# zhongzisha/multi_frame_super_resolution

Hardware: AMD Instinct MI355X
Metric: Mpix/s end-to-end (N-frame burst -> x2 SR) (higher is better)
Workload: dtype f32

## Files before the change

### include/mfsr.h

```cpp
#ifndef MFSR_H
#define MFSR_H

#include <stddef.h>
#include <stdint.h>

#ifdef __cplusplus
extern "C" {
#endif

#define MFSR_VERSION 100
#define MFSR_MAX_FUSE_GROUP 4
#define MFSR_MAX_BURST_FUSE 16

typedef void* mfsr_stream_t;

typedef struct { float x, y; } mfsr_float2;
typedef struct { float x, y, z; } mfsr_float3;
typedef struct { float x, y, z, w; } mfsr_float4;

typedef struct {
    const void* ptr;
    int32_t pitch;
    int32_t width;
    int32_t height;
// ... 233 lines not shown
int mfsr_preAlignPyramid(const float* img, int width, int height, int pitch, void* pyramid, mfsr_stream_t stream);
int mfsr_preAlign(const void* refPyramid, const void* movedPyramid, int width, int height, float maxAngleDeg,
                  void* workspace, mfsr_prealign* result, mfsr_stream_t stream);
int mfsr_preAlign_identity(mfsr_prealign* result, mfsr_stream_t stream);
int mfsr_trackTilesFusedBase(const float* refImg, const float* movedImg, const mfsr_float2* preShift, int preShiftPitch,
                             mfsr_float2* coordinates, int coordinatesPitch, int imgWidth, int imgHeight, int imgPitch,
                             int maxShift, int tileSize, int tileCountX, int tileCountY, float threshold,
                             const float* refSquaredSums, const mfsr_prealign* base, float baseInvScale,
                             mfsr_stream_t stream);
int mfsr_trackTilesFusedUp(const float* refImg, const float* movedImg, const mfsr_float2* coarseShifts, int coarsePitch,
                           int oldLevel, int newLevel, int oldCountX, int oldCountY, int oldTileSize, mfsr_float2* coordinates,
                           int coordinatesPitch, int imgWidth, int imgHeight, int imgPitch, int maxShift, int tileSize,
                           int tileCountX, int tileCountY, float threshold, const float* refSquaredSums,
                           const mfsr_prealign* base, float baseInvScale, mfsr_stream_t stream);
int mfsr_CreateFlowFieldFromTilesBase(mfsr_float2* outImg, mfsr_tex2d texObjShiftXY, int imgWidth, int imgHeight,
                                      int imgPitch, const mfsr_prealign* base, mfsr_stream_t stream);
int mfsr_lucasKanadeIterationWarped(const mfsr_float2* shiftsIn, mfsr_float2* shiftsOut, int pitchShift, const float* refImg,
                                    const float* movedImg, int pitchImg, const float* sumIn, const float* diffIn, float* sumOut,
                                    float* diffOut, int pitchSD, int width, int height, int halfWindowSize, float minDet,
                                    float outScale, mfsr_stream_t stream);
typedef struct {
    const uint16_t* dataIn;
    mfsr_float3* halfOut;
    float* pyr0;
    float* pyr1;
} mfsr_prepare_frame;
int mfsr_prepareFrameFusedBatch(int nFrames, const mfsr_prepare_frame* frames, int halfPitch, float maxVal, int dimX, int dimY,
                                int pyr0Pitch, int pyr1Pitch, const float* taps, int ntaps, mfsr_stream_t stream);
typedef struct {
    const float* movedImg;
    const mfsr_float2* coarseShifts;
    mfsr_float2* coordinates;
    const mfsr_prealign* base;
} mfsr_track_frame;
int mfsr_trackTilesFastSupported(int tileSize, int maxShift);
int mfsr_trackTilesFusedBatch(int nFrames, const mfsr_track_frame* frames, const float* refImg, int coarsePitch, int oldLevel,
                              int newLevel, int oldCountX, int oldCountY, int oldTileSize, int coordinatesPitch, int imgWidth,
                              int imgHeight, int imgPitch, int maxShift, int tileSize, int tileCountX, int tileCountY, float threshold,
                              const float* refSquaredSums, float baseInvScale, mfsr_stream_t stream);
typedef struct {
    mfsr_float2* outImg;
    const mfsr_float2* tileShifts;
    const mfsr_prealign* base;
    const float* movedImg;
    float* sumOut;
    float* diffOut;
} mfsr_flowfield_frame;
int mfsr_CreateFlowFieldWarpedBatch(int nFrames, const mfsr_flowfield_frame* frames, int tilePitch, int tileCountX, int tileCountY,
                                    int imgWidth, int imgHeight, int imgPitch, const float* refImg, int pitchImg, int pitchSD,
                                    mfsr_stream_t stream);
typedef struct {
    const mfsr_float3* movedHalf;
    mfsr_float4* mask;
    const mfsr_float2* flow;
} mfsr_robustness_frame;
int mfsr_robustnessMaskFusedBatch(int nFrames, const mfsr_robustness_frame* frames, const mfsr_float3* rawImgRef, int flowPitch,
                                  int flowWidth, int flowHeight, int imgWidth, int imgHeight, int imgPitch, int maskPitch, float alpha,
                                  float beta, float thresholdM, mfsr_stream_t stream);
int mfsr_prepareFrameMeansBatch(int nFrames, const mfsr_prepare_frame* frames, int meansRowBytes, float maxVal, int w, int h,
                                int pyr0RowBytes, int pyr1RowBytes, const float* taps, int ntaps, mfsr_stream_t stream);
typedef struct {
    const mfsr_float3* movedMeans;
    const uint16_t* movedRaw;
    mfsr_float4* mask;
    const mfsr_float2* flow;
} mfsr_robustness_group_frame;
int mfsr_robustnessMaskGroup(int nFrames, const mfsr_robustness_group_frame* frames, const mfsr_float3* refHalf, int refRowBytes,
                             int flowRowBytes, int meansRowBytes, int maskRowBytes, int w, int h, float maxVal, float alpha,
                             float beta, float thresholdM, mfsr_stream_t stream);
int mfsr_set_robustness_group(int enable);
typedef struct {
    const mfsr_float2* shiftsIn;
    mfsr_float2* shiftsOut;
    const float* movedImg;
    const float* sumIn;
    const float* diffIn;
    float* sumOut;
    float* diffOut;
} mfsr_lk_frame;
int mfsr_lucasKanadeSweepBatch(int nFrames, const mfsr_lk_frame* frames, const float* refImg, int pitchShift, int pitchImg,
                               int pitchSD, int width, int height, int halfWindowSize, float minDet, float outScale,
                               mfsr_stream_t stream);
int mfsr_lucasKanadeSweepBand(int width, int height, int halfWindowSize, int nFrames);
int mfsr_CreateFlowFieldWarped(mfsr_float2* outImg, mfsr_tex2d texObjShiftXY, int imgWidth, int imgHeight, int imgPitch,
                               mfsr_float2 baseShift, float baseRotation, const mfsr_prealign* base, const float* refImg,
                               const float* movedImg, int pitchImg, float* sumOut, float* diffOut, int pitchSD,
                               mfsr_stream_t stream);

int mfsr_finishFusedRows(const mfsr_float3* finalImg, const mfsr_float3* weight, int imgPitch, const mfsr_float3* fallback,
                         int fbPitch, int fbW, int fbH, float u0, float u1, float v0, float v1, mfsr_float3* outImg,
                         int outPitch, uint16_t* out16, int width, int height, float threshold, int applyGamma, float maxOut,
                         int rowOffset, int fullHeight, mfsr_stream_t stream);
int mfsr_finishFusedWindow(const mfsr_float3* finalImg, const mfsr_float3* weight, int imgPitch, const mfsr_float3* fallback,
                           int fbPitch, int fbW, int fbH, float u0, float u1, float v0, float v1, mfsr_float3* outImg,
                           int outPitch, uint16_t* out16, int width, int height, float threshold, int applyGamma, float maxOut,
                           int colOffset, int rowOffset, int fullWidth, int fullHeight, mfsr_stream_t stream);

typedef struct {
    int32_t width, height;
    int32_t frames;
    int32_t reference;
    int32_t scale;
    int32_t mono;
    int32_t cfa[4];
    float black[3], white[3];
    float maxVal;
    int32_t levels;
    int32_t levelFactor[4];
    int32_t tileSize[4];
    int32_t maxShift[4];
    float minimumThreshold;
    float sigmaTracking;
    int32_t lkIterations;
    int32_t lkHalfWindow;
    float lkMinDet;
    float alpha, beta, thresholdM;
    float sigmaTensor;
    float Dth, Dtr, kDetail, kDenoise, kStretch, kShrink;
    float weightThreshold;
    int32_t applyGamma;
    int32_t fused;
    int32_t pairFrames;
    int32_t asyncFuse;
    int32_t preAlign;
    float preAlignMaxAngle;
    int32_t uploadRing;
    int32_t maskErode;
    int32_t rawPacking;
} mfsr_config;

typedef struct mfsr_burst mfsr_burst;

int mfsr_config_default(mfsr_config* cfg, int width, int height, int frames, int scale, int mono);
size_t mfsr_burst_workspace_bytes(const mfsr_config* cfg);
size_t mfsr_burst_accumulator_bytes(const mfsr_config* cfg);
int mfsr_burst_create(mfsr_burst** out, const mfsr_config* cfg, void* workspace, size_t workspaceBytes);
void mfsr_burst_destroy(mfsr_burst* b);

int mfsr_window_check(const mfsr_config* cfg, int x0, int y0, int w, int h);
int mfsr_burst_set_window(mfsr_burst* b, int x0, int y0, int w, int h);
int mfsr_burst_get_window(const mfsr_burst* b, int* x0, int* y0, int* w, int* h);
int mfsr_burst_set_reference(mfsr_burst* b, const uint16_t* rawRef, mfsr_stream_t stream);
int mfsr_burst_set_reference_rows(mfsr_burst* b, const uint16_t* rawRef, int hrRow0, int hrRow1, mfsr_stream_t stream);
int mfsr_burst_add_frame(mfsr_burst* b, const uint16_t* raw, int isReference, mfsr_float3* imgOut,
                         mfsr_float3* totalWeights, mfsr_stream_t stream);
int mfsr_burst_begin(mfsr_burst* b, mfsr_float3* imgOut, mfsr_float3* totalWeights, mfsr_stream_t stream);
int mfsr_burst_flush(mfsr_burst* b, mfsr_stream_t stream);
int mfsr_burst_hold_fuse(mfsr_burst* b, int enable);
int mfsr_burst_fuse_stats(const mfsr_burst* b, int* burstLaunches, int* groupsFused);
int mfsr_set_burst_fuse(int enable);
int mfsr_set_margin_sites(int enable);
int mfsr_set_finish_fuse(int enable);
int mfsr_burst_debug_finish_fused(const mfsr_burst* b, int* finishes);
int mfsr_burst_finish(mfsr_burst* b, const mfsr_float3* imgOut, const mfsr_float3* totalWeights, mfsr_float3* outImg,
                      uint16_t* out16, mfsr_stream_t stream);
int mfsr_burst_finish_rows(mfsr_burst* b, const mfsr_float3* imgOut, const mfsr_float3* totalWeights,
                           mfsr_float3* outImg, uint16_t* out16, int row0, int rows, mfsr_stream_t stream);
int mfsr_burst_set_reference_host(mfsr_burst* b, const uint16_t* hostRaw, mfsr_stream_t stream);
int mfsr_burst_add_frame_host(mfsr_burst* b, const uint16_t* hostRaw, int isReference, mfsr_float3* imgOut,
                              mfsr_float3* totalWeights, mfsr_stream_t stream);
int mfsr_burst_prefetch_host(mfsr_burst* b, const uint16_t* const* hostRaws, int nFrames, mfsr_stream_t stream);
int mfsr_burst_finish_host(mfsr_burst* b, const mfsr_float3* imgOut, const mfsr_float3* totalWeights, uint16_t* out16Dev,
                           uint16_t* out16Host, mfsr_stream_t stream);
int mfsr_burst_host_sync(mfsr_burst* b);
int mfsr_burst_set_host_row_bytes(mfsr_burst* b, int rowBytes);
int mfsr_burst_field_dims(const mfsr_burst* b, int* flowW, int* flowH, int* maskW, int* maskH);
int mfsr_burst_align_frame(mfsr_burst* b, const uint16_t* raw, int isReference, mfsr_float2* flowOut, int flowPitch,
                           mfsr_float4* maskOut, int maskPitch, mfsr_stream_t stream);
int mfsr_burst_align_frames(mfsr_burst* b, int nFrames, const uint16_t* const* raws, const int* isReference,
                            mfsr_float2* const* flowOut, int flowPitch, mfsr_float4* const* maskOut, int maskPitch,
                            mfsr_stream_t stream);
int mfsr_burst_group_size(const mfsr_config* cfg);
int mfsr_burst_fuse_rows(mfsr_burst* b, int nFrames, const uint16_t* const* raws, const mfsr_float2* const* flows, int flowPitch,
                         const mfsr_float4* const* masks, int maskPitch, mfsr_float3* imgOut, mfsr_float3* totalWeights,
                         int accumulatorsUndefined, int rowBegin, int rowEnd, mfsr_stream_t stream);

typedef struct {
    int32_t rowBegin, rowEnd;
    int32_t flowRow0, flowRows;
    int32_t maskRow0, maskRows;
    int32_t rawRow0, rawRows;
    float maxFlowY;
    int32_t reserved[3];
} mfsr_stripe_plan;
int mfsr_dist_stripe_plan(const mfsr_config* cfg, int worldSize, int rank, int rawHalo, mfsr_stripe_plan* out);
int mfsr_checkFlowBound(const mfsr_float2* flow, int pitch, int width, int rows, float bound, int* flag, mfsr_stream_t stream);
int mfsr_maxAbsFlowY(const mfsr_float2* flow, int pitch, int width, int rows, int* maxBits, mfsr_stream_t stream);
int mfsr_exactDivisionOk(float d);

typedef struct mfsr_stream mfsr_stream;
size_t mfsr_stream_workspace_bytes(const mfsr_config* cfg, int radius);
int mfsr_stream_create(mfsr_stream** out, const mfsr_config* cfg, int radius, int framesInHostMemory, void* workspace,
                       size_t workspaceBytes);
void mfsr_stream_destroy(mfsr_stream* s);
int mfsr_stream_push(mfsr_stream* s, const uint16_t* frame, mfsr_float3* outImg, uint16_t* out16, long long* produced,
                     mfsr_stream_t stream);
int mfsr_stream_drain(mfsr_stream* s, mfsr_float3* outImg, uint16_t* out16, long long* produced, mfsr_stream_t stream);
int mfsr_stream_reset(mfsr_stream* s);
int mfsr_stream_set_window(mfsr_stream* s, int x0, int y0, int w, int h);

size_t mfsr_burst_joint_workspace_bytes(const mfsr_config* cfg);
int mfsr_burst_process_joint(mfsr_burst* b, const uint16_t* const* frames, void* jointWorkspace, size_t jointBytes,
                             mfsr_float3* imgOut, mfsr_float3* totalWeights, mfsr_stream_t stream);

typedef struct {
    int (*next_frame)(void* user, uint16_t* dst, mfsr_stream_t stream);
    void (*reset)(void* user);
    void* user;
} mfsr_frame_source;
int mfsr_burst_process_source(mfsr_burst* b, const mfsr_frame_source* src, mfsr_float3* imgOut, mfsr_float3* totalWeights,
                              mfsr_float3* outImg, uint16_t* out16, int* framesUsed, mfsr_stream_t stream);

int mfsr_frameSharpness(int nFrames, const uint16_t* const* frames, int pitch, int width, int height, const int32_t cfa[4],
                        int mono, const int32_t rect[4], long long* sumsDev, mfsr_stream_t stream);
int mfsr_select_frames(int n, const long long* sums, int candidates, float keepRatio, int* reference, int32_t* keep);
int mfsr_burst_select_frames(mfsr_burst* b, int nFrames, const uint16_t* const* frames, int candidates, float keepRatio,
                             long long* sumsDev, int* reference, int32_t* keep, long long* sums, int32_t rect[4],
                             mfsr_stream_t stream);

int mfsr_detectDefects(int nFrames, const uint16_t* const* frames, int pitch, int width, int height, int mono, int threshold,
                       int spread, int minVotes, uint8_t* mapDev, int mapPitch, uint32_t* countsDev, mfsr_stream_t stream);
int mfsr_repairDefects(int nFrames, uint16_t* const* frames, int pitch, int width, int height, int mono, const uint8_t* mapDev,
                       int mapPitch, mfsr_stream_t stream);
int mfsr_burst_repair_defects(mfsr_burst* b, int nFrames, uint16_t* const* frames, int threshold, int spread, int minVotes,
                              uint8_t* mapDev, uint32_t* countsDev, uint32_t counts[2], mfsr_stream_t stream);

int mfsr_frameLevels(int nFrames, const uint16_t* const* frames, int pitch, int width, int height, const int32_t black[4], int sat,
                     const int32_t rect[4], long long* levelsDev, mfsr_stream_t stream);
int mfsr_exposure_gains(int n, const long long* levels, int reference, const int32_t cfa[4], int mono, int perColour, int deadband,
                        int minGain, int maxGain, int32_t* gains, int32_t* status);
int mfsr_applyGains(int nFrames, uint16_t* const* frames, int pitch, int width, int height, const int32_t cfa[4], int mono,
                    const int32_t black[4], int sat, int maxValue, const int32_t* gains, const int32_t* status, mfsr_stream_t stream);
int mfsr_exposure_defaults(const mfsr_config* cfg, int32_t black[4], int32_t* sat, int32_t* maxValue, int32_t* deadband,
                           int32_t* minGain, int32_t* maxGain, int32_t* perColour);
int mfsr_burst_match_exposure(mfsr_burst* b, int nFrames, uint16_t* const* frames, int reference, int perColour, int deadband,
// ... 309 lines not shown
```

### multi_frame_super_resolution_amd/capi.py

```python
from __future__ import annotations

import ctypes
import os
import re
from typing import Dict, List, Tuple

_PKG_DIR = os.path.dirname(os.path.abspath(__file__))
_ROOT = os.path.dirname(_PKG_DIR)
HEADER_PATH = os.path.join(_ROOT, "include", "mfsr.h")
LIB_PATH = os.environ.get("MFSR_LIB") or os.path.join(_PKG_DIR, "lib", "libmfsr_hip.so")


class Float2(ctypes.Structure):
    _fields_ = [("x", ctypes.c_float), ("y", ctypes.c_float)]


class Float3(ctypes.Structure):
    _fields_ = [("x", ctypes.c_float), ("y", ctypes.c_float), ("z", ctypes.c_float)]


class Float4(ctypes.Structure):
    _fields_ = [("x", ctypes.c_float), ("y", ctypes.c_float), ("z", ctypes.c_float), ("w", ctypes.c_float)]


# ... 177 lines not shown
        ret = re.sub(r"\s+", " ", m.group(1)).replace(" *", "*").strip()
        name = m.group(2)
        args = []
        argtxt = re.sub(r"\s+", " ", m.group(3)).strip()
        if argtxt and argtxt != "void":
            for a in argtxt.split(","):
                a = a.strip()
                am = re.match(r"^(.*?)(\w+)(\[\d*\])?$", a)
                typ = am.group(1).strip()
                if am.group(3):
                    typ += "*"
                typ = typ.replace(" *", "*").replace("* ", "*")
                args.append((typ, am.group(2)))
        protos[name] = (ret, args)
    return protos


def path_names(path: str = HEADER_PATH) -> List[str]:
    text = re.sub(r"/\*.*?\*/", " ", open(path).read(), flags=re.S)
    m = re.search(r"typedef\s+enum\s*\{([^{}]*)\}\s*mfsr_path\s*;", text)
    if not m:
        raise ValueError("mfsr.h: enum mfsr_path not found")
    names = [re.sub(r"\s*=.*", "", e).strip() for e in m.group(1).split(",")]
    names = [n for n in names if n]
    if names[-1] != "MFSR_PATH_COUNT" or any(not n.startswith("MFSR_PATH_") for n in names):
        raise ValueError("mfsr.h: unexpected enumerators in mfsr_path")
    return [n[len("MFSR_PATH_"):].lower() for n in names[:-1]]


def _ctype_of(typ: str):
    if "*" in typ:
        return ctypes.c_void_p
    base = typ.replace("const", "").strip()
    if base not in _BY_VALUE:
        raise TypeError(f"mfsr.h: unhandled parameter type {typ!r}")
    return _BY_VALUE[base]


class MfsrError(RuntimeError):
    def __init__(self, fn: str, code: int, msg: str):
        super().__init__(f"{fn} failed with code {code}: {msg}")
        self.code = code


class StripePlan(ctypes.Structure):

    _fields_ = [("rowBegin", ctypes.c_int32), ("rowEnd", ctypes.c_int32), ("flowRow0", ctypes.c_int32),
                ("flowRows", ctypes.c_int32), ("maskRow0", ctypes.c_int32), ("maskRows", ctypes.c_int32),
                ("rawRow0", ctypes.c_int32), ("rawRows", ctypes.c_int32), ("maxFlowY", ctypes.c_float),
                ("reserved", ctypes.c_int32 * 3)]


DIST_HEADER_PATH = os.path.join(_ROOT, "include", "mfsr_dist.h")
DIST_LIB_PATH = os.path.join(_PKG_DIR, "lib", "libmfsr_dist.so")
DIST_STRIPES, DIST_REDUCE, DIST_REDUCE_SCATTER = 0, 1, 2
DIST_ID_BYTES = 128


class _Lib:

    def __init__(self, path: str = LIB_PATH, header: str = HEADER_PATH, mode: int = ctypes.DEFAULT_MODE):
        if not os.path.exists(path):
            raise ImportError(
                f"{path} is missing: build it with `python -c 'import __graft_entry__ as g; g.build()'` "
                "(hipcc --offload-arch=gfx950).  There is no CPU fallback.")
        self.path = path
        self.cdll = ctypes.CDLL(path, mode=mode)
        self.protos = parse_header(header)
        self.raw = {}
        for name, (ret, args) in self.protos.items():
            fn = getattr(self.cdll, name)
            fn.restype = _RET[ret]
            fn.argtypes = [_ctype_of(t) for t, _ in args]
            self.raw[name] = fn

    def __getattr__(self, name: str):
        raw = self.__dict__["raw"].get("mfsr_" + name) or self.__dict__["raw"].get(name)
        if raw is None:
            raise AttributeError(name)
        full = raw.__name__ if hasattr(raw, "__name__") else name
        ret = self.protos[full][0]
        if ret != "int" or full in ("mfsr_version", "mfsr_device_count", "mfsr_gaussin_filter_1D", "mfsr_burst_group_size",
                                     "mfsr_trackTilesFastSupported", "mfsr_packed_row_bytes", "mfsr_render_row_bytes",
                                     "mfsr_get_accumulate_fast_exp", "mfsr_exactDivisionOk", "mfsr_lucasKanadeSweepBand"):
            return raw

        def checked(*a):
            rc = raw(*a)
            if rc != 0:
                es = self.raw.get("mfsr_error_string") or lib().raw["mfsr_error_string"]
                msg = es(rc)
                raise MfsrError(full, rc, msg.decode() if msg else "?")
            return rc

        checked.__name__ = full
        return checked


_lib = None
_dist_lib = None


def lib() -> _Lib:
    global _lib
    if _lib is None:
        _lib = _Lib()
    return _lib


def dist_lib() -> _Lib:
    global _dist_lib
    if _dist_lib is None:
        lib()
        _dist_lib = _Lib(DIST_LIB_PATH, DIST_HEADER_PATH)
    return _dist_lib


def f3(v) -> Float3:
    return Float3(float(v[0]), float(v[1]), float(v[2]))


def f2(v) -> Float2:
    return Float2(float(v[0]), float(v[1]))


def tex(t, width: int | None = None, height: int | None = None, pitch: int | None = None) -> Tex2D:
    h = t.shape[0] if height is None else height
    w = t.shape[1] if width is None else width
    p = t.stride(0) * t.element_size() if pitch is None else pitch
    return Tex2D(t.data_ptr(), p, w, h)
```

### multi_frame_super_resolution_amd/csrc/common.hpp

```cpp
#pragma once

#include <hip/hip_runtime.h>

#include <atomic>
#include <cstdint>
#include <cstdio>
#include <cstdlib>

#include "../../include/mfsr.h"

#define MFSR_WAVE 64

#define MFSR_HIP_TRY(expr)                                                                          \
    do {                                                                                            \
        hipError_t e_ = (expr);                                                                     \
        if (e_ != hipSuccess) {                                                                     \
            fprintf(stderr, "mfsr: %s failed: %s (%s:%d)\n", #expr, hipGetErrorString(e_), __FILE__, \
                    __LINE__);                                                                      \
            return (int)e_;                                                                         \
        }                                                                                           \
    } while (0)

#define MFSR_REQUIRE(cond)                                                                  \
    do {                                                                                    \
        if (!(cond)) {                                                                      \
            fprintf(stderr, "mfsr: invalid argument: %s (%s:%d)\n", #cond, __FILE__, __LINE__); \
            return MFSR_E_INVALID;                                                          \
        }                                                                                   \
    } while (0)

static inline int mfsr_launch_status(const char* what)
{
    hipError_t e = hipGetLastError();
    if (e != hipSuccess) {
        fprintf(stderr, "mfsr: launch of %s failed: %s\n", what, hipGetErrorString(e));
        return (int)e;
    }
    return MFSR_OK;
}

static inline hipStream_t mfsr_s(mfsr_stream_t s) { return (hipStream_t)s; }

static inline bool mfsr_window_ok(int hrW, int hrH, int x0, int y0, int w, int h)
{
    if (hrW <= 0 || hrH <= 0 || x0 < 0 || y0 < 0 || w <= 0 || h <= 0) return false;
    if ((x0 % 16) != 0 || (y0 % 16) != 0) return false;
    if ((long long)x0 + w > hrW || (long long)y0 + h > hrH) return false;
    if ((w % 16) != 0 && x0 + w != hrW) return false;
    if ((h % 16) != 0 && y0 + h != hrH) return false;
    return true;
}
static inline unsigned mfsr_cdiv(long long a, long long b) { return (unsigned)((a + b - 1) / b); }
int mfsr_render_validate(const mfsr_render* r);
static inline mfsr_render mfsr_plain_render()
{
    mfsr_render r = {};
    r.format = MFSR_OUT_RGB16;
    return r;
}

#define MFSR_BATCH_MAX 4

#define MFSR_INTERNAL __attribute__((visibility("hidden")))

static inline bool mfsr_env_is0(const char* name)
{
    const char* e = getenv(name);
    return e && e[0] == '0';
}
static inline bool mfsr_env_is1(const char* name)
{
    const char* e = getenv(name);
    return e && e[0] == '1';
}
static inline int mfsr_env_int(const char* name, int dflt)
{
    const char* e = getenv(name);
    return e ? atoi(e) : dflt;
}
class MfsrKnob {
public:
    template <class FromEnv>
    int get(FromEnv fromEnv)
    {
        int v = v_.load(std::memory_order_relaxed);
        if (v < 0) {
            const int e = fromEnv();
            if (v_.compare_exchange_strong(v, e, std::memory_order_relaxed)) v = e;
        }
        return v;
    }
    void set(int v) { v_.store(v, std::memory_order_relaxed); }

private:
    std::atomic<int> v_{-1};
};

static inline int mfsr_device_cus()
{
    constexpr int kDevs = 64;
    static std::atomic<int> cache[kDevs];
    int dev = 0, cus = 0;
    if (hipGetDevice(&dev) != hipSuccess || dev < 0 || dev >= kDevs) return 256;
    if ((cus = cache[dev].load(std::memory_order_relaxed)) > 0) return cus;
    if (hipDeviceGetAttribute(&cus, hipDeviceAttributeMultiprocessorCount, dev) != hipSuccess || cus <= 0) return 256;
    cache[dev].store(cus, std::memory_order_relaxed);
    return cus;
}

static inline int mfsr_pack_cfa(const int32_t pattern[4], int* packed)
{
    MFSR_REQUIRE(pattern != nullptr);
    for (int i = 0; i < 4; i++) MFSR_REQUIRE(pattern[i] >= 0 && pattern[i] <= MFSR_WHITE);
    *packed = pattern[0] | (pattern[1] << 8) | (pattern[2] << 16) | (pattern[3] << 24);
    return MFSR_OK;
}
MFSR_INTERNAL int mfsr_cfa_packed();
namespace mfsr_cfa {
MFSR_INTERNAL int deBayersSubSample3(int cfa, const uint16_t* dataIn, mfsr_float3* imgOut, float maxVal, int dimX, int dimY, int strideOut,
                                     mfsr_stream_t stream);
MFSR_INTERNAL int prepareFrames(int cfa, int n, const mfsr_prepare_frame* f, int halfPitch, float maxVal, int dimX, int dimY, int pyr0Pitch,
                                int pyr1Pitch, const float* taps, int ntaps, mfsr_stream_t stream, bool means);
MFSR_INTERNAL int deBayerGreenKernel(int cfa, int width, int height, const float* imgIn, int strideIn, mfsr_float3* outImage, int strideOut,
                                     mfsr_float3 blackPoint, mfsr_float3 scale, mfsr_stream_t stream);
MFSR_INTERNAL int deBayerRedBlueKernel(int cfa, int width, int height, const float* imgIn, int strideIn, mfsr_float3* outImage,
                                       int strideOut, mfsr_float3 blackPoint, mfsr_float3 scale, mfsr_stream_t stream);
MFSR_INTERNAL int deBayerFused(int cfa, const uint16_t* raw, mfsr_float3* outImage, int strideOut, int width, int height,
                               mfsr_float3 blackPoint, mfsr_float3 scale, mfsr_stream_t stream);
MFSR_INTERNAL int deBayerFusedRing(int cfa, const uint16_t* raw, mfsr_tex2d outImage, mfsr_float3 blackPoint, mfsr_float3 scale,
                                   mfsr_stream_t stream);
MFSR_INTERNAL int accumulateSuperResFullRows(int cfa, int nFrames, const uint16_t* const* dataIn, mfsr_float3* imgOut,
                                             mfsr_float3* totalWeights, const mfsr_float4* const* certaintyMask, mfsr_tex2d kernelParam,
                                             const mfsr_tex2d* shifts, mfsr_float3 whiteLevel, mfsr_float3 blackLevel, int dimX, int dimY,
                                             int scale, int strideOut, int strideMask, int accumulatorsUndefined, int rowBegin, int rowEnd,
                                             mfsr_stream_t stream);
MFSR_INTERNAL int accumulateSuperResFullWindow(int cfa, int nFrames, const uint16_t* const* dataIn, mfsr_float3* imgOut,
                                               mfsr_float3* totalWeights, const mfsr_float4* const* certaintyMask, mfsr_tex2d kernelParam,
                                               const mfsr_tex2d* shifts, mfsr_float3 whiteLevel, mfsr_float3 blackLevel, int dimX, int dimY,
                                               int scale, int strideOut, int strideMask, int accumulatorsUndefined, int x0, int y0, int w,
                                               int h, mfsr_stream_t stream);
MFSR_INTERNAL int accumulateSuperResBurst(int cfa, int nFrames, const uint16_t* const* dataIn, mfsr_tex2d imgOut, mfsr_tex2d totalWeights,
                                          const mfsr_tex2d* certaintyMasks, mfsr_tex2d kernelParam, const mfsr_tex2d* shifts,
                                          mfsr_float3 whiteLevel, mfsr_float3 blackLevel, int scale, int accumulatorsUndefined,
                                          mfsr_stream_t stream);
// ... 132 lines not shown
```

### multi_frame_super_resolution_amd/csrc/debayer.hip

```cpp
#include <cstring>
#include "common.hpp"
#include "half_pixel.hpp"

static std::atomic<int> g_cfa{MFSR_RED | (MFSR_GREEN << 8) | (MFSR_GREEN << 16) | (MFSR_BLUE << 24)};

int mfsr_cfa_packed() { return g_cfa.load(std::memory_order_relaxed); }

extern "C" int mfsr_set_cfa_pattern(const int32_t pattern[4])
{
    int packed = 0;
    const int rc = mfsr_pack_cfa(pattern, &packed);
    if (rc == MFSR_OK) g_cfa.store(packed, std::memory_order_relaxed);
    return rc;
}

extern "C" int mfsr_get_cfa_pattern(int32_t pattern[4])
{
    MFSR_REQUIRE(pattern != nullptr);
    const int packed = mfsr_cfa_packed();
    for (int i = 0; i < 4; i++) pattern[i] = (packed >> (8 * i)) & 0xff;
    return MFSR_OK;
}

__global__ void __launch_bounds__(256) k_deBayersSubSample3(const uint16_t* __restrict__ dataIn, pix3* __restrict__ imgOut,
// ... 98 lines not shown
            if (gx == cx && gy == cy && lx >= c0 && lx < c0 + PREP_TX && ly >= c0 && ly < c0 + PREP_TY) row_ptr(halfOut, halfPitch, gy)[gx] = p;
        }
        sG[i] = 0.299f * p.x + 0.587f * p.y + 0.114f * p.z;
    }
    __syncthreads();
    if (MEANS) {
        static_assert(PREP_TY == 16, "four rows for each of the block's four thread rows");
        const int lx = threadIdx.x, r0 = 4 * threadIdx.y;
        float mean[4][3];
#pragma unroll
        for (int c = 0; c < 3; c++) {
            float v[6][3];
#pragma unroll
            for (int y = 0; y < 6; y++)
#pragma unroll
                for (int x = 0; x < 3; x++) v[y][x] = sM[(c * PREP_MH + r0 + y) * PREP_MW + lx + x];
#pragma unroll
            for (int r = 0; r < 4; r++) {
                float m = 0.0f;
#pragma unroll
                for (int y = 0; y < 3; y++)
#pragma unroll
                    for (int x = 0; x < 3; x++) m += v[r + y][x];
                mean[r][c] = div9(m);
            }
        }
        const int gx = x0 + lx;
#pragma unroll
        for (int r = 0; r < 4; r++) {
            const int gy = y0 + r0 + r;
            if (gx < dimX && gy < dimY) {
                const pix3 o = {mean[r][0], mean[r][1], mean[r][2]};
                row_ptr(halfOut, halfPitch, gy)[gx] = o;
            }
        }
        __syncthreads();
    }
    for (int i = tid; i < PREP_TX * GH; i += 256) {
        const int ly = i / PREP_TX, lx = i - ly * PREP_TX;
        float s = 0;
        for (int t = 0; t < taps.n; t++) s += taps.t[t] * sG[ly * GW + lx + t];
        sH[i] = s;
    }
    __syncthreads();
    {
        const int lx = threadIdx.x;
#pragma unroll
        for (int r = 0; r < PREP_TY / 4; r++) {
            const int ly = threadIdx.y + 4 * r;
            float s = 0;
            for (int t = 0; t < taps.n; t++) s += taps.t[t] * sH[(ly + t) * PREP_TX + lx];
            sO[ly * PREP_TX + lx] = s;
            const int gx = x0 + lx, gy = y0 + ly;
            if (gx < dimX && gy < dimY) row_ptr(pyr0, pyr0Pitch, gy)[gx] = s;
        }
    }
    if (pyr1 == nullptr) return;
    __syncthreads();
    {
        const int ox = tid & 31, oy = tid >> 5;
        const int gx = x0 / 2 + ox, gy = y0 / 2 + oy;
        if (gx < dimX / 2 && gy < dimY / 2) {
            const float ax = sO[(2 * oy) * PREP_TX + 2 * ox], ay = sO[(2 * oy) * PREP_TX + 2 * ox + 1];
            const float bx = sO[(2 * oy + 1) * PREP_TX + 2 * ox], by = sO[(2 * oy + 1) * PREP_TX + 2 * ox + 1];
            row_ptr(pyr1, pyr1Pitch, gy)[gx] = ((ax + ay) + (bx + by)) * 0.25f;
        }
    }
}

int mfsr_cfa::prepareFrames(int cfa, int n, const mfsr_prepare_frame* f, int halfPitch, float maxVal, int dimX, int dimY, int pyr0Pitch,
                            int pyr1Pitch, const float* taps, int ntaps, mfsr_stream_t stream, bool means)
{
    MFSR_REQUIRE(f && n >= 1 && n <= MFSR_BATCH_MAX && taps && dimX > 0 && dimY > 0);
    MFSR_REQUIRE((long long)halfPitch >= 12LL * dimX && (halfPitch & 3) == 0);
    MFSR_REQUIRE((long long)pyr0Pitch >= 4LL * dimX && (pyr0Pitch & 3) == 0);
    MFSR_REQUIRE(ntaps > 0 && (ntaps & 1) == 1);
    if (ntaps / 2 > PREP_MAXC0) return MFSR_E_UNSUPPORTED;
    if (means && ntaps < 3) return MFSR_E_UNSUPPORTED;
    PrepFrames fr;
    memset(&fr, 0, sizeof(fr));
    for (int i = 0; i < n; i++) {
        MFSR_REQUIRE(f[i].dataIn && f[i].halfOut && f[i].pyr0 && ((uintptr_t)f[i].dataIn & 3) == 0);
        MFSR_REQUIRE((f[i].pyr1 != nullptr) == (f[0].pyr1 != nullptr));
        fr.f[i] = PrepFrame{f[i].dataIn, (pix3*)f[i].halfOut, f[i].pyr0, f[i].pyr1};
    }
    if (f[0].pyr1) MFSR_REQUIRE((long long)pyr1Pitch >= 4LL * (dimX / 2) && (pyr1Pitch & 3) == 0 && dimX >= 2 && dimY >= 2);
    PrepTaps tp;
    tp.n = ntaps;
    for (int i = 0; i < ntaps; i++) tp.t[i] = taps[i];
    const int c0 = ntaps / 2, GW = PREP_TX + 2 * c0, GH = PREP_TY + 2 * c0;
    const size_t lds = sizeof(float) * ((size_t)GW * GH + (size_t)PREP_TX * GH + (size_t)PREP_TX * PREP_TY);
    dim3 block(64, 4), grid(mfsr_cdiv(dimX, PREP_TX), mfsr_cdiv(dimY, PREP_TY), n);
    if (means) {
        const size_t planes = 3 * PREP_MW * PREP_MH, rows = (size_t)PREP_TX * GH;
        const size_t ldsMeans = sizeof(float) * ((size_t)GW * GH + (planes > rows ? planes : rows));
        hipLaunchKernelGGL(k_prepareFrameFused<true>, grid, block, ldsMeans, mfsr_s(stream), fr, halfPitch, maxVal, dimX, dimY, pyr0Pitch,
                           pyr1Pitch, tp, cfa);
        return mfsr_launch_status("prepareFrameMeans");
    }
    hipLaunchKernelGGL(k_prepareFrameFused<false>, grid, block, lds, mfsr_s(stream), fr, halfPitch, maxVal, dimX, dimY, pyr0Pitch, pyr1Pitch,
                       tp, cfa);
    return mfsr_launch_status("prepareFrameFused");
}

extern "C" int mfsr_prepareFrameFused(const uint16_t* dataIn, mfsr_float3* halfOut, int halfPitch, float maxVal, int dimX,
                                      int dimY, float* pyr0, int pyr0Pitch, float* pyr1, int pyr1Pitch, const float* taps,
                                      int ntaps, mfsr_stream_t stream)
{
    const mfsr_prepare_frame f = {dataIn, halfOut, pyr0, pyr1};
    return mfsr_cfa::prepareFrames(mfsr_cfa_packed(), 1, &f, halfPitch, maxVal, dimX, dimY, pyr0Pitch, pyr1Pitch, taps, ntaps, stream, false);
}

extern "C" int mfsr_prepareFrameFusedBatch(int nFrames, const mfsr_prepare_frame* frames, int halfPitch, float maxVal, int dimX, int dimY,
                                           int pyr0Pitch, int pyr1Pitch, const float* taps, int ntaps, mfsr_stream_t stream)
{
    return mfsr_cfa::prepareFrames(mfsr_cfa_packed(), nFrames, frames, halfPitch, maxVal, dimX, dimY, pyr0Pitch, pyr1Pitch, taps, ntaps, stream,
                                   false);
}

extern "C" int mfsr_prepareFrameMeansBatch(int nFrames, const mfsr_prepare_frame* frames, int meansRowBytes, float maxVal, int w, int h,
                                           int pyr0RowBytes, int pyr1RowBytes, const float* taps, int ntaps, mfsr_stream_t stream)
{
    return mfsr_cfa::prepareFrames(mfsr_cfa_packed(), nFrames, frames, meansRowBytes, maxVal, w, h, pyr0RowBytes, pyr1RowBytes, taps, ntaps,
                                   stream, true);
}

struct Lvl {
    float bp[3], sc[3];
};

__device__ __forceinline__ float green_at(const float* __restrict__ imgIn, int strideIn, int x, int y, int thisPixel,
                                          const Lvl& L)
{
#define RAWC(xx, yy, c) ((row_ptr(imgIn, strideIn, (yy))[(xx)] - L.bp[c]) * L.sc[c])
    if (thisPixel == MFSR_GREEN) return RAWC(x, y, 1);
    if (thisPixel != MFSR_RED && thisPixel != MFSR_BLUE) return 0.0f;
    const int c = (thisPixel == MFSR_RED) ? 0 : 2;
    const float p = RAWC(x, y, c);
    const float xMinus2 = RAWC(x - 2, y, c), xMinus1 = RAWC(x - 1, y, 1), xPlus1 = RAWC(x + 1, y, 1),
                xPlus2 = RAWC(x + 2, y, c);
    const float yMinus2 = RAWC(x, y - 2, c), yMinus1 = RAWC(x, y - 1, 1), yPlus1 = RAWC(x, y + 1, 1),
                yPlus2 = RAWC(x, y + 2, c);
#undef RAWC
    const float gradientX = 0.5f * fabsf(xPlus1 - xMinus1);
    const float gradientY = 0.5f * fabsf(yPlus1 - yMinus1);
    const float laplaceX = 0.25f * fabsf(2.0f * p - xMinus2 - xPlus2);
    const float laplaceY = 0.25f * fabsf(2.0f * p - yMinus2 - yPlus2);
    const float interpolX = 0.125f * (-xMinus2 + 4.0f * xMinus1 + 2.0f * p + 4.0f * xPlus1 - xPlus2);
    const float interpolY = 0.125f * (-yMinus2 + 4.0f * yMinus1 + 2.0f * p + 4.0f * yPlus1 - yPlus2);
    const float weight = (gradientY + laplaceY) / (gradientX + gradientY + laplaceX + laplaceY + 0.000000001f);
    return weight * interpolX + (1.0f - weight) * interpolY;
}

__global__ void __launch_bounds__(256) k_deBayerGreen(int width, int height, const float* __restrict__ imgIn, int strideIn,
                                                     pix3* outImage, int strideOut, Lvl L, int cfa)
{
    const int x = blockIdx.x * blockDim.x + threadIdx.x;
    const int y = blockIdx.y * blockDim.y + threadIdx.y;
    if (x >= width - 2 || x < 2) return;
    if (y >= height - 2 || y < 2) return;
    row_ptr(outImage, strideOut, y)[x].y = green_at(imgIn, strideIn, x, y, cfa_at(cfa, y, x), L);
}

static inline Lvl make_lvl(mfsr_float3 bp, mfsr_float3 sc)
{
    Lvl L;
// ... 224 lines not shown
```

### multi_frame_super_resolution_amd/csrc/erode.hip

```cpp
#include "common.hpp"

#define ER_TX 64
#define ER_TY 16
#define ER_ROWS 4

struct ErodeFrames {
    const float4* in[MFSR_MAX_FUSE_GROUP];
    float4* out[MFSR_MAX_FUSE_GROUP];
};

__device__ __forceinline__ float4 min3(const float4& a, const float4& b)
{
    return make_float4(fminf(a.x, b.x), fminf(a.y, b.y), fminf(a.z, b.z), 0.0f);
}

template <int R>
__global__ void __launch_bounds__(ER_TX* ER_ROWS)
    k_maskErode(ErodeFrames fr, int width, int height, int inPitch, int outPitch)
{
    constexpr int LW = ER_TX + 2 * R, LH = ER_TY + 2 * R;
    constexpr int NT = ER_TX * ER_ROWS, PER = (LH * ER_TX + NT - 1) / NT;
    __shared__ float4 sT[LH][LW];
    const float4* __restrict__ in = fr.in[blockIdx.z];
    float4* __restrict__ out = fr.out[blockIdx.z];
    const int lx = threadIdx.x, ly = threadIdx.y;
    const int tid = ly * ER_TX + lx;
    const int x0 = blockIdx.x * ER_TX, y0 = blockIdx.y * ER_TY;
    for (int t = tid; t < LH * LW; t += NT) {
        const int r = t / LW, c = t - r * LW;
        const int gy = clampi(y0 - R + r, 1, height - 2), gx = clampi(x0 - R + c, 1, width - 2);
        sT[r][c] = row_ptr(in, inPitch, gy)[gx];
    }
    __syncthreads();
    float4 m[PER];
#pragma unroll
    for (int k = 0; k < PER; k++) {
        const int t = tid + k * NT;
        if (t < LH * ER_TX) {
            const int r = t / ER_TX, c = t - r * ER_TX;
            float4 v = sT[r][c];
#pragma unroll
            for (int i = 1; i <= 2 * R; i++) v = min3(v, sT[r][c + i]);
            v.w = sT[r][c + R].w;
            m[k] = v;
        }
    }
    __syncthreads();
#pragma unroll
    for (int k = 0; k < PER; k++) {
        const int t = tid + k * NT;
        if (t < LH * ER_TX) sT[t / ER_TX][t % ER_TX] = m[k];
    }
    __syncthreads();
    const int x = x0 + lx;
    if (x >= width) return;
#pragma unroll
    for (int k = 0; k < ER_TY / ER_ROWS; k++) {
        const int r = ly + k * ER_ROWS, y = y0 + r;
        if (y >= height) break;
        float4 v = sT[r][lx];
#pragma unroll
        for (int j = 1; j <= 2 * R; j++) v = min3(v, sT[r + j][lx]);
        v.w = sT[r + R][lx].w;
        if (x < 1 || y < 1 || x >= width - 1 || y >= height - 1) v = make_float4(0.0f, 0.0f, 0.0f, 0.0f);
        row_ptr(out, outPitch, y)[x] = v;
    }
}

extern "C" int mfsr_erodeMaskBatch(int nFrames, const mfsr_float4* const* in, mfsr_float4* const* out, int width, int height,
                                   int inPitch, int outPitch, int radius, mfsr_stream_t stream)
{
    MFSR_REQUIRE(nFrames >= 1 && nFrames <= MFSR_MAX_FUSE_GROUP && in != nullptr && out != nullptr);
    MFSR_REQUIRE(radius >= 1 && radius <= 2);
    MFSR_REQUIRE(width >= 3 && height >= 3);
    MFSR_REQUIRE((long long)inPitch >= 16LL * width && (inPitch & 15) == 0);
    MFSR_REQUIRE((long long)outPitch >= 16LL * width && (outPitch & 15) == 0);
    ErodeFrames fr;
    for (int k = 0; k < MFSR_MAX_FUSE_GROUP; k++) {
        fr.in[k] = nullptr;
        fr.out[k] = nullptr;
    }
    const unsigned long long inSpan = (unsigned long long)inPitch * (height - 1) + 16ULL * width;
    const unsigned long long outSpan = (unsigned long long)outPitch * (height - 1) + 16ULL * width;
    for (int k = 0; k < nFrames; k++) {
        MFSR_REQUIRE(in[k] != nullptr && out[k] != nullptr);
        MFSR_REQUIRE(((uintptr_t)in[k] & 15) == 0 && ((uintptr_t)out[k] & 15) == 0);
        fr.in[k] = (const float4*)in[k];
        fr.out[k] = (float4*)out[k];
    }
    for (int k = 0; k < nFrames; k++) {
        const unsigned long long o0 = (unsigned long long)(uintptr_t)out[k], o1 = o0 + outSpan;
        for (int j = 0; j < nFrames; j++) {
            const unsigned long long i0 = (unsigned long long)(uintptr_t)in[j];
            MFSR_REQUIRE(o1 <= i0 || i0 + inSpan <= o0);
            if (j != k) {
                const unsigned long long p0 = (unsigned long long)(uintptr_t)out[j];
                MFSR_REQUIRE(o1 <= p0 || p0 + outSpan <= o0);
            }
        }
    }
    dim3 block(ER_TX, ER_ROWS), grid(mfsr_cdiv(width, ER_TX), mfsr_cdiv(height, ER_TY), nFrames);
    if (radius == 1)
        hipLaunchKernelGGL(k_maskErode<1>, grid, block, 0, mfsr_s(stream), fr, width, height, inPitch, outPitch);
    else
        hipLaunchKernelGGL(k_maskErode<2>, grid, block, 0, mfsr_s(stream), fr, width, height, inPitch, outPitch);
    return mfsr_launch_status("erodeMaskBatch");
}
```

### multi_frame_super_resolution_amd/csrc/lk_fused.hip

```cpp
#include <cstdlib>
#include <cstring>
#include "common.hpp"
#include "lk_math.hpp"

constexpr int LK_TY = 16;

__device__ __forceinline__ int lk_mirror_index(int i, int n)
{
    i = i < 0 ? -1 - i : i;
    return i >= n ? 2 * n - 1 - i : i;
}

__device__ __forceinline__ int lk_mirror_index_clamped(int i, int n)
{
    return clampi(lk_mirror_index(i, n), 0, n - 1);
}

template <typename T>
__device__ __forceinline__ T* lk_at(T* base, int pitch, int y, int x)
{
    return (T*)((char*)base + (uint32_t)((uint32_t)y * (uint32_t)pitch + (uint32_t)x * (uint32_t)sizeof(T)));
}

struct LkGather {
// ... 321 lines not shown
        sf = base->sinRotation;
        bx = base->shiftX;
        by = base->shiftY;
    } else {
        if (baseRotation != 0.0f) {
            cf = cosf(baseRotation);
            sf = sinf(baseRotation);
        }
        bx = baseShift.x;
        by = baseShift.y;
    }
    float2 shift;
    shift.x = cf * -bx - sf * -by;
    shift.y = sf * -bx + cf * -by;
    const float patchCenterX = (float)(pxX - imgWidth / 2);
    const float patchCenterY = (float)(pxY - imgHeight / 2);
    shift.x += cf * patchCenterX - sf * patchCenterY - patchCenterX;
    shift.y += sf * patchCenterX + cf * patchCenterY - patchCenterY;
    const float2 shiftPatch =
        tex2<ADDR_CLAMP>(texShift, mfsr_div((float)pxX + 0.5f, dW), mfsr_div((float)pxY + 0.5f, dH));
    shift.x += shiftPatch.x;
    shift.y += shiftPatch.y;
    *lk_at(outImg, imgPitch, pxY, pxX) = shift;
    float wv, rv;
    lk_warp_sample(refImg, movedImg, pitchImg, imgWidth, imgHeight, pxX, pxY, shift, wv, rv, dW, dH);
    *lk_at(sumOut, pitchSD, pxY, pxX) = wv + rv;
    *lk_at(diffOut, pitchSD, pxY, pxX) = wv - rv;
}

static int flow_field_warped_impl(int n, const mfsr_flowfield_frame* f, int tilePitch, int tileW, int tileH, int imgWidth, int imgHeight,
                                  int imgPitch, mfsr_float2 baseShift, float baseRotation, const float* refImg, int pitchImg, int pitchSD,
                                  mfsr_stream_t stream)
{
    MFSR_REQUIRE(f && n >= 1 && n <= MFSR_BATCH_MAX && refImg && imgWidth >= 2 && imgHeight >= 2);
    MFSR_REQUIRE((long long)imgPitch >= 8LL * imgWidth && (imgPitch & 7) == 0);
    MFSR_REQUIRE((long long)pitchImg >= 4LL * imgWidth && (pitchImg & 3) == 0 && (long long)pitchSD >= 4LL * imgWidth && (pitchSD & 3) == 0);
    if ((long long)imgPitch * imgHeight >= (1LL << 32) || (long long)pitchImg * imgHeight >= (1LL << 32) ||
        (long long)pitchSD * imgHeight >= (1LL << 32))
        return MFSR_E_UNSUPPORTED;
    mfsr_tex2d tex;
    tex.ptr = f[0].tileShifts;
    tex.pitch = tilePitch;
    tex.width = tileW;
    tex.height = tileH;
    MFSR_REQUIRE(mfsr_tex_ok(tex, 8) && (tilePitch & 7) == 0);
    FlowFieldFrames fr;
    memset(&fr, 0, sizeof(fr));
    for (int i = 0; i < n; i++) {
        MFSR_REQUIRE(f[i].outImg && f[i].tileShifts && f[i].movedImg && f[i].sumOut && f[i].diffOut);
        MFSR_REQUIRE(((uintptr_t)f[i].outImg & 7) == 0 && ((uintptr_t)f[i].tileShifts & 7) == 0);
        MFSR_REQUIRE((f[i].base != nullptr) == (f[0].base != nullptr));
        fr.f[i] = FlowFieldFrame{(float2*)f[i].outImg, (const float2*)f[i].tileShifts, f[i].base, f[i].movedImg, f[i].sumOut, f[i].diffOut};
    }
    dim3 block(64, 4), grid(mfsr_cdiv(imgWidth, 64), mfsr_cdiv(imgHeight, 4), n);
    const MfsrExactDiv dW = mfsr_exact_div((float)imgWidth), dH = mfsr_exact_div((float)imgHeight);
    if (f[0].base)
        hipLaunchKernelGGL(k_flowFieldWarped<true>, grid, block, 0, mfsr_s(stream), fr, tex, imgWidth, imgHeight, imgPitch,
                           make_float2(0.0f, 0.0f), 0.0f, refImg, pitchImg, pitchSD, dW, dH);
    else
        hipLaunchKernelGGL(k_flowFieldWarped<false>, grid, block, 0, mfsr_s(stream), fr, tex, imgWidth, imgHeight, imgPitch,
                           make_float2(baseShift.x, baseShift.y), baseRotation, refImg, pitchImg, pitchSD, dW, dH);
    return mfsr_launch_status("CreateFlowFieldWarped");
}

extern "C" int mfsr_CreateFlowFieldWarped(mfsr_float2* outImg, mfsr_tex2d texObjShiftXY, int imgWidth, int imgHeight, int imgPitch,
                                          mfsr_float2 baseShift, float baseRotation, const mfsr_prealign* base, const float* refImg,
                                          const float* movedImg, int pitchImg, float* sumOut, float* diffOut, int pitchSD,
                                          mfsr_stream_t stream)
{
    const mfsr_flowfield_frame f = {outImg, (const mfsr_float2*)texObjShiftXY.ptr, base, movedImg, sumOut, diffOut};
    return flow_field_warped_impl(1, &f, texObjShiftXY.pitch, texObjShiftXY.width, texObjShiftXY.height, imgWidth, imgHeight, imgPitch,
                                  baseShift, baseRotation, refImg, pitchImg, pitchSD, stream);
}

extern "C" int mfsr_CreateFlowFieldWarpedBatch(int nFrames, const mfsr_flowfield_frame* frames, int tilePitch, int tileCountX,
                                               int tileCountY, int imgWidth, int imgHeight, int imgPitch, const float* refImg,
                                               int pitchImg, int pitchSD, mfsr_stream_t stream)
{
    const mfsr_float2 z = {0.0f, 0.0f};
    return flow_field_warped_impl(nFrames, frames, tilePitch, tileCountX, tileCountY, imgWidth, imgHeight, imgPitch, z, 0.0f, refImg,
                                  pitchImg, pitchSD, stream);
}

#define MFSR_LK_SWEEP_MAX_BATCH 4
struct LkSweepFrame {
    const float2* flowIn;
    float2* flowOut;
    const float* moved;
    const float* sumIn;
    const float* diffIn;
    float* sumOut;
    float* diffOut;
};
struct LkSweepBatch {
    LkSweepFrame f[MFSR_LK_SWEEP_MAX_BATCH];
};

__device__ __forceinline__ float lk_wshr1(float v)
{
    return __uint_as_float(__builtin_amdgcn_update_dpp(0u, __float_as_uint(v), 0x138, 0xf, 0xf, true));
}
__device__ __forceinline__ float lk_wshl1(float v)
{
    return __uint_as_float(__builtin_amdgcn_update_dpp(0u, __float_as_uint(v), 0x130, 0xf, 0xf, true));
}

template <int HT>
__global__ void __launch_bounds__(64)
    k_lkSweep(LkSweepBatch batch, const float* __restrict__ refImg, int pitchShift, int pitchImg, int pitchSD, int width, int height,
              float minDet, float outScale, int bandRows, int strips, int bands, int perXcd, int nFramesLaunch, MfsrExactDiv dW, MfsrExactDiv dH)
{
    constexpr int h = HT, HALO = HT + 2, WIN = 2 * HT + 1, VW = 64 - 2 * HALO;
    int sIdx, bIdx, fIdx;
    if (perXcd > 0) {
        const int t = ((int)blockIdx.x & 7) * perXcd + ((int)blockIdx.x >> 3);
        if (t >= strips * bands * nFramesLaunch) return;
        sIdx = t % strips;
        bIdx = (t / strips) % bands;
        fIdx = t / (strips * bands);
    } else {
        sIdx = blockIdx.x, bIdx = blockIdx.y, fIdx = blockIdx.z;
    }
    const LkSweepFrame F = batch.f[fIdx];
    const int lane = threadIdx.x;
    const int cx0 = sIdx * VW, ry0 = bIdx * bandRows;
    const int colIn = cx0 - HALO + lane;
    const int gxIn = lk_mirror_index(colIn, width);
    const int colOut = colIn - h;
    const bool outLane = lane >= 2 * h + 2 && lane <= 61 && colOut < width;
    const int colOutC = min(max(colOut, 0), width - 1);
    const bool ringCol = colOut < h || colOut >= width - h;
    const int rows = min(bandRows, height - ry0);
    const int T = rows + 2 * HALO;

    float s0 = 0, s1 = 0, s2 = 0, s3 = 0, s4 = 0;
    float d0 = 0;
    float H[5][WIN];
#pragma unroll
    for (int k = 0; k < 5; k++)
#pragma unroll
        for (int j = 0; j < WIN; j++) H[k][j] = 0.0f;

    auto load_sum = [&](int t, float& sv) { sv = *lk_at(F.sumIn, pitchSD, lk_mirror_index(ry0 - HALO + t, height), gxIn); };
    auto load_diff = [&](int t, float& dv) { dv = *lk_at(F.diffIn, pitchSD, lk_mirror_index(ry0 - HALO + t, height), gxIn); };
    float sA, sB, dA = 0, dB = 0;
    load_sum(0, sA);
    load_sum(min(1, T - 1), sB);
    LkGather pend;
    int pendY = -1;
    auto finish_pending = [&]() {
        if (pendY < 0) return;
        const float wv = lk_warp_finish(pend);
        const float rv = pend.rv;
        if (outLane) {
            *lk_at(F.sumOut, pitchSD, pendY, colOutC) = wv + rv;
            *lk_at(F.diffOut, pitchSD, pendY, colOutC) = wv - rv;
        }
    };

    for (int t0 = 0; t0 < T; t0 += WIN) {
#pragma unroll
        for (int j = 0; j < WIN; j++) {
            const int t = t0 + j;
            if (t >= T) break;
            s0 = s1, s1 = s2, s2 = s3, s3 = s4, s4 = sA;
            d0 = dA, dA = dB;
            sA = sB;
            load_sum(min(t + 2, T - 1), sB);
            load_diff(t, dB);
            if (t < 4) continue;
            const int y = ry0 + t - 2 * HALO;
            const int yc = min(max(y, 0), height - 1);
            float2 shift = *lk_at(F.flowIn, pitchShift, yc, colOutC);
            const float rvOwn = *lk_at(refImg, pitchImg, yc, colOutC);
            const float xp1 = lk_wshl1(s2), xp2 = lk_wshl1(xp1), xm1 = lk_wshr1(s2), xm2 = lk_wshr1(xm1);
            float tx = xp2;
            tx -= xp1 * 8.0f;
            tx += xm1 * 8.0f;
            tx -= xm2;
            const float Ix = tx * (1.0f / 24.0f);
            float ty = s4;
            ty -= s3 * 8.0f;
            ty += s1 * 8.0f;
            ty -= s0;
            const float Iy = ty * (1.0f / 24.0f);
            const float It = d0;
            float P[5] = {Ix * Ix, Ix * Iy, Iy * Iy, Ix * It, Iy * It};
#pragma unroll
            for (int k = 0; k < 5; k++) {
                float acc = P[k];
#pragma unroll
                for (int q = 0; q < 2 * HT; q++) acc = P[k] + lk_wshr1(acc);
                H[k][j] = acc;
            }
            if (t < 2 * HALO) continue;
            float V[5];
#pragma unroll
            for (int k = 0; k < 5; k++) {
                float sum = 0;
#pragma unroll
                for (int d = 1; d <= WIN; d++) sum += H[k][(j + d) % WIN];
                V[k] = sum;
            }
            if (!(ringCol || y < h || y >= height - h)) {
                float inv[4];
                if (lk_pinv(V[0], V[1], V[2], minDet, inv)) {
                    float UV0 = inv[0] * V[3] + inv[1] * V[4];
                    float UV1 = inv[2] * V[3] + inv[3] * V[4];
                    UV0 = isnan(UV0) ? 0 : UV0;
                    UV1 = isnan(UV1) ? 0 : UV1;
                    shift.x += UV0;
                    shift.y += UV1;
                }
            }
            if (F.sumOut) {
                finish_pending();
                lk_warp_issue(F.moved, pitchImg, width, height, colOutC, y, shift, outLane, pend, dW, dH);
                pend.rv = rvOwn;
                pendY = y;
            }
            shift.x *= outScale;
            shift.y *= outScale;
            if (outLane) *lk_at(F.flowOut, pitchShift, y, colOutC) = shift;
        }
    }
    if (F.sumOut) finish_pending();
}

static bool lk_sweep_geometry(int nFrames, int width, int height, int h)
{
    return nFrames >= 1 && nFrames <= MFSR_LK_SWEEP_MAX_BATCH && h >= 1 && h <= 7 && width >= 64 && height >= 2 * (h + 2);
}
int mfsr_lk_sweep_accepts(int nFrames, int width, int height, int halfWindowSize, int pitchShift, int pitchImg, int pitchSD)
{
    MFSR_REQUIRE(nFrames >= 1 && nFrames <= MFSR_LK_SWEEP_MAX_BATCH);
    if (!lk_sweep_geometry(nFrames, width, height, halfWindowSize)) return MFSR_E_UNSUPPORTED;
    MFSR_REQUIRE((long long)pitchShift >= 8LL * width && (pitchShift & 7) == 0);
    MFSR_REQUIRE((long long)pitchImg >= 4LL * width && (pitchImg & 3) == 0 && (long long)pitchSD >= 4LL * width && (pitchSD & 3) == 0);
    if ((long long)pitchShift * height >= (1LL << 32) || (long long)pitchImg * height >= (1LL << 32) || (long long)pitchSD * height >= (1LL << 32))
        return MFSR_E_UNSUPPORTED;
    return MFSR_OK;
}

extern "C" int mfsr_lucasKanadeSweepBand(int width, int height, int halfWindowSize, int nFrames)
{
    if (!lk_sweep_geometry(nFrames, width, height, halfWindowSize)) return 0;
    const int h = halfWindowSize, VW = 64 - 2 * (h + 2);
    const int strips = mfsr_cdiv(width, VW);
    static const int forceBand = mfsr_env_int("MFSR_LK_BAND", 0);
    int band = (int)((long long)height * strips * nFrames / 8192);
    band = (band + 4) & ~7;
    band = band < 8 ? 8 : (band > 32 ? 32 : band);
    {
        static const int occ[8] = {0, 8, 7, 6, 5, 4, 4, 4};
        const long long places = 1024LL * occ[h];
        const long long maxBands = places / ((long long)strips * nFrames);
        if (maxBands >= 1) {
            int b = (int)((height + maxBands - 1) / maxBands);
            b = b < 8 ? 8 : b;
            if (b <= 64) band = b;
        }
    }
    if (forceBand >= 8) band = forceBand;
    return band;
}

extern "C" int mfsr_lucasKanadeSweepBatch(int nFrames, const mfsr_lk_frame* frames, const float* refImg, int pitchShift, int pitchImg,
                                          int pitchSD, int width, int height, int halfWindowSize, float minDet, float outScale,
                                          mfsr_stream_t stream)
{
    MFSR_REQUIRE(frames && refImg);
    const int rc = mfsr_lk_sweep_accepts(nFrames, width, height, halfWindowSize, pitchShift, pitchImg, pitchSD);
    if (rc) return rc;
    LkSweepBatch b;
    memset(&b, 0, sizeof(b));
    for (int i = 0; i < nFrames; i++) {
        const mfsr_lk_frame& f = frames[i];
        MFSR_REQUIRE(f.shiftsIn && f.shiftsOut && f.shiftsIn != f.shiftsOut && f.movedImg && f.sumIn && f.diffIn);
        MFSR_REQUIRE(((uintptr_t)f.shiftsIn & 7) == 0 && ((uintptr_t)f.shiftsOut & 7) == 0);
        MFSR_REQUIRE((f.sumOut != nullptr) == (f.diffOut != nullptr) && f.sumOut != f.sumIn && f.diffOut != f.diffIn);
        MFSR_REQUIRE(!f.sumOut || outScale == 1.0f);
        b.f[i] = LkSweepFrame{(const float2*)f.shiftsIn, (float2*)f.shiftsOut, f.movedImg, f.sumIn, f.diffIn, f.sumOut, f.diffOut};
    }
    const int h = halfWindowSize, VW = 64 - 2 * (h + 2);
    const int strips = mfsr_cdiv(width, VW);
    const int band = mfsr_lucasKanadeSweepBand(width, height, h, nFrames);
    static const int xcdRemap = mfsr_env_int("MFSR_LK_XCD", 1);
    const int bands = mfsr_cdiv(height, band);
    const int total = strips * bands * nFrames;
    const int perXcd = xcdRemap ? mfsr_cdiv(total, 8) : 0;
    dim3 grid = perXcd ? dim3(8 * perXcd, 1, 1) : dim3(strips, bands, nFrames), block(64);
    const MfsrExactDiv dW = mfsr_exact_div((float)width), dH = mfsr_exact_div((float)height);
#define LKS_CASE(HT)                                                                                                          \
    case HT:                                                                                                                  \
        hipLaunchKernelGGL(k_lkSweep<HT>, grid, block, 0, mfsr_s(stream), b, refImg, pitchShift, pitchImg, pitchSD, width,    \
                           height, minDet, outScale, band, strips, bands, perXcd, nFrames, dW, dH);                           \
        break;
    switch (h) {
        LKS_CASE(1)
        LKS_CASE(2)
        LKS_CASE(3)
        LKS_CASE(4)
        LKS_CASE(5)
        LKS_CASE(6)
        LKS_CASE(7)
    }
#undef LKS_CASE
    return mfsr_launch_status("lucasKanadeSweepBatch");
}
```

### multi_frame_super_resolution_amd/csrc/pipeline.cpp

```cpp
#include <hip/hip_runtime.h>

#include <cmath>
#include <cstdio>
#include <cstring>
#include <new>
#include <vector>

#include "common.hpp"
#include "raw_stage.hpp"

namespace {

constexpr int kMaxLevels = 4;
constexpr int kMaxTimedLaunches = 4096;
constexpr int kRing = 2 * MFSR_MAX_FUSE_GROUP;
constexpr int kRingMax = MFSR_MAX_BURST_FUSE;
inline int ring_size(const mfsr_config* c) { return c->frames <= kRing ? kRing : (c->frames < kRingMax ? c->frames : kRingMax); }
constexpr int kMaxUploadRing = 32;

inline size_t align_up(size_t v, size_t a) { return (v + a - 1) / a * a; }

struct Img {
    void* ptr = nullptr;
    int pitch = 0;
    int w = 0, h = 0;
};

struct FrameProducts {
    uint16_t* raw;
    Img half;
    Img pyr[8];
    void* prePyr;
};

struct AlignScratch {
    Img shifts[kMaxLevels];
    Img lkSum[2], lkDiff[2];
    mfsr_prealign* preResult;
};

struct Layout {
    int W, H, hw, hh, tw, th, hrW, hrH;
    int flowScale;
    int lw[kMaxLevels], lh[kMaxLevels];
    int tcx[kMaxLevels], tcy[kMaxLevels];
    int maxFactor;
    FrameProducts ref, mov[MFSR_MAX_FUSE_GROUP];
    AlignScratch work[MFSR_MAX_FUSE_GROUP];
    int nAlign;
    Img kparam4;
    Img tensor, tensorTmp, tensorSm;
    Img fallback;
    Img tmpA, tmpB;
    Img flowBuf[2 * kRingMax];
    Img maskBuf[kRingMax];
    Img maskRaw[MFSR_MAX_FUSE_GROUP];
    Img pre[kMaxLevels];
    Img warped, Ix, Iy, It, rawf;
    float *refTiles, *movTiles, *cc, *boxX, *boxY, *sqsum, *dist;
    float* refSq[kMaxLevels];
    void* preWork;
    uint16_t* rawRing[kMaxUploadRing];
    uint16_t* refRaw[2];
    uint8_t* stage[kMaxUploadRing + 2];
    size_t total;
};

struct Bump {
    char* base;
    size_t off;
    void* take(size_t bytes)
    {
        off = align_up(off, 256);
        void* p = base ? base + off : nullptr;
        off += bytes;
        return p;
    }
    Img image(int w, int h, int elemBytes)
    {
        Img im;
        im.w = w;
        im.h = h;
        im.pitch = (int)align_up((size_t)w * elemBytes, 64);
        im.ptr = take((size_t)im.pitch * h);
        return im;
    }
};

int ilog2(int v)
{
    int l = 0;
    while ((1 << l) < v) l++;
    return l;
}

int validate(const mfsr_config* c)
{
    MFSR_REQUIRE(c != nullptr);
    MFSR_REQUIRE(c->width >= 64 && c->height >= 64 && (c->width % 4) == 0 && (c->height % 4) == 0);
    MFSR_REQUIRE(c->frames >= 1 && c->reference >= 0 && c->reference < c->frames);
    MFSR_REQUIRE(c->scale >= 1 && c->scale <= 8);
    MFSR_REQUIRE(c->levels >= 1 && c->levels <= kMaxLevels);
    MFSR_REQUIRE(c->levelFactor[c->levels - 1] == 1);
    for (int l = 0; l < c->levels; l++) {
        const int f = c->levelFactor[l];
        MFSR_REQUIRE(f >= 1 && f <= 128 && (f & (f - 1)) == 0);
        if (l > 0) MFSR_REQUIRE(c->levelFactor[l] < c->levelFactor[l - 1]);
        MFSR_REQUIRE(c->tileSize[l] >= 4 && c->tileSize[l] <= 128 && c->maxShift[l] >= 1 && c->maxShift[l] <= 15);
        MFSR_REQUIRE(c->tileSize[l] > 2 * c->maxShift[l]);
        if (c->fused) {
            const long long T = c->tileSize[l], S = c->maxShift[l], Lt = T + 2 * S, R = 2 * S + 1;
            if (4 * (T * T + Lt * (Lt + 1) + 1 + Lt * R + R * R + 4) > 160 * 1024) {
                fprintf(stderr, "mfsr: tileSize %d / maxShift %d exceeds the fused tile tracker's LDS budget (use cfg.fused = 0)\n",
                        (int)T, (int)S);
                return MFSR_E_UNSUPPORTED;
            }
        }
    }
    MFSR_REQUIRE(c->lkIterations >= 0 && c->lkHalfWindow >= 0 && c->lkHalfWindow <= 15);
    MFSR_REQUIRE(c->maxVal > 0);
    if (c->preAlign) MFSR_REQUIRE(c->preAlignMaxAngle >= 0.0f && c->preAlignMaxAngle <= 45.0f);
    MFSR_REQUIRE(c->uploadRing == 0 || (c->uploadRing >= 3 && c->uploadRing <= kMaxUploadRing));
    MFSR_REQUIRE(c->pairFrames >= 0 && c->pairFrames <= MFSR_MAX_FUSE_GROUP);
    MFSR_REQUIRE(c->maskErode >= 0 && c->maskErode <= 2);
    if (c->rawPacking != MFSR_PACK_NONE) MFSR_REQUIRE(c->uploadRing > 0 && mfsr_packed_row_bytes(c->rawPacking, c->width) > 0);
    return MFSR_OK;
}

Layout make_layout(const mfsr_config* c, char* base)
{
    Layout layout;
    memset((void*)&layout, 0, sizeof(layout));
    Layout* L = &layout;
    Bump b{base, 0};
    L->W = c->width;
    L->H = c->height;
    L->hw = c->width / 2;
    L->hh = c->height / 2;
    L->tw = c->mono ? L->W : L->hw;
    L->th = c->mono ? L->H : L->hh;
    L->flowScale = c->mono ? 1 : 2;
    L->hrW = c->width * c->scale;
    L->hrH = c->height * c->scale;
    L->maxFactor = c->levelFactor[0];
    const int nl = ilog2(L->maxFactor) + 1;

    L->ref.half = b.image(L->hw, L->hh, 12);
    L->mov[0].half = b.image(L->hw, L->hh, 12);
    for (int i = 0; i < nl; i++) {
        L->ref.pyr[i] = b.image(L->tw >> i, L->th >> i, 4);
        L->mov[0].pyr[i] = b.image(L->tw >> i, L->th >> i, 4);
    }
    L->kparam4 = b.image(L->tw, L->th, 16);
    L->tensor = b.image(L->tw, L->th, 12);
    L->tensorTmp = b.image(L->tw, L->th, 12);
    L->tensorSm = b.image(L->tw, L->th, 12);
    L->fallback = b.image(L->W, L->H, 12);
    L->tmpA = b.image(L->tw, L->th, 4);
    L->tmpB = b.image(L->tw, L->th, 4);
    for (int i = 0; i < 2 * kRing; i++) L->flowBuf[i] = b.image(L->tw, L->th, 8);
    for (int i = 0; i < kRing; i++) L->maskBuf[i] = b.image(L->hw, L->hh, 16);
    size_t maxTileFloats = 0, maxTiles = 0, maxDist = 0;
    for (int l = 0; l < c->levels; l++) {
        const int f = c->levelFactor[l];
        L->lw[l] = L->tw / f;
        L->lh[l] = L->th / f;
        L->tcx[l] = L->lw[l] / c->tileSize[l] > 0 ? L->lw[l] / c->tileSize[l] : 1;
        L->tcy[l] = L->lh[l] / c->tileSize[l] > 0 ? L->lh[l] / c->tileSize[l] : 1;
        L->work[0].shifts[l] = b.image(L->tcx[l], L->tcy[l], 8);
        L->pre[l] = b.image(L->tcx[l], L->tcy[l], 8);
        const size_t tiles = (size_t)L->tcx[l] * L->tcy[l];
        const size_t Lt = (size_t)c->tileSize[l] + 2 * c->maxShift[l];
        const size_t R = 2 * (size_t)c->maxShift[l] + 1;
        if (tiles * Lt * Lt > maxTileFloats) maxTileFloats = tiles * Lt * Lt;
        if (tiles > maxTiles) maxTiles = tiles;
        if (tiles * R * R > maxDist) maxDist = tiles * R * R;
    }
    for (int l = 0; l < kMaxLevels; l++) L->refSq[l] = nullptr;
    if (c->fused) {
        for (int l = 0; l < c->levels; l++) L->refSq[l] = (float*)b.take((size_t)L->tcx[l] * L->tcy[l] * 4);
        for (int i = 0; i < 2; i++) {
            L->work[0].lkSum[i] = b.image(L->tw, L->th, 4);
            L->work[0].lkDiff[i] = b.image(L->tw, L->th, 4);
        }
    }
    L->Ix = b.image(L->tw, L->th, 4);
    L->Iy = b.image(L->tw, L->th, 4);
    if (!c->fused) {
        L->warped = b.image(L->tw, L->th, 4);
        L->It = b.image(L->tw, L->th, 4);
        L->rawf = b.image(L->W, L->H, 4);
        L->refTiles = (float*)b.take(maxTileFloats * 4);
        L->movTiles = (float*)b.take(maxTileFloats * 4);
        L->cc = (float*)b.take(maxTileFloats * 4);
        L->boxX = (float*)b.take(maxTileFloats * 4);
        L->boxY = (float*)b.take(maxTileFloats * 4);
        L->sqsum = (float*)b.take(maxTiles * 4);
        L->dist = (float*)b.take(maxDist * 4);
    }
    if (c->preAlign) {
        const size_t pb = mfsr_preAlign_pyramid_bytes(L->tw, L->th);
        L->ref.prePyr = b.take(pb);
        L->mov[0].prePyr = b.take(pb);
        L->preWork = b.take(mfsr_preAlign_workspace_bytes(c->preAlignMaxAngle));
        L->work[0].preResult = (mfsr_prealign*)b.take(sizeof(mfsr_prealign));
    }
    L->nAlign = c->fused ? mfsr_burst_group_size(c) : 1;
    for (int q = 1; q < L->nAlign; q++) {
        FrameProducts& M = L->mov[q];
        AlignScratch& S = L->work[q];
        M.half = b.image(L->hw, L->hh, 12);
        for (int i = 0; i < nl; i++) M.pyr[i] = b.image(L->tw >> i, L->th >> i, 4);
        for (int l = 0; l < c->levels; l++) S.shifts[l] = b.image(L->tcx[l], L->tcy[l], 8);
        for (int i = 0; i < 2; i++) {
            S.lkSum[i] = b.image(L->tw, L->th, 4);
            S.lkDiff[i] = b.image(L->tw, L->th, 4);
        }
        if (c->preAlign) {
            M.prePyr = b.take(mfsr_preAlign_pyramid_bytes(L->tw, L->th));
            S.preResult = (mfsr_prealign*)b.take(sizeof(mfsr_prealign));
        }
    }
    for (int i = 0; i < c->uploadRing; i++) L->rawRing[i] = (uint16_t*)b.take((size_t)L->W * L->H * 2);
    if (c->uploadRing > 0)
        for (int i = 0; i < 2; i++) L->refRaw[i] = (uint16_t*)b.take((size_t)L->W * L->H * 2);
    if (c->maskErode > 0)
        for (int i = 0; i < mfsr_burst_group_size(c); i++) L->maskRaw[i] = b.image(L->hw, L->hh, 16);
    if (c->rawPacking != MFSR_PACK_NONE)
        for (int i = 0; i < c->uploadRing + 2; i++)
            L->stage[i] = (uint8_t*)b.take((size_t)mfsr_packed_row_bytes(c->rawPacking, L->W) * L->H);
    for (int i = kRing; i < ring_size(c); i++) {
        L->flowBuf[2 * i] = b.image(L->tw, L->th, 8);
        L->flowBuf[2 * i + 1] = b.image(L->tw, L->th, 8);
        L->maskBuf[i] = b.image(L->hw, L->hh, 16);
    }
    L->total = align_up(b.off, 256);
    return layout;
}

mfsr_tex2d as_tex(const Img& im)
{
    mfsr_tex2d t;
    t.ptr = im.ptr;
    t.pitch = im.pitch;
    t.width = im.w;
    t.height = im.h;
    return t;
}

}

struct FuseGroup {
    int n;
    int slot[MFSR_MAX_FUSE_GROUP];
    const uint16_t* raw[MFSR_MAX_FUSE_GROUP];
    const Img* flow[MFSR_MAX_FUSE_GROUP];
    const Img* mask[MFSR_MAX_FUSE_GROUP];
    bool deferred[MFSR_MAX_FUSE_GROUP];
    int isRef[MFSR_MAX_FUSE_GROUP];
    mfsr_float3 *imgOut, *totalWeights;
};

struct mfsr_burst {
    mfsr_burst(const mfsr_config& c, char* workspace) : cfg(c), L(make_layout(&c, workspace)) {}
    mfsr_config cfg;
    int cfa;
    const Layout L;
    FrameProducts ref;
    float taps[99];
    int ntaps;
    float tensorTaps[99];
    int ntensorTaps;
    const Img* flowCur;
    const Img* maskCur;
    mfsr_prealign* preCur;
    bool haveRef;
    bool refStale;
    FuseGroup pend;
    FuseGroup held;
    bool heldHas;
    int group;
    bool holdFuse;
    int nHold;
    FuseGroup hold[MFSR_MAX_BURST_FUSE / MFSR_MAX_FUSE_GROUP];
    int burstLaunches, burstGroups;
    int nFramesTimed;
    struct Fresh {
        bool has;
        mfsr_float3 *imgOut, *totalWeights;
    } fresh;
    int frameCounter;
    hipStream_t fuseStream;
    int ring;
    hipEvent_t evAligned[kRingMax];
    hipEvent_t evFused[kRingMax];
    hipEvent_t evRefStart, evRefDone;
    bool refOnFuse;
    bool fusedOutstanding[kRingMax];
    const Img* slotFlow[kRingMax];
    hipStream_t copyStream;
    hipStream_t downStream;
    hipEvent_t evFinished, evDown;
    bool downRecorded;
    hipEvent_t evBand[16];
    int framesSinceRef;
    bool holdLastGroup;
    hipEvent_t evUp[kMaxUploadRing + 2];
    hipEvent_t evFree[kMaxUploadRing + 2];
    bool freeRecorded[kMaxUploadRing + 2];
    hipStream_t freeOn[kMaxUploadRing + 2];
    int hostRowBytes;
    bool renderOn;
    mfsr_render render;
    bool sharpenOn;
    mfsr_sharpen sharpen;
    int sharpenedFinishes;
    bool denoiseOn;
    mfsr_denoise denoise;
    int denoisedFinishes;
    int robustGroupLaunches;
    uint16_t* finishOut16;
    bool finishTaken;
    int fusedFinishes;
    std::vector<uint64_t> autoStats;
    std::vector<float> autoLut;
    bool localToneOn;
    mfsr_local_tone localTone;
    const float* localToneGrid;
    std::vector<uint64_t> toneStats;
    std::vector<float> toneGrid;
    bool chainOn;
    mfsr_finish_chain chain;
    const float* chainGrid;
    int chainReach;
    int chainedFinishes;
    int geometryFinishes;
    unsigned long long hostEpoch;
    hipEvent_t evEpoch;
    hipEvent_t evUnp[kMaxUploadRing + 2];
    hipEvent_t unpDone[kMaxUploadRing + 2];
    int unpQ[kMaxUploadRing + 2], nUnp;
    struct Prefetched {
        const uint16_t* host;
        int slot;
    } prefetched[kMaxUploadRing];
    int nPrefetched, prefetchHead;
    bool upPending;
    int upPendingSlot;
    int refSlot;
    bool hostBusy;
    int upCounter, refCounter;
    const uint16_t* refHost;
    const uint16_t* refDev;
    std::vector<float> jointHost;
    struct Window {
        bool on = false;
        int x0 = 0, y0 = 0, w = 0, h = 0;
    } win, winNext;
    bool timing;
    int nEvents;
    hipEvent_t evStart[kMaxTimedLaunches], evStop[kMaxTimedLaunches];
    unsigned char evLaunches[kMaxTimedLaunches];
    int32_t paths[MFSR_PATH_COUNT];
};

#define TRY(expr)                  \
    do {                           \
// ... 19 lines not shown
}

static int fuse_group(mfsr_burst* b, const FuseGroup& g, int fresh, int r0, int r1, mfsr_stream_t stream)
{
    const mfsr_config& c = b->cfg;
    const Layout& L = b->L;
    const mfsr_float3 white = cfg_white(c), black = cfg_black(c);
    mfsr_tex2d maskTex[MFSR_MAX_FUSE_GROUP], flows[MFSR_MAX_FUSE_GROUP];
    group_tables(g, maskTex, flows);
    const mfsr_float4* masks[MFSR_MAX_FUSE_GROUP];
    for (int i = 0; i < g.n; i++) masks[i] = (const mfsr_float4*)maskTex[i].ptr;
    const int maskPitch = maskTex[0].pitch;
    if (!b->win.on)
        return mfsr_cfa::accumulateSuperResFullRows(b->cfa, g.n, g.raw, g.imgOut, g.totalWeights, masks, as_tex(L.kparam4), flows, white, black,
                                               L.W, L.H, c.scale, 12 * L.hrW, maskPitch, fresh, r0, r1, stream);
    const int pitch = 12 * b->win.w;
    const size_t off = (size_t)r0 * pitch;
    return mfsr_cfa::accumulateSuperResFullWindow(b->cfa, g.n, g.raw, (mfsr_float3*)((char*)g.imgOut + off),
                                             (mfsr_float3*)((char*)g.totalWeights + off), masks, as_tex(L.kparam4), flows, white, black, L.W,
                                             L.H, c.scale, pitch, maskPitch, fresh, b->win.x0, b->win.y0 + r0, b->win.w, r1 - r0, stream);
}

extern "C" int mfsr_config_default(mfsr_config* cfg, int width, int height, int frames, int scale, int mono)
{
    MFSR_REQUIRE(cfg != nullptr);
    memset(cfg, 0, sizeof(*cfg));
    cfg->width = width;
    cfg->height = height;
    cfg->frames = frames;
    cfg->reference = 0;
    cfg->scale = scale;
    cfg->mono = mono;
    if (mono) {
        cfg->cfa[0] = cfg->cfa[1] = cfg->cfa[2] = cfg->cfa[3] = MFSR_GREEN;
    } else {
        cfg->cfa[0] = MFSR_RED;
        cfg->cfa[1] = MFSR_GREEN;
        cfg->cfa[2] = MFSR_GREEN;
        cfg->cfa[3] = MFSR_BLUE;
    }
    for (int i = 0; i < 3; i++) {
        cfg->black[i] = 256.0f;
        cfg->white[i] = 4095.0f - 256.0f;
    }
    cfg->maxVal = 4095.0f;
    cfg->levels = 2;
    cfg->levelFactor[0] = 2;
    cfg->levelFactor[1] = 1;
    cfg->tileSize[0] = 32;
    cfg->tileSize[1] = 32;
    cfg->maxShift[0] = 4;
    cfg->maxShift[1] = 4;
    cfg->minimumThreshold = 0.0f;
    cfg->sigmaTracking = 0.5f;
    cfg->lkIterations = 3;
    cfg->lkHalfWindow = 3;
    cfg->lkMinDet = 1e-4f;
    cfg->alpha = 1e-4f;
    cfg->beta = 1e-6f;
    cfg->thresholdM = 1.0f;
    cfg->sigmaTensor = 1.0f;
    cfg->Dth = 0.005f;
    cfg->Dtr = 0.05f;
    cfg->kDetail = 0.3f;
    cfg->kDenoise = 2.0f;
    cfg->kStretch = 2.0f;
    cfg->kShrink = 2.0f;
    cfg->weightThreshold = 1e-3f;
    cfg->applyGamma = 0;
    cfg->fused = 1;
    cfg->pairFrames = 1;
    cfg->preAlign = 0;
    cfg->preAlignMaxAngle = 20.0f;
    cfg->asyncFuse = 0;
    return MFSR_OK;
}

extern "C" size_t mfsr_burst_workspace_bytes(const mfsr_config* cfg)
{
    if (validate(cfg) != MFSR_OK) return 0;
    return make_layout(cfg, nullptr).total;
}

extern "C" size_t mfsr_burst_accumulator_bytes(const mfsr_config* cfg)
{
    if (!cfg || cfg->width <= 0 || cfg->height <= 0 || cfg->scale <= 0) return 0;
    return (size_t)12 * cfg->scale * cfg->width * (size_t)cfg->scale * cfg->height;
}

extern "C" int mfsr_burst_create(mfsr_burst** out, const mfsr_config* cfg, void* workspace, size_t workspaceBytes)
{
    MFSR_REQUIRE(out != nullptr && workspace != nullptr);
    TRY(validate(cfg));
    int cfa = 0;
    TRY(mfsr_pack_cfa(cfg->cfa, &cfa));
    if (mfsr_device_count() <= 0) {
        fprintf(stderr, "mfsr: no HIP device available (there is no CPU fallback)\n");
        return MFSR_E_NODEVICE;
    }
    MFSR_REQUIRE(((uintptr_t)workspace & 255) == 0);
    mfsr_burst* b = new (std::nothrow) mfsr_burst(*cfg, (char*)workspace);
    MFSR_REQUIRE(b != nullptr);
    if (b->L.total > workspaceBytes) {
        fprintf(stderr, "mfsr: workspace too small: need %zu bytes, got %zu\n", b->L.total, workspaceBytes);
        delete b;
        return MFSR_E_WORKSPACE;
    }
    b->cfa = cfa;
    b->ntaps = mfsr_gaussin_filter_1D(cfg->sigmaTracking, b->taps);
    b->ntensorTaps = mfsr_gaussin_filter_1D(cfg->sigmaTensor, b->tensorTaps);
    b->flowCur = &b->L.flowBuf[0];
    b->maskCur = &b->L.maskBuf[0];
    b->preCur = b->L.work[0].preResult;
    b->ref = b->L.ref;
    b->pend.n = 0;
    b->group = mfsr_burst_group_size(&b->cfg);
    b->ring = ring_size(&b->cfg);
    b->holdFuse = false;
    b->nHold = 0;
    b->burstLaunches = b->burstGroups = 0;
    b->fresh.has = false;
    b->nFramesTimed = 0;
    b->timing = false;
    b->nEvents = 0;
    memset(b->evStart, 0, sizeof(b->evStart));
    memset(b->evStop, 0, sizeof(b->evStop));
    b->frameCounter = 0;
    b->fuseStream = nullptr;
    b->evRefStart = b->evRefDone = nullptr;
    b->refOnFuse = false;
    for (int i = 0; i < kRingMax; i++) {
        b->evAligned[i] = b->evFused[i] = nullptr;
        b->fusedOutstanding[i] = false;
        b->slotFlow[i] = nullptr;
    }
    if (cfg->asyncFuse) {
        int lo = 0, hi = 0;
        hipError_t e = hipDeviceGetStreamPriorityRange(&lo, &hi);
        static const int prioMode = [] {
            const char* v = getenv("MFSR_FUSE_PRIO");
            return !v ? 0 : (v[0] == 'l' ? 1 : (v[0] == 'n' ? 2 : 0));
        }();
        const int prio = prioMode == 1 ? lo : (prioMode == 2 ? (lo + hi) / 2 : hi);
        if (e == hipSuccess) e = hipStreamCreateWithPriority(&b->fuseStream, hipStreamNonBlocking, prio);
        if (e == hipSuccess) e = hipEventCreateWithFlags(&b->evRefStart, hipEventDisableTiming);
        if (e == hipSuccess) e = hipEventCreateWithFlags(&b->evRefDone, hipEventDisableTiming);
        for (int i = 0; i < b->ring && e == hipSuccess; i++) {
            e = hipEventCreateWithFlags(&b->evAligned[i], hipEventDisableTiming);
            if (e == hipSuccess) e = hipEventCreateWithFlags(&b->evFused[i], hipEventDisableTiming);
        }
        if (e != hipSuccess) {
            mfsr_burst_destroy(b);
            return MFSR_E_NODEVICE;
        }
    }
    b->copyStream = nullptr;
    b->downStream = nullptr;
    b->evFinished = b->evDown = nullptr;
    b->downRecorded = false;
    b->upCounter = b->refCounter = 0;
    for (int i = 0; i < 16; i++) b->evBand[i] = nullptr;
    b->framesSinceRef = 0;
    b->holdLastGroup = false;
    b->heldHas = false;
    b->held.n = 0;
    b->refHost = b->refDev = nullptr;
    b->refSlot = -1;
    b->hostBusy = false;
    b->upPending = false;
    b->upPendingSlot = -1;
    b->nPrefetched = b->prefetchHead = 0;
    for (int i = 0; i < kMaxUploadRing + 2; i++) {
        b->evUp[i] = b->evFree[i] = b->evUnp[i] = b->unpDone[i] = nullptr;
        b->freeRecorded[i] = false;
        b->freeOn[i] = nullptr;
    }
    b->hostRowBytes = 0;
    b->renderOn = false;
    b->sharpenOn = false;
    b->sharpenedFinishes = 0;
    b->denoiseOn = false;
    b->denoisedFinishes = 0;
    b->localToneOn = false;
    b->localToneGrid = nullptr;
    b->chainOn = false;
    b->chainGrid = nullptr;
    b->chainReach = 0;
    b->chainedFinishes = 0;
    b->geometryFinishes = 0;
    b->robustGroupLaunches = 0;
    b->finishOut16 = nullptr;
    b->finishTaken = false;
    b->fusedFinishes = 0;
    b->nUnp = 0;
    b->hostEpoch = 0;
    b->evEpoch = nullptr;
    if (cfg->uploadRing > 0) {
        hipError_t e = hipStreamCreateWithFlags(&b->copyStream, hipStreamNonBlocking);
        if (e == hipSuccess) e = hipStreamCreateWithFlags(&b->downStream, hipStreamNonBlocking);
        if (e == hipSuccess) e = hipEventCreateWithFlags(&b->evFinished, hipEventDisableTiming);
        if (e == hipSuccess) e = hipEventCreateWithFlags(&b->evDown, hipEventDisableTiming);
        if (e == hipSuccess) e = hipEventCreateWithFlags(&b->evEpoch, hipEventDisableTiming);
// ... 321 lines not shown
    *w = v.on ? v.w : b->L.hrW;
    *h = v.on ? v.h : b->L.hrH;
    return MFSR_OK;
}

static int track_tiles(mfsr_burst* b, const FrameProducts& refF, float* const* refSq, const FrameProducts& movF,
                       const AlignScratch& work, const mfsr_prealign* hostBase, mfsr_stream_t stream)
{
    const mfsr_config& c = b->cfg;
    const Layout& L = b->L;
    const mfsr_float2 zero2 = {0.0f, 0.0f};
    for (int l = 0; l < c.levels; l++) {
        const int pi = ilog2(c.levelFactor[l]);
        const Img& ref = refF.pyr[pi];
        const Img& mov = movF.pyr[pi];
        const int T = c.tileSize[l], S = c.maxShift[l];
        const int tiles = L.tcx[l] * L.tcy[l];
        const mfsr_float2* pre = nullptr;
        b->paths[mfsr_trackTilesFastSupported(T, S) ? MFSR_PATH_TRACK_FAST_PAIR : MFSR_PATH_TRACK_GENERIC_PAIR]++;
        if (c.fused && l > 0) {
            TRY(mfsr_trackTilesFusedUp((const float*)ref.ptr, (const float*)mov.ptr, (const mfsr_float2*)work.shifts[l - 1].ptr,
                                       work.shifts[l - 1].pitch, c.levelFactor[l - 1], c.levelFactor[l], L.tcx[l - 1], L.tcy[l - 1],
                                       c.tileSize[l - 1], (mfsr_float2*)work.shifts[l].ptr, work.shifts[l].pitch, ref.w, ref.h, ref.pitch, S,
                                       T, L.tcx[l], L.tcy[l], c.minimumThreshold, refSq[l], c.preAlign ? work.preResult : nullptr,
                                       1.0f / (float)c.levelFactor[l], stream));
            b->paths[MFSR_PATH_TRACK_FUSED_UP]++;
            continue;
        }
        if (l > 0) {
            TRY(mfsr_UpSampleShifts((const mfsr_float2*)work.shifts[l - 1].ptr, (mfsr_float2*)L.pre[l].ptr,
                                    work.shifts[l - 1].pitch, L.pre[l].pitch, c.levelFactor[l - 1], c.levelFactor[l],
                                    L.tcx[l - 1], L.tcy[l - 1], L.tcx[l], L.tcy[l], c.tileSize[l - 1], T, stream));
            pre = (const mfsr_float2*)L.pre[l].ptr;
        }
        if (c.fused) {
            TRY(mfsr_trackTilesFusedBase((const float*)ref.ptr, (const float*)mov.ptr, pre, L.pre[l].pitch,
                                         (mfsr_float2*)work.shifts[l].ptr, work.shifts[l].pitch, ref.w, ref.h, ref.pitch, S, T,
                                         L.tcx[l], L.tcy[l], c.minimumThreshold, refSq[l],
                                         c.preAlign ? work.preResult : nullptr, 1.0f / (float)c.levelFactor[l], stream));
            b->paths[MFSR_PATH_TRACK_FUSED_BASE]++;
        } else {
            b->paths[MFSR_PATH_TRACK_CHAIN]++;
            if (!pre) {
                MFSR_HIP_TRY(hipMemsetAsync(L.pre[l].ptr, 0, (size_t)L.pre[l].pitch * L.pre[l].h, mfsr_s(stream)));
                pre = (const mfsr_float2*)L.pre[l].ptr;
            }
            TRY(mfsr_convertToTilesOverlapBorder((const float*)ref.ptr, L.refTiles, ref.w, ref.h, ref.pitch, S, T, L.tcx[l],
                                                 L.tcy[l], zero2, 0.0f, stream));
            mfsr_float2 base = zero2;
            float rot = 0.0f;
            if (hostBase) {
                const float inv = 1.0f / (float)c.levelFactor[l];
                base.x = hostBase->shiftX * inv;
                base.y = hostBase->shiftY * inv;
                rot = hostBase->rotation;
            }
            TRY(mfsr_convertToTilesOverlapPreShift((const float*)mov.ptr, L.movTiles, pre, L.pre[l].pitch, mov.w, mov.h,
                                                   mov.pitch, S, T, L.tcx[l], L.tcy[l], base, rot, stream));
            TRY(mfsr_crossCorrelateTiles(L.refTiles, L.movTiles, L.cc, S, T, tiles, stream));
            TRY(mfsr_squaredSum(L.refTiles, L.sqsum, S, T, tiles, stream));
            TRY(mfsr_boxFilterWithBorderX(L.movTiles, L.boxX, S, T, tiles, stream));
            TRY(mfsr_boxFilterWithBorderY(L.boxX, L.boxY, S, T, tiles, stream));
            TRY(mfsr_normalizedCC(L.cc, L.sqsum, L.boxY, L.dist, S, T, tiles, stream));
            TRY(mfsr_findMinimum(L.dist, (mfsr_float2*)work.shifts[l].ptr, work.shifts[l].pitch, S, tiles, L.tcx[l],
                                 c.minimumThreshold, stream));
            TRY(mfsr_addRoundedPreShift(pre, L.pre[l].pitch, (mfsr_float2*)work.shifts[l].ptr, work.shifts[l].pitch, L.tcx[l],
                                        L.tcy[l], stream));
        }
    }
    return MFSR_OK;
}

static int upload_slot_of(const mfsr_burst* b, const uint16_t* raw)
{
    if (!raw) return -1;
    for (int i = 0; i < b->cfg.uploadRing; i++)
        if (b->L.rawRing[i] == raw) return i;
    for (int i = 0; i < 2; i++)
        if (b->cfg.uploadRing > 0 && b->L.refRaw[i] == raw) return b->cfg.uploadRing + i;
    return -1;
}

static int align_deferred(mfsr_burst* b, FuseGroup& g, mfsr_stream_t stream);

static int timed_begin(mfsr_burst* b, mfsr_stream_t stream, bool* timed)
{
    *timed = b->timing && b->nEvents < kMaxTimedLaunches;
    if (*timed) {
        const int i = b->nEvents;
        if (!b->evStart[i]) MFSR_HIP_TRY(hipEventCreate(&b->evStart[i]));
        if (!b->evStop[i]) MFSR_HIP_TRY(hipEventCreate(&b->evStop[i]));
        MFSR_HIP_TRY(hipEventRecord(b->evStart[i], mfsr_s(stream)));
    }
    return MFSR_OK;
}
static int timed_end(mfsr_burst* b, bool timed, int launches, int frames, mfsr_stream_t stream)
{
    if (timed) {
        MFSR_HIP_TRY(hipEventRecord(b->evStop[b->nEvents], mfsr_s(stream)));
        b->evLaunches[b->nEvents] = launches;
        b->nEvents++;
        b->nFramesTimed += frames;
    }
    return MFSR_OK;
}

static bool fresh_for(const mfsr_burst* b, const mfsr_float3* imgOut, const mfsr_float3* totalWeights)
{
    return b->fresh.has && b->fresh.imgOut == imgOut && b->fresh.totalWeights == totalWeights;
}
static int zero_fresh(mfsr_burst* b, mfsr_stream_t stream)
{
    const size_t bytes = acc_bytes(b);
    MFSR_HIP_TRY(hipMemsetAsync(b->fresh.imgOut, 0, bytes, mfsr_s(stream)));
    MFSR_HIP_TRY(hipMemsetAsync(b->fresh.totalWeights, 0, bytes, mfsr_s(stream)));
    b->fresh.has = false;
    return MFSR_OK;
}
static int take_fresh(mfsr_burst* b, const mfsr_float3* imgOut, const mfsr_float3* totalWeights, mfsr_stream_t stream, int* freshNow)
{
    *freshNow = fresh_for(b, imgOut, totalWeights);
    if (b->fresh.has && !*freshNow) TRY(zero_fresh(b, stream));
    b->fresh.has = false;
    return MFSR_OK;
}

static int release_group_slots(mfsr_burst* b, const FuseGroup& g, mfsr_stream_t stream)
{
    if (!b->copyStream) return MFSR_OK;
    for (int j = 0; j < g.n; j++) {
        const int us = upload_slot_of(b, g.raw[j]);
        if (us >= 0) TRY(record_free(b, us, stream));
    }
    return MFSR_OK;
}

static int wait_slot_fused(mfsr_burst* b, int slot, mfsr_stream_t stream)
{
    if (b->fuseStream && b->fusedOutstanding[slot]) {
        MFSR_HIP_TRY(hipStreamWaitEvent(mfsr_s(stream), b->evFused[slot], 0));
        b->fusedOutstanding[slot] = false;
    }
    return MFSR_OK;
}

static bool burst_idle(const mfsr_burst* b) { return b->pend.n == 0 && !b->heldHas && b->nHold == 0 && b->nUnp == 0; }

static MfsrKnob g_burst_fuse;
static bool burst_fuse_enabled()
{
    return g_burst_fuse.get([] { return mfsr_env_is0("MFSR_BURST_FUSE") ? 0 : 1; }) == 1;
}
extern "C" int mfsr_set_burst_fuse(int enable)
{
    g_burst_fuse.set(enable ? 1 : 0);
    return MFSR_OK;
}
static MfsrKnob g_finish_fuse;
static bool finish_fuse_enabled()
{
    return g_finish_fuse.get([] { return mfsr_env_is0("MFSR_FINISH_FUSE") ? 0 : 1; }) == 1;
}
extern "C" int mfsr_set_finish_fuse(int enable)
{
    g_finish_fuse.set(enable ? 1 : 0);
    return MFSR_OK;
}
extern "C" int mfsr_burst_debug_finish_fused(const mfsr_burst* b, int* finishes)
{
    MFSR_REQUIRE(b && finishes);
    *finishes = b->fusedFinishes;
    return MFSR_OK;
}
extern "C" int mfsr_burst_hold_fuse(mfsr_burst* b, int enable)
{
    MFSR_REQUIRE(b != nullptr);
    b->holdFuse = enable != 0;
    return MFSR_OK;
}
extern "C" int mfsr_burst_fuse_stats(const mfsr_burst* b, int* burstLaunches, int* groupsFused)
{
    MFSR_REQUIRE(b && burstLaunches && groupsFused);
    *burstLaunches = b->burstLaunches;
    *groupsFused = b->burstGroups;
    return MFSR_OK;
}

static bool can_hold_group(const mfsr_burst* b, bool hostBurst)
{
    const mfsr_config& c = b->cfg;
    if (!b->holdFuse || !burst_fuse_enabled() || hostBurst || b->heldHas || b->fuseStream || b->win.on) return false;
    if (!c.fused || c.mono || c.scale != 2 || b->group != MFSR_MAX_FUSE_GROUP || b->pend.n != MFSR_MAX_FUSE_GROUP) return false;
    if (b->L.tw * 2 != b->L.W || b->L.th * 2 != b->L.H) return false;
    if (b->nHold >= MFSR_MAX_BURST_FUSE / MFSR_MAX_FUSE_GROUP) return false;
    if (b->nHold > 0 && (b->hold[0].imgOut != b->pend.imgOut || b->hold[0].totalWeights != b->pend.totalWeights)) return false;
    for (int i = 0; i < b->pend.n; i++)
        if (upload_slot_of(b, b->pend.raw[i]) >= 0) return false;
    return true;
}

static int launch_group(mfsr_burst* b, const FuseGroup& g, mfsr_stream_t callerStream)
{
    const int n = g.n;
    if (n == 0) return MFSR_OK;
    mfsr_stream_t stream = callerStream;
    if (b->fuseStream) {
        stream = (mfsr_stream_t)b->fuseStream;
        for (int i = 0; i < n; i++) MFSR_HIP_TRY(hipStreamWaitEvent(b->fuseStream, b->evAligned[g.slot[i]], 0));
    }
    bool timed;
    TRY(timed_begin(b, stream, &timed));
    int freshNow;
    TRY(take_fresh(b, g.imgOut, g.totalWeights, stream, &freshNow));
    TRY(fuse_group(b, g, freshNow, 0, out_h(b), stream));
    TRY(timed_end(b, timed, 1, n, stream));
    TRY(release_group_slots(b, g, stream));
    if (b->fuseStream) {
        for (int i = 0; i < n; i++) {
            MFSR_HIP_TRY(hipEventRecord(b->evFused[g.slot[i]], b->fuseStream));
            b->fusedOutstanding[g.slot[i]] = true;
        }
    }
    return MFSR_OK;
}

static int drain_waiting(mfsr_burst* b, mfsr_stream_t stream, bool heldToo = true)
{
    const int G = b->nHold;
    b->nHold = 0;
    const mfsr_config& c = b->cfg;
    const Layout& L = b->L;
    int rc = MFSR_E_UNSUPPORTED;
    if (G >= 2) {
        const uint16_t* raws[MFSR_MAX_BURST_FUSE];
        mfsr_tex2d masks[MFSR_MAX_BURST_FUSE], flows[MFSR_MAX_BURST_FUSE];
        for (int g = 0; g < G; g++) {
            const int k = g * MFSR_MAX_FUSE_GROUP;
            for (int i = 0; i < MFSR_MAX_FUSE_GROUP; i++) raws[k + i] = b->hold[g].raw[i];
            group_tables(b->hold[g], masks + k, flows + k);
        }
        mfsr_float3* imgOut = b->hold[0].imgOut;
        mfsr_float3* totalWeights = b->hold[0].totalWeights;
        mfsr_tex2d acc[2];
        for (int p = 0; p < 2; p++) {
            acc[p].ptr = p ? (void*)totalWeights : (void*)imgOut;
            acc[p].pitch = 12 * L.hrW;
            acc[p].width = L.hrW;
            acc[p].height = L.hrH;
        }
        int freshNow = fresh_for(b, imgOut, totalWeights);
        bool timed;
        TRY(timed_begin(b, stream, &timed));
        const mfsr_float3 white = cfg_white(c), black = cfg_black(c);
        uint16_t* const out16 = b->finishOut16;
        b->finishOut16 = nullptr;
        if (out16) {
            mfsr_tex2d fb;
            fb.ptr = L.fallback.ptr;
            fb.pitch = L.fallback.pitch;
            fb.width = L.W;
            fb.height = L.H;
            rc = mfsr_cfa::accumulateSuperResBurstFinish(b->cfa, G * MFSR_MAX_FUSE_GROUP, raws, acc[0], acc[1], masks, as_tex(L.kparam4), flows, white,
                                                    black, c.scale, freshNow, fb, 0.0f, 1.0f, 0.0f, 1.0f, c.weightThreshold, out16,
                                                    L.hrW, L.hrH, 0, 65535.0f, 0, 0, L.hrW, L.hrH, stream);
            if (rc == MFSR_OK) {
                b->finishTaken = true;
                b->fusedFinishes++;
            }
        }
        if (rc == MFSR_E_UNSUPPORTED)
            rc = mfsr_cfa::accumulateSuperResBurst(b->cfa, G * MFSR_MAX_FUSE_GROUP, raws, acc[0], acc[1], masks, as_tex(L.kparam4), flows, white, black,
                                              c.scale, freshNow, stream);
        if (rc == MFSR_OK) {
            TRY(take_fresh(b, imgOut, totalWeights, stream, &freshNow));
            b->burstLaunches++;
            b->burstGroups += G;
            TRY(timed_end(b, timed, G, G * MFSR_MAX_FUSE_GROUP, stream));
        } else if (rc != MFSR_E_UNSUPPORTED)
            return rc;
    }
    for (int g = 0; g < G && rc == MFSR_E_UNSUPPORTED; g++) {
        TRY(wait_uploads(b, stream));
        TRY(launch_group(b, b->hold[g], stream));
    }
    if (!heldToo || !b->heldHas) return MFSR_OK;
    const FuseGroup held = b->held;
    b->heldHas = false;
    b->held.n = 0;
    TRY(wait_uploads(b, stream));
    return launch_group(b, held, stream);
}

static int accumulate_pending(mfsr_burst* b, mfsr_stream_t stream)
{
    TRY(drain_waiting(b, stream));
    TRY(align_deferred(b, b->pend, stream));
    TRY(wait_uploads(b, stream));
    const FuseGroup g = b->pend;
    b->pend.n = 0;
    return launch_group(b, g, stream);
}

static int wait_ref_products(mfsr_burst* b, mfsr_stream_t stream)
{
    if (b->refOnFuse && mfsr_s(stream) != b->fuseStream) MFSR_HIP_TRY(hipStreamWaitEvent(mfsr_s(stream), b->evRefDone, 0));
    return MFSR_OK;
}

static int join_fuse(mfsr_burst* b, mfsr_stream_t stream)
{
// ... 17 lines not shown
static bool lk_warped_path(const mfsr_burst* b)
{
    static const bool lkWarped = !mfsr_env_is0("MFSR_LK_WARPED");
    const mfsr_config& c = b->cfg;
    return c.fused && lkWarped && c.lkIterations > 0 && b->L.tw >= 64 && b->L.th >= 32;
}

static const Img* final_flow(const mfsr_burst* b, int slot, int isReference)
{
    const mfsr_config& c = b->cfg;
    return &b->L.flowBuf[2 * slot + (!isReference && c.fused ? (c.lkIterations & 1) : 0)];
}

static int align_pre(mfsr_burst* b, const uint16_t* raw, int isReference, int slot, const FrameProducts& mov, bool prepared,
                     const AlignScratch& work, const Img* suppliedShifts, mfsr_stream_t stream)
{
    const mfsr_config& c = b->cfg;
    const Layout& L = b->L;
    const FrameProducts& ref = b->ref;
    TRY(wait_uploads(b, stream));
    TRY(wait_slot_fused(b, slot, stream));
    const Img* flow = &L.flowBuf[2 * slot];
    if (isReference) {
        const Img* mask = &L.maskBuf[slot];
        MFSR_HIP_TRY(hipMemsetAsync(flow->ptr, 0, (size_t)flow->pitch * flow->h, mfsr_s(stream)));
        return mfsr_fill_f32((float*)mask->ptr, (size_t)mask->pitch / 4 * mask->h, 1.0f, stream);
    }
    if (!prepared) TRY(prepare_frame(b, raw, mov, stream));
    mfsr_prealign hostBase;
    const mfsr_prealign* hb = nullptr;
    if (c.preAlign) {
        if (!prepared) TRY(mfsr_preAlignPyramid((const float*)mov.pyr[0].ptr, L.tw, L.th, mov.pyr[0].pitch, mov.prePyr, stream));
        TRY(mfsr_preAlign(ref.prePyr, mov.prePyr, L.tw, L.th, c.preAlignMaxAngle, L.preWork, work.preResult, stream));
        b->preCur = work.preResult;
        if (!c.fused) {
            MFSR_HIP_TRY(hipMemcpyAsync(&hostBase, work.preResult, sizeof(hostBase), hipMemcpyDeviceToHost, mfsr_s(stream)));
            MFSR_HIP_TRY(hipStreamSynchronize(mfsr_s(stream)));
            hb = &hostBase;
        }
    }
    if (!suppliedShifts) TRY(track_tiles(b, ref, L.refSq, mov, work, hb, stream));
    const int last = c.levels - 1;
    const Img& tileShifts = suppliedShifts ? *suppliedShifts : work.shifts[last];
    const mfsr_float2 zero2 = {0.0f, 0.0f};
    if (lk_warped_path(b)) {
        TRY(mfsr_CreateFlowFieldWarped((mfsr_float2*)flow->ptr, as_tex(tileShifts), L.tw, L.th, flow->pitch, zero2, 0.0f,
                                       c.preAlign ? work.preResult : nullptr, (const float*)ref.pyr[0].ptr,
                                       (const float*)mov.pyr[0].ptr, ref.pyr[0].pitch, (float*)work.lkSum[0].ptr,
                                       (float*)work.lkDiff[0].ptr, work.lkSum[0].pitch, stream));
        b->paths[MFSR_PATH_FLOW_WARPED]++;
    } else if (c.preAlign && c.fused) {
        TRY(mfsr_CreateFlowFieldFromTilesBase((mfsr_float2*)flow->ptr, as_tex(tileShifts), L.tw, L.th, flow->pitch, work.preResult,
                                              stream));
        b->paths[MFSR_PATH_FLOW_BASE]++;
    } else {
        mfsr_float2 base = zero2;
        float rot = 0.0f;
        if (hb) {
            base.x = hb->shiftX;
            base.y = hb->shiftY;
            rot = hb->rotation;
        }
        TRY(mfsr_CreateFlowFieldFromTiles((mfsr_float2*)flow->ptr, as_tex(tileShifts), c.tileSize[last], L.tcx[last], L.tcy[last],
                                          L.tw, L.th, flow->pitch, base, rot, stream));
        b->paths[MFSR_PATH_FLOW_PLAIN]++;
    }
    return MFSR_OK;
}

static mfsr_lk_frame lk_frame_desc(const Layout& L, int slot, int it, bool lastIt, const FrameProducts& mov, const AlignScratch& work)
{
    const int in = it & 1, out = in ^ 1;
    mfsr_lk_frame f;
    f.shiftsIn = (const mfsr_float2*)L.flowBuf[2 * slot + in].ptr;
    f.shiftsOut = (mfsr_float2*)L.flowBuf[2 * slot + out].ptr;
    f.movedImg = (const float*)mov.pyr[0].ptr;
    f.sumIn = (const float*)work.lkSum[in].ptr;
    f.diffIn = (const float*)work.lkDiff[in].ptr;
    f.sumOut = lastIt ? nullptr : (float*)work.lkSum[out].ptr;
    f.diffOut = lastIt ? nullptr : (float*)work.lkDiff[out].ptr;
    return f;
}

static void prepare_table(const Layout& L, const FuseGroup& g, const int* idx, const int* mq, int m, mfsr_prepare_frame* pf)
{
    const int nlev = ilog2(L.maxFactor) + 1;
    for (int k = 0; k < m; k++) {
        const Img* pyr = L.mov[mq[k]].pyr;
        pf[k].dataIn = g.raw[idx[mq[k]]];
        pf[k].halfOut = (mfsr_float3*)L.mov[mq[k]].half.ptr;
        pf[k].pyr0 = (float*)pyr[0].ptr;
        pf[k].pyr1 = nlev > 1 ? (float*)pyr[1].ptr : nullptr;
    }
}

static int align_lk(mfsr_burst* b, int slot, const FrameProducts& mov, const AlignScratch& work, mfsr_stream_t stream)
{
    const mfsr_config& c = b->cfg;
    const Layout& L = b->L;
    const FrameProducts& ref = b->ref;
    const bool warped = lk_warped_path(b);
    for (int it = 0; it < c.lkIterations; it++) {
        const bool lastIt = it == c.lkIterations - 1;
        const int in = it & 1, out = in ^ 1;
        const float scale = lastIt ? (float)L.flowScale : 1.0f;
        const Img* flow = &L.flowBuf[2 * slot + (c.fused ? in : 0)];
        const Img* other = &L.flowBuf[2 * slot + out];
        if (warped) {
            const mfsr_lk_frame one = lk_frame_desc(L, slot, it, lastIt, mov, work);
            const int rcs = mfsr_lucasKanadeSweepBatch(1, &one, (const float*)ref.pyr[0].ptr, flow->pitch, ref.pyr[0].pitch,
                                                       work.lkSum[0].pitch, L.tw, L.th, c.lkHalfWindow, c.lkMinDet, scale, stream);
            if (rcs != MFSR_E_UNSUPPORTED) {
                if (rcs) return rcs;
                b->paths[MFSR_PATH_LK_SWEEP_SINGLE]++;
                continue;
            }
            TRY(mfsr_lucasKanadeIterationWarped((const mfsr_float2*)flow->ptr, (mfsr_float2*)other->ptr, flow->pitch,
                                                (const float*)ref.pyr[0].ptr, (const float*)mov.pyr[0].ptr, ref.pyr[0].pitch,
                                                one.sumIn, one.diffIn, one.sumOut, one.diffOut, work.lkSum[0].pitch, L.tw, L.th,
                                                c.lkHalfWindow, c.lkMinDet, scale, stream));
            b->paths[MFSR_PATH_LK_ITERATION_WARPED]++;
        } else if (c.fused) {
            TRY(mfsr_lucasKanadeIterationFused((const mfsr_float2*)flow->ptr, (mfsr_float2*)other->ptr, flow->pitch,
                                               (const float*)ref.pyr[0].ptr, (const float*)mov.pyr[0].ptr, ref.pyr[0].pitch, L.tw, L.th,
                                               c.lkHalfWindow, c.lkMinDet, scale, stream));
            b->paths[MFSR_PATH_LK_ITERATION_FUSED]++;
        } else {
            TRY(mfsr_WarpingKernel(L.tw, L.th, L.warped.pitch, as_tex(*flow), (float*)L.warped.ptr, as_tex(mov.pyr[0]), stream));
            TRY(mfsr_ComputeDerivativesKernel(L.tw, L.th, L.Ix.pitch, (float*)L.Ix.ptr, (float*)L.Iy.ptr, (float*)L.It.ptr,
                                              as_tex(L.warped), as_tex(ref.pyr[0]), stream));
            TRY(mfsr_lucasKanadeOptim((mfsr_float2*)flow->ptr, (const float*)L.Ix.ptr, (const float*)L.Iy.ptr, (const float*)L.It.ptr,
                                      flow->pitch, L.Ix.pitch, L.tw, L.th, c.lkHalfWindow, c.lkMinDet, stream));
            b->paths[MFSR_PATH_LK_CHAIN]++;
        }
    }
    if (L.flowScale != 1 && !(c.fused && c.lkIterations > 0)) {
        const Img* flow = final_flow(b, slot, 0);
        TRY(mfsr_scaleFlow((mfsr_float2*)flow->ptr, flow->pitch, L.tw, L.th, (float)L.flowScale, stream));
        b->paths[MFSR_PATH_SCALE_FLOW]++;
    }
    return MFSR_OK;
}

static int align_post(mfsr_burst* b, int slot, const FrameProducts& mov, mfsr_stream_t stream)
{
    const mfsr_config& c = b->cfg;
    const Layout& L = b->L;
    const FrameProducts& ref = b->ref;
    const Img* flow = final_flow(b, slot, 0);
    const Img* mask = &L.maskBuf[slot];
    const Img* fOut = c.maskErode > 0 ? &L.maskRaw[0] : mask;
    if (c.fused) {
        TRY(mfsr_robustnessMaskFused((const mfsr_float3*)ref.half.ptr, (const mfsr_float3*)mov.half.ptr, (mfsr_float4*)fOut->ptr,
                                     as_tex(*flow), L.hw, L.hh, ref.half.pitch, fOut->pitch, c.alpha, c.beta, c.thresholdM, stream));
        b->paths[MFSR_PATH_ROBUST_FUSED]++;
    } else {
        b->paths[MFSR_PATH_ROBUST_CHAIN]++;
        TRY(mfsr_zeroRing_f32x4((mfsr_float4*)fOut->ptr, fOut->pitch, L.hw, L.hh, stream));
        TRY(mfsr_ComputeRobustnessMask((const mfsr_float3*)ref.half.ptr, (const mfsr_float3*)mov.half.ptr, (mfsr_float4*)fOut->ptr,
                                       as_tex(*flow), L.hw, L.hh, ref.half.pitch, fOut->pitch, c.alpha, c.beta, c.thresholdM, stream));
    }
    if (c.maskErode > 0) {
        const mfsr_float4* ein = (const mfsr_float4*)fOut->ptr;
        mfsr_float4* eout = (mfsr_float4*)mask->ptr;
        TRY(mfsr_erodeMaskBatch(1, &ein, &eout, L.hw, L.hh, fOut->pitch, mask->pitch, c.maskErode, stream));
    }
    return MFSR_OK;
}

static void aligned_outputs(mfsr_burst* b, int slot, int isReference, const Img** flowOut, const Img** maskOut)
{
    *flowOut = b->slotFlow[slot] = final_flow(b, slot, isReference);
    *maskOut = &b->L.maskBuf[slot];
}

static int align_frame(mfsr_burst* b, const uint16_t* raw, int isReference, int slot, const FrameProducts* prepared,
                       const Img* suppliedShifts, const Img** flowOut, const Img** maskOut, mfsr_stream_t stream)
{
    const FrameProducts& mov = prepared ? *prepared : b->L.mov[0];
    const AlignScratch& work = b->L.work[0];
    TRY(align_pre(b, raw, isReference, slot, mov, prepared != nullptr, work, suppliedShifts, stream));
    if (!isReference) {
        TRY(align_lk(b, slot, mov, work, stream));
        TRY(align_post(b, slot, mov, stream));
    }
    aligned_outputs(b, slot, isReference, flowOut, maskOut);
    return MFSR_OK;
}

enum AlignBatch { ALIGN_BATCH_OFF, ALIGN_BATCH_LK, ALIGN_BATCH_STAGES };
static AlignBatch align_batch_mode()
{
    static const AlignBatch mode = [] {
        const char* e = getenv("MFSR_ALIGN_BATCH");
        if (e && e[0] == '0') return ALIGN_BATCH_OFF;
        return e && e[0] == '1' && e[1] == 's' ? ALIGN_BATCH_LK : ALIGN_BATCH_STAGES;
    }();
    return mode;
}

static bool can_defer_alignment(const mfsr_burst* b, bool supplied)
{
    const mfsr_config& c = b->cfg;
    static const bool hostDefer = mfsr_env_is1("MFSR_HOST_DEFER");
    const bool hostImmediate = b->holdLastGroup && !b->hostBusy && (b->framesSinceRef < b->group || !hostDefer);
    const Layout& L = b->L;
    return align_batch_mode() != ALIGN_BATCH_OFF && b->group > 1 && L.nAlign >= b->group && lk_warped_path(b) && !supplied &&
           !hostImmediate &&
           mfsr_lk_sweep_accepts(b->group, L.tw, L.th, c.lkHalfWindow, L.flowBuf[0].pitch, b->ref.pyr[0].pitch, L.work[0].lkSum[0].pitch) ==
               MFSR_OK;
}

static int align_deferred(mfsr_burst* b, FuseGroup& g, mfsr_stream_t stream)
{
    const mfsr_config& c = b->cfg;
    const Layout& L = b->L;
    const FrameProducts& ref = b->ref;
    int idx[MFSR_MAX_FUSE_GROUP], n = 0;
    for (int i = 0; i < g.n; i++)
        if (g.deferred[i]) idx[n++] = i;
    if (n == 0) return MFSR_OK;
    TRY(wait_uploads(b, stream));
    b->paths[MFSR_PATH_ALIGN_BATCHES]++;
    const int nlev = ilog2(L.maxFactor) + 1;
    bool stageBatch = align_batch_mode() == ALIGN_BATCH_STAGES && c.fused && !c.mono && !c.preAlign && b->ntaps / 2 <= 8 &&
                      L.tw == L.hw && L.th == L.hh;
    for (int l = 0; l < c.levels && stageBatch; l++) stageBatch = mfsr_trackTilesFastSupported(c.tileSize[l], c.maxShift[l]) != 0;
    int mq[MFSR_MAX_FUSE_GROUP], m = 0;
    for (int q = 0; q < n; q++)
        if (!g.isRef[idx[q]]) mq[m++] = q;
    const bool maskGroup = stageBatch && m > 0 && b->ntaps >= 3 && mfsr_robustness_group() != 0 &&
                           mfsr_robustness_group_fits(L.hh, L.flowBuf[0].pitch, L.mov[0].half.pitch, L.maskBuf[0].pitch) != 0;
    if (stageBatch) {
        b->paths[MFSR_PATH_STAGE_BATCHES]++;
        for (int q = 0; q < n; q++) {
            const int i = idx[q], slot = g.slot[i];
            if (g.isRef[i]) {
                TRY(align_pre(b, g.raw[i], 1, slot, L.mov[q], false, L.work[q], nullptr, stream));
            } else
                TRY(wait_slot_fused(b, slot, stream));
        }
        if (m > 0) {
            mfsr_prepare_frame pf[MFSR_MAX_FUSE_GROUP];
            prepare_table(L, g, idx, mq, m, pf);
            TRY(mfsr_cfa::prepareFrames(b->cfa, m, pf, L.mov[0].half.pitch, c.maxVal, L.hw, L.hh, L.mov[0].pyr[0].pitch,
                                        nlev > 1 ? L.mov[0].pyr[1].pitch : 0, b->taps, b->ntaps, stream, maskGroup));
            b->paths[MFSR_PATH_PREPARE_BATCH]++;
            for (int k = 0; k < m; k++) {
                const Img* pyr = L.mov[mq[k]].pyr;
                for (int i = 2; i < nlev; i++)
                    TRY(mfsr_downsample2x((const float*)pyr[i - 1].ptr, pyr[i - 1].pitch, (float*)pyr[i].ptr, pyr[i].pitch, pyr[i].w, pyr[i].h,
                                          stream));
            }
            for (int l = 0; l < c.levels; l++) {
                const int pi = ilog2(c.levelFactor[l]);
                mfsr_track_frame tf[MFSR_MAX_FUSE_GROUP];
                for (int k = 0; k < m; k++) {
                    tf[k].movedImg = (const float*)L.mov[mq[k]].pyr[pi].ptr;
                    tf[k].coarseShifts = l > 0 ? (const mfsr_float2*)L.work[mq[k]].shifts[l - 1].ptr : nullptr;
                    tf[k].coordinates = (mfsr_float2*)L.work[mq[k]].shifts[l].ptr;
                    tf[k].base = nullptr;
                }
                const Img& refImg = ref.pyr[pi];
                const Img* shifts = L.work[0].shifts;
                TRY(mfsr_trackTilesFusedBatch(m, tf, (const float*)refImg.ptr, l > 0 ? shifts[l - 1].pitch : 0, l > 0 ? c.levelFactor[l - 1] : 0,
                                              c.levelFactor[l], l > 0 ? L.tcx[l - 1] : 0, l > 0 ? L.tcy[l - 1] : 0,
                                              l > 0 ? c.tileSize[l - 1] : 0, shifts[l].pitch, refImg.w, refImg.h, refImg.pitch, c.maxShift[l],
                                              c.tileSize[l], L.tcx[l], L.tcy[l], c.minimumThreshold, L.refSq[l],
                                              1.0f / (float)c.levelFactor[l], stream));
                b->paths[MFSR_PATH_TRACK_FUSED_BATCH]++;
                b->paths[MFSR_PATH_TRACK_FAST_PAIR]++;
            }
            const int last = c.levels - 1;
            mfsr_flowfield_frame ff[MFSR_MAX_FUSE_GROUP];
            for (int k = 0; k < m; k++) {
                const int slot = g.slot[idx[mq[k]]];
                ff[k].outImg = (mfsr_float2*)L.flowBuf[2 * slot].ptr;
                ff[k].tileShifts = (const mfsr_float2*)L.work[mq[k]].shifts[last].ptr;
                ff[k].base = nullptr;
                ff[k].movedImg = (const float*)L.mov[mq[k]].pyr[0].ptr;
                ff[k].sumOut = (float*)L.work[mq[k]].lkSum[0].ptr;
                ff[k].diffOut = (float*)L.work[mq[k]].lkDiff[0].ptr;
            }
            const Img& grid = L.work[0].shifts[last];
            TRY(mfsr_CreateFlowFieldWarpedBatch(m, ff, grid.pitch, grid.w, grid.h, L.tw, L.th, L.flowBuf[0].pitch,
                                                (const float*)ref.pyr[0].ptr, ref.pyr[0].pitch, L.work[0].lkSum[0].pitch, stream));
            b->paths[MFSR_PATH_FLOW_WARPED_BATCH]++;
        }
    } else {
        for (int q = 0; q < n; q++) {
            const int i = idx[q];
            TRY(align_pre(b, g.raw[i], g.isRef[i], g.slot[i], L.mov[q], false, L.work[q], nullptr, stream));
        }
    }
    for (int it = 0; it < c.lkIterations; it++) {
        mfsr_lk_frame fr[MFSR_MAX_FUSE_GROUP];
        int m = 0;
        const bool lastIt = it == c.lkIterations - 1;
        for (int q = 0; q < n; q++)
            if (!g.isRef[idx[q]]) fr[m++] = lk_frame_desc(L, g.slot[idx[q]], it, lastIt, L.mov[q], L.work[q]);
        if (m == 0) break;
        TRY(mfsr_lucasKanadeSweepBatch(m, fr, (const float*)ref.pyr[0].ptr, L.flowBuf[0].pitch, ref.pyr[0].pitch, L.work[0].lkSum[0].pitch,
                                       L.tw, L.th, c.lkHalfWindow, c.lkMinDet, lastIt ? (float)L.flowScale : 1.0f, stream));
        b->paths[MFSR_PATH_LK_SWEEP_BATCH]++;
    }
    bool maskBatch = stageBatch && m > 0;
    if (maskBatch && maskGroup) {
        mfsr_robustness_group_frame gf[MFSR_MAX_FUSE_GROUP];
        for (int k = 0; k < m; k++) {
            const int slot = g.slot[idx[mq[k]]];
            gf[k].movedMeans = (const mfsr_float3*)L.mov[mq[k]].half.ptr;
            gf[k].movedRaw = g.raw[idx[mq[k]]];
            gf[k].mask = (mfsr_float4*)(c.maskErode > 0 ? L.maskRaw[k].ptr : L.maskBuf[slot].ptr);
            gf[k].flow = (const mfsr_float2*)final_flow(b, slot, 0)->ptr;
        }
        TRY(mfsr_cfa::robustnessMaskGroup(b->cfa, m, gf, (const mfsr_float3*)ref.half.ptr, ref.half.pitch, L.flowBuf[0].pitch, L.mov[0].half.pitch,
                                     L.maskBuf[0].pitch, L.hw, L.hh, c.maxVal, c.alpha, c.beta, c.thresholdM, stream));
        b->robustGroupLaunches++;
        b->paths[MFSR_PATH_ROBUST_BATCH]++;
    } else if (maskBatch) {
        mfsr_robustness_frame rf[MFSR_MAX_FUSE_GROUP];
        for (int k = 0; k < m; k++) {
            const int slot = g.slot[idx[mq[k]]];
            rf[k].movedHalf = (const mfsr_float3*)L.mov[mq[k]].half.ptr;
            rf[k].mask = (mfsr_float4*)(c.maskErode > 0 ? L.maskRaw[k].ptr : L.maskBuf[slot].ptr);
            rf[k].flow = (const mfsr_float2*)final_flow(b, slot, 0)->ptr;
        }
        const int rc = mfsr_robustnessMaskFusedBatch(m, rf, (const mfsr_float3*)ref.half.ptr, L.flowBuf[0].pitch, L.tw, L.th, L.hw, L.hh,
                                                     ref.half.pitch, L.maskBuf[0].pitch, c.alpha, c.beta, c.thresholdM, stream);
        if (rc == MFSR_E_UNSUPPORTED)
            maskBatch = false;
        else if (rc)
            return rc;
        else
            b->paths[MFSR_PATH_ROBUST_BATCH]++;
    }
    if (maskBatch && c.maskErode > 0) {
        const mfsr_float4* ein[MFSR_MAX_FUSE_GROUP];
        mfsr_float4* eout[MFSR_MAX_FUSE_GROUP];
        for (int k = 0; k < m; k++) {
            ein[k] = (const mfsr_float4*)L.maskRaw[k].ptr;
            eout[k] = (mfsr_float4*)L.maskBuf[g.slot[idx[mq[k]]]].ptr;
        }
        TRY(mfsr_erodeMaskBatch(m, ein, eout, L.hw, L.hh, L.maskRaw[0].pitch, L.maskBuf[0].pitch, c.maskErode, stream));
    }
    for (int q = 0; q < n; q++) {
        const int i = idx[q], slot = g.slot[i];
        if (!g.isRef[i] && !maskBatch) TRY(align_post(b, slot, L.mov[q], stream));
        aligned_outputs(b, slot, g.isRef[i], &g.flow[i], &g.mask[i]);
        g.deferred[i] = false;
        b->flowCur = g.flow[i];
        b->maskCur = g.mask[i];
        if (b->fuseStream) MFSR_HIP_TRY(hipEventRecord(b->evAligned[g.slot[i]], mfsr_s(stream)));
    }
    return MFSR_OK;
}

static int add_frame_impl(mfsr_burst* b, const uint16_t* raw, int isReference, mfsr_float3* imgOut, mfsr_float3* totalWeights,
                          bool hostBurst, mfsr_stream_t stream, const FrameProducts* prepared = nullptr,
                          const Img* suppliedShifts = nullptr)
{
    MFSR_REQUIRE(b && raw && imgOut && totalWeights);
    MFSR_REQUIRE(b->haveRef);
    MFSR_REQUIRE(!b->refStale);
    const mfsr_config& c = b->cfg;
    b->holdLastGroup = hostBurst;
    if (b->pend.n && (b->pend.imgOut != imgOut || b->pend.totalWeights != totalWeights)) TRY(flush_pending(b, stream));
    if (b->nHold && (b->hold[0].imgOut != imgOut || b->hold[0].totalWeights != totalWeights ||
                     b->nHold * MFSR_MAX_FUSE_GROUP + b->pend.n >= b->ring))
        TRY(drain_waiting(b, stream, false));
    if (b->pend.n >= b->group) TRY(accumulate_pending(b, stream));
    MFSR_REQUIRE(b->pend.n < MFSR_MAX_FUSE_GROUP);
    const int slot = b->frameCounter++ % b->ring;
    const Img *flow = nullptr, *mask = nullptr;
    const bool defer = can_defer_alignment(b, prepared || suppliedShifts);
    b->paths[defer ? MFSR_PATH_FRAMES_DEFERRED : MFSR_PATH_FRAMES_IMMEDIATE]++;
    if (!defer) {
        TRY(align_deferred(b, b->pend, stream));
        TRY(align_frame(b, raw, isReference, slot, prepared, suppliedShifts, &flow, &mask, stream));
        b->flowCur = flow;
        b->maskCur = mask;
        if (b->fuseStream) MFSR_HIP_TRY(hipEventRecord(b->evAligned[slot], mfsr_s(stream)));
    }
    if (defer) b->slotFlow[slot] = nullptr;
    const int i = b->pend.n++;
    b->pend.slot[i] = slot;
    b->pend.raw[i] = raw;
    b->pend.flow[i] = flow;
    b->pend.mask[i] = mask;
    b->pend.deferred[i] = defer;
    b->pend.isRef[i] = isReference;
    b->pend.imgOut = imgOut;
    b->pend.totalWeights = totalWeights;
    b->framesSinceRef++;
    if (b->pend.n < b->group) return MFSR_OK;
    if (b->holdLastGroup && b->framesSinceRef == c.frames) return MFSR_OK;
    static const int holdGroups = mfsr_env_int("MFSR_HOST_HOLD", 2);
    if (b->holdLastGroup && holdGroups >= 2 && !b->heldHas && c.frames - b->framesSinceRef <= b->group &&
        c.frames - b->framesSinceRef > 0 && !b->pend.deferred[0]) {
        bool aligned = true;
        for (int j = 0; j < b->pend.n; j++) aligned = aligned && !b->pend.deferred[j];
        if (aligned) {
            b->held = b->pend;
            b->heldHas = true;
            b->pend.n = 0;
            return MFSR_OK;
        }
    }
    if (can_hold_group(b, hostBurst)) {
        TRY(align_deferred(b, b->pend, stream));
        b->hold[b->nHold++] = b->pend;
        b->pend.n = 0;
        return MFSR_OK;
    }
    return accumulate_pending(b, stream);
}

extern "C" int mfsr_burst_add_frame(mfsr_burst* b, const uint16_t* raw, int isReference, mfsr_float3* imgOut,
                                    mfsr_float3* totalWeights, mfsr_stream_t stream)
{
    return add_frame_impl(b, raw, isReference, imgOut, totalWeights, false, stream);
}

extern "C" int mfsr_burst_group_size(const mfsr_config* cfg)
{
    if (!cfg || cfg->pairFrames <= 0) return 1;
    if (cfg->pairFrames >= 2) return cfg->pairFrames < MFSR_MAX_FUSE_GROUP ? cfg->pairFrames : MFSR_MAX_FUSE_GROUP;
    return ((cfg->scale == 2 || cfg->scale == 4) && !cfg->mono) ? MFSR_MAX_FUSE_GROUP : 2;
}

extern "C" int mfsr_burst_field_dims(const mfsr_burst* b, int* flowW, int* flowH, int* maskW, int* maskH)
{
    MFSR_REQUIRE(b != nullptr);
    if (flowW) *flowW = b->L.tw;
    if (flowH) *flowH = b->L.th;
    if (maskW) *maskW = b->L.hw;
    if (maskH) *maskH = b->L.hh;
    return MFSR_OK;
}

extern "C" int mfsr_burst_align_frame(mfsr_burst* b, const uint16_t* raw, int isReference, mfsr_float2* flowOut, int flowPitch,
                                      mfsr_float4* maskOut, int maskPitch, mfsr_stream_t stream)
{
    MFSR_REQUIRE(b && raw && flowOut && maskOut);
    MFSR_REQUIRE(b->haveRef);
    MFSR_REQUIRE(!b->refStale);
    const Layout& L = b->L;
    MFSR_REQUIRE((long long)flowPitch >= 8LL * L.tw && (flowPitch & 7) == 0 && ((uintptr_t)flowOut & 7) == 0);
    MFSR_REQUIRE((long long)maskPitch >= 16LL * L.hw && (maskPitch & 15) == 0 && ((uintptr_t)maskOut & 15) == 0);
    TRY(drain_waiting(b, stream, false));
    const int slot = b->frameCounter++ % b->ring;
    const Img *flow = nullptr, *mask = nullptr;
    TRY(align_frame(b, raw, isReference, slot, nullptr, nullptr, &flow, &mask, stream));
    b->flowCur = flow;
    b->maskCur = mask;
    MFSR_HIP_TRY(hipMemcpy2DAsync(flowOut, flowPitch, flow->ptr, flow->pitch, (size_t)L.tw * 8, L.th, hipMemcpyDeviceToDevice,
                                  mfsr_s(stream)));
    MFSR_HIP_TRY(hipMemcpy2DAsync(maskOut, maskPitch, mask->ptr, mask->pitch, (size_t)L.hw * 16, L.hh, hipMemcpyDeviceToDevice,
                                  mfsr_s(stream)));
    return MFSR_OK;
}

extern "C" int mfsr_burst_align_frames(mfsr_burst* b, int nFrames, const uint16_t* const* raws, const int* isReference,
                                       mfsr_float2* const* flowOut, int flowPitch, mfsr_float4* const* maskOut, int maskPitch,
                                       mfsr_stream_t stream)
{
    MFSR_REQUIRE(b && raws && flowOut && maskOut && nFrames >= 0);
    MFSR_REQUIRE(b->haveRef && !b->refStale);
    MFSR_REQUIRE(b->pend.n == 0);
    const Layout& L = b->L;
    MFSR_REQUIRE((long long)flowPitch >= 8LL * L.tw && (flowPitch & 7) == 0);
    MFSR_REQUIRE((long long)maskPitch >= 16LL * L.hw && (maskPitch & 15) == 0);
    for (int k = 0; k < nFrames; k++)
        MFSR_REQUIRE(raws[k] && flowOut[k] && maskOut[k] && ((uintptr_t)flowOut[k] & 7) == 0 && ((uintptr_t)maskOut[k] & 15) == 0);
    TRY(drain_waiting(b, stream, false));
    const bool batch = can_defer_alignment(b, false);
    const int per = batch ? b->group : 1;
    for (int k0 = 0; k0 < nFrames; k0 += per) {
        const int n = nFrames - k0 < per ? nFrames - k0 : per;
        FuseGroup p = {};
        p.n = n;
        for (int j = 0; j < n; j++) {
            p.slot[j] = b->frameCounter++ % b->ring;
            p.raw[j] = raws[k0 + j];
            p.isRef[j] = isReference ? isReference[k0 + j] : 0;
            p.deferred[j] = batch;
            if (!batch) TRY(align_frame(b, p.raw[j], p.isRef[j], p.slot[j], nullptr, nullptr, &p.flow[j], &p.mask[j], stream));
        }
        TRY(align_deferred(b, p, stream));
        for (int j = 0; j < n; j++) {
            b->flowCur = p.flow[j];
            b->maskCur = p.mask[j];
            MFSR_HIP_TRY(hipMemcpy2DAsync(flowOut[k0 + j], flowPitch, p.flow[j]->ptr, p.flow[j]->pitch, (size_t)L.tw * 8, L.th,
                                          hipMemcpyDeviceToDevice, mfsr_s(stream)));
            MFSR_HIP_TRY(hipMemcpy2DAsync(maskOut[k0 + j], maskPitch, p.mask[j]->ptr, p.mask[j]->pitch, (size_t)L.hw * 16, L.hh,
// ... 1084 lines not shown
    s->mask = s->flow0 + (size_t)(nFrames - 1) * s->flowBytes;
    s->total = s->mask + up256((size_t)16 * s->hw * s->hh);
    return true;
}
}

extern "C" size_t mfsr_noise_temporal_scratch_bytes(const mfsr_config* cfg, int nFrames)
{
    TemporalScratch s;
    return temporal_scratch(cfg, nFrames, &s) ? s.total : 0;
}

extern "C" int mfsr_burst_calibrate_noise_temporal(mfsr_burst* b, int nFrames, const uint16_t* const* frames, int reference, float tol,
                                                   int minBlocks, void* scratchDev, size_t scratchBytes, double* alpha, double* beta,
                                                   int32_t* status, int32_t* points, long long* blocks, mfsr_stream_t stream)
{
    MFSR_REQUIRE(b && frames && scratchDev && alpha && beta && status);
    MFSR_REQUIRE(nFrames >= 2 && nFrames <= 64 && reference >= 0 && reference < nFrames);
    MFSR_REQUIRE(!(tol > 0.25f) && tol == tol);
    for (int k = 0; k < nFrames; k++) MFSR_REQUIRE(frames[k] != nullptr && ((uintptr_t)frames[k] & 1) == 0);
    const mfsr_config& c = b->cfg;
    TemporalScratch s;
    MFSR_REQUIRE(temporal_scratch(&c, nFrames, &s));
    MFSR_REQUIRE(((uintptr_t)scratchDev & 255) == 0 && scratchBytes >= s.total);
    if (!burst_idle(b)) {
        fprintf(stderr, "mfsr: mfsr_burst_calibrate_noise_temporal with frames pending (flush or finish the burst first)\n");
        return MFSR_E_INVALID;
    }
    int32_t black[4], sat = 0, defBlocks = 0, r[4];
    float white[4];
    TRY(mfsr_noise_defaults(&c, black, white, &sat, &defBlocks, r));
    const float useTol = tol > 0.0f ? tol : 0.0625f;
    const int useBlocks = minBlocks > 0 ? minBlocks : defBlocks;

    TRY(flush_pending(b, stream));
    memset(b->paths, 0, sizeof(b->paths));
    b->sharpenedFinishes = b->denoisedFinishes = b->chainedFinishes = b->geometryFinishes = 0;
    b->robustGroupLaunches = 0;
    b->fusedFinishes = 0;
    TRY(mfsr_burst_set_reference(b, frames[reference], stream));

    char* base = (char*)scratchDev;
    const uint16_t* moved[64];
    const mfsr_float2* flows[64];
    mfsr_float2* flowOut[64];
    mfsr_float4* maskOut[64];
    int m = 0;
    for (int k = 0; k < nFrames; k++) {
        if (k == reference) {
            flows[k] = nullptr;
            continue;
        }
        moved[m] = frames[k];
        flowOut[m] = (mfsr_float2*)(base + s.flow0 + (size_t)m * s.flowBytes);
        maskOut[m] = (mfsr_float4*)(base + s.mask);
        flows[k] = flowOut[m];
        m++;
    }
    TRY(mfsr_burst_align_frames(b, m, moved, nullptr, flowOut, 8 * s.tw, maskOut, 16 * s.hw, stream));
    uint32_t* histDev = (uint32_t*)base;
    long long* sumDev = (long long*)(base + sizeof(uint32_t) * MFSR_NOISE_HIST_ENTRIES);
    long long* countDev = sumDev + MFSR_NOISE_LEVEL_ENTRIES;
    TRY(mfsr_noiseStatsTemporal(nFrames, frames, 2 * c.width, c.width, c.height, flows, 8 * s.tw, s.tw, s.th, black, sat, r, useTol,
                                histDev, sumDev, countDev, stream));
    std::vector<unsigned char> host(MFSR_NOISE_SCRATCH_BYTES);
    TRY(download(host.data(), scratchDev, host.size(), stream));
    const uint32_t* hist = (const uint32_t*)host.data();
    const long long* sum = (const long long*)(host.data() + sizeof(uint32_t) * MFSR_NOISE_HIST_ENTRIES);
    const long long* count = sum + MFSR_NOISE_LEVEL_ENTRIES;
    TRY(mfsr_noise_fit_temporal(hist, sum, count, black, white, useBlocks, alpha, beta, status, points));
    if (blocks) {
        long long n = 0;
        for (int l = 0; l < 64; l++) n += count[l];
        *blocks = n;
    }
    return MFSR_OK;
}

extern "C" int mfsr_burst_debug_views(mfsr_burst* b, mfsr_tex2d* flow, mfsr_tex2d* mask, mfsr_tex2d* kernelParam,
                                      mfsr_tex2d* tracking)
{
    MFSR_REQUIRE(b != nullptr);
    if ((flow || mask) && b->pend.n > 0 && b->pend.deferred[b->pend.n - 1]) return MFSR_E_INVALID;
    if (flow) *flow = as_tex(*b->flowCur);
    if (mask) *mask = as_tex(*b->maskCur);
    if (kernelParam) *kernelParam = as_tex(b->L.kparam4);
    if (tracking) *tracking = as_tex(b->ref.pyr[0]);
    return MFSR_OK;
}

extern "C" int mfsr_burst_debug_paths(const mfsr_burst* b, int32_t* counts, int capacity, int* count)
{
    MFSR_REQUIRE(b && counts && count && capacity >= 0);
    const int n = capacity < (int)MFSR_PATH_COUNT ? capacity : (int)MFSR_PATH_COUNT;
    for (int i = 0; i < n; i++) counts[i] = b->paths[i];
    *count = (int)MFSR_PATH_COUNT;
    return MFSR_OK;
}

extern "C" int mfsr_burst_debug_frame_views(mfsr_burst* b, int framesBack, mfsr_tex2d* flow, mfsr_tex2d* mask)
{
    MFSR_REQUIRE(b != nullptr && framesBack >= 0 && framesBack < b->ring && framesBack < b->frameCounter);
    const int slot = (int)((b->frameCounter - 1 - framesBack) % b->ring);
    MFSR_REQUIRE(b->slotFlow[slot] != nullptr);
    if (flow) *flow = as_tex(*b->slotFlow[slot]);
    if (mask) *mask = as_tex(b->L.maskBuf[slot]);
    return MFSR_OK;
}

extern "C" int mfsr_burst_prealign_result(mfsr_burst* b, mfsr_prealign* hostOut, mfsr_stream_t stream)
{
    MFSR_REQUIRE(b && hostOut);
    MFSR_REQUIRE(b->cfg.preAlign && b->preCur);
    TRY(align_deferred(b, b->pend, stream));
    MFSR_HIP_TRY(hipMemcpyAsync(hostOut, b->preCur, sizeof(*hostOut), hipMemcpyDeviceToHost, mfsr_s(stream)));
    MFSR_HIP_TRY(hipStreamSynchronize(mfsr_s(stream)));
    return MFSR_OK;
}

namespace {
struct StreamLayout {
    size_t burstWs, accBytes, entryBytes;
    size_t offBurst, offImg, offTw, offEntries, total;
};
size_t stream_entry(const mfsr_config* c, char* base, FrameProducts* fp)
{
    const Layout L = make_layout(c, nullptr);
    Bump b{base, 0};
    const int nl = ilog2(L.maxFactor) + 1;
    FrameProducts tmp;
    memset((void*)&tmp, 0, sizeof(tmp));
    tmp.raw = (uint16_t*)b.take((size_t)L.W * L.H * 2);
    tmp.half = b.image(L.hw, L.hh, 12);
    for (int i = 0; i < nl; i++) tmp.pyr[i] = b.image(L.tw >> i, L.th >> i, 4);
    tmp.prePyr = c->preAlign ? b.take(mfsr_preAlign_pyramid_bytes(L.tw, L.th)) : nullptr;
    if (fp) *fp = tmp;
    return align_up(b.off, 256);
}
int stream_layout(const mfsr_config* c, int radius, StreamLayout* S)
{
    memset(S, 0, sizeof(*S));
    const Layout L = make_layout(c, nullptr);
    S->burstWs = L.total;
    S->accBytes = (size_t)12 * L.hrW * L.hrH;
    S->entryBytes = stream_entry(c, nullptr, nullptr);
    size_t off = 0;
    S->offBurst = off;
    off = align_up(off + S->burstWs, 256);
    S->offImg = off;
    off = align_up(off + S->accBytes, 256);
    S->offTw = off;
    off = align_up(off + S->accBytes, 256);
    S->offEntries = off;
    off += S->entryBytes * (size_t)(2 * radius + 1);
    S->total = align_up(off, 256);
    return MFSR_OK;
}
}

struct mfsr_stream {
    mfsr_config cfg;
    int R, cap, hostFrames;
    mfsr_burst* b;
    StreamLayout S;
    mfsr_float3 *imgOut, *totalWeights;
    std::vector<FrameProducts>* fp;
    long long pushed, produced;
    hipStream_t copyStream;
    hipEvent_t evUp, evWindow[64];
    bool windowRecorded[64];
    long long lastWindow;
};

extern "C" size_t mfsr_stream_workspace_bytes(const mfsr_config* cfg, int radius)
{
    if (validate(cfg) != MFSR_OK || radius < 0 || radius > 15) return 0;
    StreamLayout S;
    stream_layout(cfg, radius, &S);
    return S.total;
}

extern "C" int mfsr_stream_create(mfsr_stream** out, const mfsr_config* cfg, int radius, int framesInHostMemory, void* workspace,
                                  size_t workspaceBytes)
{
    MFSR_REQUIRE(out && workspace && radius >= 0 && radius <= 15 && ((uintptr_t)workspace & 255) == 0);
    TRY(validate(cfg));
    mfsr_stream* s = new (std::nothrow) mfsr_stream;
    MFSR_REQUIRE(s != nullptr);
    memset((void*)s, 0, sizeof(*s));
    s->cfg = *cfg;
    s->cfg.frames = 2 * radius + 1;
    s->cfg.uploadRing = 0;
    s->R = radius;
    s->cap = 2 * radius + 1;
    s->hostFrames = framesInHostMemory ? 1 : 0;
    stream_layout(&s->cfg, radius, &s->S);
// ... 368 lines not shown
```

### multi_frame_super_resolution_amd/csrc/robustness.hip

```cpp
#include <cstdlib>
#include <cstring>
#include "common.hpp"
#include "half_pixel.hpp"

__global__ void __launch_bounds__(256)
    k_ComputeRobustnessMask(const pix3* __restrict__ rawImgRef, const pix3* __restrict__ rawImgMoved,
                            float4* __restrict__ robustnessMask, mfsr_tex2d texUV, int imgWidth, int imgHeight,
                            int imgPitch, int maskPitch, float alpha, float beta, float thresholdM)
{
    const int pxX = blockIdx.x * blockDim.x + threadIdx.x;
    const int pxY = blockIdx.y * blockDim.y + threadIdx.y;
    if (pxX >= imgWidth - 1 || pxY >= imgHeight - 1 || pxX < 1 || pxY < 1) return;

    const float2 shiftf =
        tex2<ADDR_CLAMP>(texUV, ((float)pxX + 0.5f) / (float)imgWidth, ((float)pxY + 0.5f) / (float)imgHeight);
    const float2 s = tex2<ADDR_CLAMP>(texUV, ((float)pxX + (float)2 + 0.5f) / (float)imgWidth,
                                      ((float)pxY + (float)2 + 0.5f) / (float)imgHeight);
    float2 maxShift, minShift;
    maxShift.x = fmaxf(s.x, shiftf.x);
    maxShift.y = fmaxf(s.y, shiftf.y);
    minShift.x = fminf(s.x, shiftf.x);
    minShift.y = fminf(s.y, shiftf.y);

    const int shx = round2i(shiftf.x * 0.5f);
// ... 104 lines not shown
        const pix3 p = row_ptr(rawImgRef, imgPitch, gy)[gx];
        sR[0][r][c] = p.x;
        sR[1][r][c] = p.y;
        sR[2][r][c] = p.z;
    }
    const int shxE = round2i(shiftfE.x * 0.5f), shyE = round2i(shiftfE.y * 0.5f);
    pix3 pmv[9];
#pragma unroll
    for (int y = 0; y < 3; y++) {
        const pix3* rm = row_ptr(rawImgMoved, imgPitch, clampi(pxYe + shyE + y - 1, 0, imgHeight - 1));
#pragma unroll
        for (int x = 0; x < 3; x++) pmv[y * 3 + x] = rm[clampi(pxXe + shxE + x - 1, 0, imgWidth - 1)];
    }
    __syncthreads();
    const int pxX = x0 + lx, pxY = y0 + ly;
    if (pxX >= imgWidth || pxY >= imgHeight) return;
    float4* out = row_ptr(robustnessMask, maskPitch, pxY) + pxX;
    if (pxX < 1 || pxY < 1 || pxX >= imgWidth - 1 || pxY >= imgHeight - 1) {
        *out = make_float4(0.0f, 0.0f, 0.0f, 0.0f);
        return;
    }
    const float2 shiftf = shiftfE, s = sE;
    float2 maxShift, minShift;
    maxShift.x = fmaxf(s.x, shiftf.x);
    maxShift.y = fmaxf(s.y, shiftf.y);
    minShift.x = fminf(s.x, shiftf.x);
    minShift.y = fminf(s.y, shiftf.y);

    float pr[3][9];
    float mr[3] = {0.0f, 0.0f, 0.0f}, mm[3] = {0.0f, 0.0f, 0.0f};
#pragma unroll
    for (int y = 0; y < 3; y++) {
#pragma unroll
        for (int x = 0; x < 3; x++) {
#pragma unroll
            for (int c = 0; c < 3; c++) {
                pr[c][y * 3 + x] = sR[c][ly + y][lx + x];
                mr[c] += pr[c][y * 3 + x];
            }
            const pix3 p = pmv[y * 3 + x];
            mm[0] += p.x;
            mm[1] += p.y;
            mm[2] += p.z;
        }
    }
#pragma unroll
    for (int c = 0; c < 3; c++) {
        mr[c] = div9(mr[c]);
        mm[c] = div9(mm[c]);
    }
    float meandist = fabsf(mr[0] - mm[0]) + fabsf(mr[1] - mm[1]) + fabsf(mr[2] - mm[2]);
    meandist = div3(meandist);
    const float hm = 0.5f * meandist;
    const float ddx = maxShift.x * hm - minShift.x * hm, ddy = maxShift.y * hm - minShift.y * hm;
    const float M = __builtin_amdgcn_sqrtf(ddx * ddx + ddy * ddy);
    const float sc = (M > thresholdM) ? 0.0f : 1.5f;
    float m3[3];
#pragma unroll
    for (int c = 0; c < 3; c++) {
        float sd2 = 0.0f;
#pragma unroll
        for (int p = 0; p < 9; p++) {
            const float d = pr[c][p] - mr[c];
            sd2 = __builtin_fmaf(d, d, sd2);
        }
        sd2 = div9(sd2);
        float smd2 = __builtin_fmaf(alpha, mr[c], beta);
        if (c == 1) smd2 *= 0.5f;
        const float sg2 = fmaxf(smd2, sd2);
        float d = fabsf(mr[c] - mm[c]);
        d = d * (sd2 * __builtin_amdgcn_rcpf(sd2 + smd2));
        const float e = __builtin_amdgcn_exp2f(-(d * d) * __builtin_amdgcn_rcpf(sg2) * 1.44269504088896340736f);
        m3[c] = fmaxf(fminf(__builtin_fmaf(sc, e, -0.12f), 1.0f), 0.0f);
    }
    *out = make_float4(m3[0], m3[1], m3[2], M);
}

struct RobustGroupFrame {
    const pix3* means;
    const uint16_t* raw;
    float4* mask;
    const float2* flow;
};
struct RobustGroupArgs {
    RobustGroupFrame f[MFSR_BATCH_MAX];
};
__device__ __forceinline__ int rb_wrap_add(int a, int b) { return (int)((unsigned)a + (unsigned)b); }

constexpr int RB_GROUP_WAVES = 8;
template <int NF>
__global__ void __launch_bounds__(RB_TX* RB_TY) __attribute__((amdgpu_waves_per_eu(RB_GROUP_WAVES, RB_GROUP_WAVES)))
    k_robustnessGroup(const pix3* __restrict__ rawImgRef, RobustGroupArgs ga, int imgWidth, int imgHeight, int imgPitch, int flowPitch,
                      int meansPitch, int maskPitch, float maxVal, int cfa, float alpha, float beta, float thresholdM, MfsrExactDiv dW,
                      MfsrExactDiv dH)
{
    __shared__ float sR[3][RB_TY + 2][RB_TX + 2];
    const int lx = threadIdx.x, ly = threadIdx.y;
    const int x0 = blockIdx.x * RB_TX, y0 = blockIdx.y * RB_TY;
    const int pxXe = min(x0 + lx, imgWidth - 1), pxYe = min(y0 + ly, imgHeight - 1);
    float2 shiftf[NF], s[NF];
    pix3 mm[NF];
    const TexCoord tc = tex_coord<ADDR_CLAMP>(imgWidth, imgHeight, mfsr_div((float)pxXe + 0.5f, dW), mfsr_div((float)pxYe + 0.5f, dH));
    const unsigned fr0 = (unsigned)tc.j0 * (unsigned)flowPitch, fr1 = (unsigned)tc.j1 * (unsigned)flowPitch;
    const unsigned o00 = fr0 + 8u * (unsigned)tc.i0, o10 = fr0 + 8u * (unsigned)tc.i1, o01 = fr1 + 8u * (unsigned)tc.i0,
                   o11 = fr1 + 8u * (unsigned)tc.i1;
    const unsigned oS = (unsigned)min(pxYe + 2, imgHeight - 1) * (unsigned)flowPitch + 8u * (unsigned)min(pxXe + 2, imgWidth - 1);
    auto fetch_flow = [&](int f) {
        const char* base = (const char*)ga.f[f].flow;
        const float2 t00 = *(const float2*)(base + o00), t10 = *(const float2*)(base + o10), t01 = *(const float2*)(base + o01),
                     t11 = *(const float2*)(base + o11);
        shiftf[f] = make_float2(lerp4(t00.x, t10.x, t01.x, t11.x, tc.a, tc.b), lerp4(t00.y, t10.y, t01.y, t11.y, tc.a, tc.b));
        s[f] = *(const float2*)(base + oS);
    };
    auto gather_mean = [&](int f) {
        const int qx = rb_wrap_add(pxXe, round2i(shiftf[f].x * 0.5f)), qy = rb_wrap_add(pxYe, round2i(shiftf[f].y * 0.5f));
        const unsigned o = (unsigned)clampi(qy, 0, imgHeight - 1) * (unsigned)meansPitch + 12u * (unsigned)clampi(qx, 0, imgWidth - 1);
        mm[f] = *(const pix3*)((const char*)ga.f[f].means + o);
    };
#pragma unroll
    for (int f = 0; f < NF && f < 2; f++) fetch_flow(f);
    for (int t = ly * RB_TX + lx; t < (RB_TY + 2) * (RB_TX + 2); t += RB_TX * RB_TY) {
        const int r = t / (RB_TX + 2), c = t - r * (RB_TX + 2);
        const int gy = clampi(y0 - 1 + r, 0, imgHeight - 1), gx = clampi(x0 - 1 + c, 0, imgWidth - 1);
        const pix3 p = row_ptr(rawImgRef, imgPitch, gy)[gx];
        sR[0][r][c] = p.x;
        sR[1][r][c] = p.y;
        sR[2][r][c] = p.z;
    }
#pragma unroll
    for (int f = 0; f < NF && f < 2; f++) gather_mean(f);
#pragma unroll
    for (int f = 2; f < NF; f++) fetch_flow(f);
    __syncthreads();
    const int pxX = x0 + lx, pxY = y0 + ly;
    if (pxX >= imgWidth || pxY >= imgHeight) return;
    const unsigned oM = (unsigned)pxY * (unsigned)maskPitch + 16u * (unsigned)pxX;
    if (pxX < 1 || pxY < 1 || pxX >= imgWidth - 1 || pxY >= imgHeight - 1) {
#pragma unroll
        for (int f = 0; f < NF; f++) *(float4*)((char*)ga.f[f].mask + oM) = make_float4(0.0f, 0.0f, 0.0f, 0.0f);
        return;
    }
#pragma unroll
    for (int f = 2; f < NF; f++) gather_mean(f);
    float mr[3], A[3], Rg[3];
    int patch = ly * (RB_TX + 2) + lx;
#pragma unroll
    for (int c = 0; c < 3; c++) {
        float pr[9];
        float m = 0.0f;
#pragma unroll
        for (int p = 0; p < 9; p++) {
            pr[p] = (&sR[c][0][0])[patch + (p / 3) * (RB_TX + 2) + p % 3];
            m += pr[p];
        }
        m = div9(m);
        float sd2 = 0.0f;
#pragma unroll
        for (int p = 0; p < 9; p++) {
            const float d = pr[p] - m;
            sd2 = __builtin_fmaf(d, d, sd2);
        }
        sd2 = div9(sd2);
        float smd2 = __builtin_fmaf(alpha, m, beta);
        if (c == 1) smd2 *= 0.5f;
        mr[c] = m;
        A[c] = sd2 * __builtin_amdgcn_rcpf(sd2 + smd2);
        Rg[c] = __builtin_amdgcn_rcpf(fmaxf(smd2, sd2));
        asm volatile("" : "+v"(patch) : "v"(mr[c]), "v"(A[c]), "v"(Rg[c]));
// ... 61 lines not shown
    texUV.pitch = flowPitch;
    texUV.width = flowWidth;
    texUV.height = flowHeight;
    MFSR_REQUIRE(mfsr_tex_ok(texUV, 8) && (flowPitch & 7) == 0);
    RobustFusedFrames fr;
    memset(&fr, 0, sizeof(fr));
    for (int i = 0; i < nFrames; i++) {
        MFSR_REQUIRE(frames[i].movedHalf && frames[i].mask && frames[i].flow);
        MFSR_REQUIRE(((uintptr_t)frames[i].mask & 15) == 0 && ((uintptr_t)frames[i].flow & 7) == 0);
        fr.f[i] = RobustFusedFrame{(const pix3*)frames[i].movedHalf, (float4*)frames[i].mask, (const float2*)frames[i].flow};
    }
    dim3 block(RB_TX, RB_TY), grid(mfsr_cdiv(imgWidth, RB_TX), mfsr_cdiv(imgHeight, RB_TY), nFrames);
    const MfsrExactDiv dW = mfsr_exact_div((float)imgWidth), dH = mfsr_exact_div((float)imgHeight);
    if (flowWidth == imgWidth && flowHeight == imgHeight)
        hipLaunchKernelGGL(k_robustnessFused<true>, grid, block, 0, mfsr_s(stream), (const pix3*)rawImgRef, fr, texUV, imgWidth, imgHeight,
                           imgPitch, maskPitch, alpha, beta, thresholdM, dW, dH);
    else
        hipLaunchKernelGGL(k_robustnessFused<false>, grid, block, 0, mfsr_s(stream), (const pix3*)rawImgRef, fr, texUV, imgWidth, imgHeight,
                           imgPitch, maskPitch, alpha, beta, thresholdM, dW, dH);
    return mfsr_launch_status(what);
}

extern "C" int mfsr_robustnessMaskFused(const mfsr_float3* rawImgRef, const mfsr_float3* rawImgMoved, mfsr_float4* robustnessMask,
                                        mfsr_tex2d texUV, int imgWidth, int imgHeight, int imgPitch, int maskPitch, float alpha,
                                        float beta, float thresholdM, mfsr_stream_t stream)
{
    MFSR_REQUIRE(rawImgRef && rawImgMoved && robustnessMask && imgWidth > 2 && imgHeight > 2);
    MFSR_REQUIRE((long long)imgPitch >= 12LL * imgWidth && (imgPitch & 3) == 0);
    MFSR_REQUIRE((long long)maskPitch >= 16LL * imgWidth && (maskPitch & 15) == 0 && ((uintptr_t)robustnessMask & 15) == 0);
    MFSR_REQUIRE(mfsr_tex_ok(texUV, 8) && ((uintptr_t)texUV.ptr & 7) == 0 && (texUV.pitch & 7) == 0);
    if (!g_robustness_fast) {
        int rc = mfsr_zeroRing_f32x4(robustnessMask, maskPitch, imgWidth, imgHeight, stream);
        if (rc) return rc;
        return mfsr_ComputeRobustnessMask(rawImgRef, rawImgMoved, robustnessMask, texUV, imgWidth, imgHeight, imgPitch, maskPitch,
                                          alpha, beta, thresholdM, stream);
    }
    const mfsr_robustness_frame one = {rawImgMoved, robustnessMask, (const mfsr_float2*)texUV.ptr};
    return robustness_fused_launch(1, &one, rawImgRef, texUV.pitch, texUV.width, texUV.height, imgWidth, imgHeight, imgPitch, maskPitch,
                                   alpha, beta, thresholdM, stream, "robustnessMaskFused");
}

extern "C" int mfsr_robustnessMaskFusedBatch(int nFrames, const mfsr_robustness_frame* frames, const mfsr_float3* rawImgRef, int flowPitch,
                                             int flowWidth, int flowHeight, int imgWidth, int imgHeight, int imgPitch, int maskPitch,
                                             float alpha, float beta, float thresholdM, mfsr_stream_t stream)
{
    MFSR_REQUIRE(frames && nFrames >= 1 && nFrames <= MFSR_BATCH_MAX && rawImgRef && imgWidth > 2 && imgHeight > 2);
    MFSR_REQUIRE((long long)imgPitch >= 12LL * imgWidth && (imgPitch & 3) == 0);
    MFSR_REQUIRE((long long)maskPitch >= 16LL * imgWidth && (maskPitch & 15) == 0);
    if (!g_robustness_fast) return MFSR_E_UNSUPPORTED;
    return robustness_fused_launch(nFrames, frames, rawImgRef, flowPitch, flowWidth, flowHeight, imgWidth, imgHeight, imgPitch, maskPitch,
                                   alpha, beta, thresholdM, stream, "robustnessMaskFusedBatch");
}

static MfsrKnob g_robustness_group;
extern "C" int mfsr_set_robustness_group(int enable)
{
    g_robustness_group.set(enable ? 1 : 0);
    return MFSR_OK;
}
int mfsr_robustness_group()
{
    return g_robustness_group.get([] { return mfsr_env_is0("MFSR_ROBUST_GROUP") ? 0 : 1; }) && g_robustness_fast;
}

int mfsr_robustness_group_fits(int h, int flowRowBytes, int meansRowBytes, int maskRowBytes)
{
    const long long lim = 1LL << 31;
    return (long long)flowRowBytes * h < lim && (long long)meansRowBytes * h < lim && (long long)maskRowBytes * h < lim;
}

template <int NF>
static void launch_robustness_group(int cfa, dim3 grid, dim3 block, hipStream_t st, const pix3* ref, const RobustGroupArgs& ga, int w, int h,
                                    int refRowBytes, int flowRowBytes, int meansRowBytes, int maskRowBytes, float maxVal, float alpha,
                                    float beta, float thresholdM)
{
    hipLaunchKernelGGL(k_robustnessGroup<NF>, grid, block, 0, st, ref, ga, w, h, refRowBytes, flowRowBytes, meansRowBytes, maskRowBytes,
                       maxVal, cfa, alpha, beta, thresholdM, mfsr_exact_div((float)w), mfsr_exact_div((float)h));
}

int mfsr_cfa::robustnessMaskGroup(int cfa, int nFrames, const mfsr_robustness_group_frame* frames, const mfsr_float3* refHalf,
                                  int refRowBytes, int flowRowBytes, int meansRowBytes, int maskRowBytes, int w, int h, float maxVal,
                                  float alpha, float beta, float thresholdM, mfsr_stream_t stream)
{
    MFSR_REQUIRE(frames && nFrames >= 1 && nFrames <= MFSR_BATCH_MAX && refHalf && w > 2 && h > 2);
    MFSR_REQUIRE((long long)refRowBytes >= 12LL * w && (refRowBytes & 3) == 0);
    MFSR_REQUIRE((long long)meansRowBytes >= 12LL * w && (meansRowBytes & 3) == 0);
    MFSR_REQUIRE((long long)maskRowBytes >= 16LL * w && (maskRowBytes & 15) == 0);
    MFSR_REQUIRE((long long)flowRowBytes >= 8LL * w && (flowRowBytes & 7) == 0);
    MFSR_REQUIRE(((uintptr_t)refHalf & 3) == 0);
    RobustGroupArgs ga;
    memset(&ga, 0, sizeof(ga));
    for (int i = 0; i < nFrames; i++) {
        MFSR_REQUIRE(frames[i].movedMeans && frames[i].movedRaw && frames[i].mask && frames[i].flow);
        MFSR_REQUIRE(((uintptr_t)frames[i].mask & 15) == 0 && ((uintptr_t)frames[i].flow & 7) == 0);
        MFSR_REQUIRE(((uintptr_t)frames[i].movedMeans & 3) == 0 && ((uintptr_t)frames[i].movedRaw & 3) == 0);
        ga.f[i].means = (const pix3*)frames[i].movedMeans;
        ga.f[i].raw = frames[i].movedRaw;
        ga.f[i].mask = (float4*)frames[i].mask;
        ga.f[i].flow = (const float2*)frames[i].flow;
    }
    if (!g_robustness_fast || !mfsr_robustness_group_fits(h, flowRowBytes, meansRowBytes, maskRowBytes)) return MFSR_E_UNSUPPORTED;
    dim3 block(RB_TX, RB_TY), grid(mfsr_cdiv(w, RB_TX), mfsr_cdiv(h, RB_TY));
    const pix3* ref = (const pix3*)refHalf;
    hipStream_t st = mfsr_s(stream);
#define RB_GROUP_ARGS cfa, grid, block, st, ref, ga, w, h, refRowBytes, flowRowBytes, meansRowBytes, maskRowBytes, maxVal, alpha, beta, thresholdM
    switch (nFrames) {
        case 1: launch_robustness_group<1>(RB_GROUP_ARGS); break;
        case 2: launch_robustness_group<2>(RB_GROUP_ARGS); break;
        case 3: launch_robustness_group<3>(RB_GROUP_ARGS); break;
        default: launch_robustness_group<4>(RB_GROUP_ARGS); break;
    }
#undef RB_GROUP_ARGS
    return mfsr_launch_status("robustnessMaskGroup");
}
extern "C" int mfsr_robustnessMaskGroup(int nFrames, const mfsr_robustness_group_frame* frames, const mfsr_float3* refHalf, int refRowBytes,
                                        int flowRowBytes, int meansRowBytes, int maskRowBytes, int w, int h, float maxVal, float alpha,
                                        float beta, float thresholdM, mfsr_stream_t stream)
{
    return mfsr_cfa::robustnessMaskGroup(mfsr_cfa_packed(), nFrames, frames, refHalf, refRowBytes, flowRowBytes, meansRowBytes, maskRowBytes, w,
                                         h, maxVal, alpha, beta, thresholdM, stream);
}

extern "C" int mfsr_ComputeRobustnessMask(const mfsr_float3* rawImgRef, const mfsr_float3* rawImgMoved,
                                          mfsr_float4* robustnessMask, mfsr_tex2d texUV, int imgWidth, int imgHeight,
                                          int imgPitch, int maskPitch, float alpha, float beta, float thresholdM,
                                          mfsr_stream_t stream)
{
    MFSR_REQUIRE(rawImgRef && rawImgMoved && robustnessMask && imgWidth > 2 && imgHeight > 2);
    MFSR_REQUIRE((long long)imgPitch >= 12LL * imgWidth && (imgPitch & 3) == 0);
    MFSR_REQUIRE((long long)maskPitch >= 16LL * imgWidth && (maskPitch & 15) == 0 && ((uintptr_t)robustnessMask & 15) == 0);
    MFSR_REQUIRE(mfsr_tex_ok(texUV, 8) && ((uintptr_t)texUV.ptr & 7) == 0 && (texUV.pitch & 7) == 0);
    dim3 block(64, 4), grid(mfsr_cdiv(imgWidth, 64), mfsr_cdiv(imgHeight, 4));
    hipLaunchKernelGGL(k_ComputeRobustnessMask, grid, block, 0, mfsr_s(stream), (const pix3*)rawImgRef,
                       (const pix3*)rawImgMoved, (float4*)robustnessMask, texUV, imgWidth, imgHeight, imgPitch, maskPitch,
                       alpha, beta, thresholdM);
    return mfsr_launch_status("ComputeRobustnessMask");
}
```

### multi_frame_super_resolution_amd/pipeline.py

```python
from __future__ import annotations

import ctypes
from collections import namedtuple
from typing import Iterable, Optional, Sequence, Tuple

import torch

from . import capi


def default_config(width: int, height: int, frames: int, scale: int = 2, mono: bool = False) -> capi.Config:
    cfg = capi.Config()
    capi.lib().config_default(ctypes.byref(cfg), width, height, frames, scale, 1 if mono else 0)
    return cfg


WINDOW_GRID = 16


def align_window(cfg: capi.Config, x: int, y: int, w: int, h: int) -> Tuple[int, int, int, int]:
    hr_w, hr_h = cfg.width * cfg.scale, cfg.height * cfg.scale
    if w <= 0 or h <= 0:
        raise ValueError("window must not be empty")
    x1, y1 = min(x + w, hr_w), min(y + h, hr_h)
# ... 857 lines not shown
        raise ValueError("count: a float32 device tensor of img's shape with dense pixels")
    h, w = int(img.shape[0]), int(img.shape[1])
    fw, fh = (w, h) if full is None else (int(full[0]), int(full[1]))
    with torch.cuda.device(img.device):
        c, grid, _ = _chain_struct(fw, fh, denoise, sharpen, local_tone, img.device)
        if c is None:
            raise ValueError("finish_chain_image: one stage at least must be on")
        r, lut, out = None, None, None
        if format is not None:
            r, lut = _render_struct(format, matrix, tone_lut, img.device, yuv)
            out = _render_buffer(format, h, w, img.device)
        two = format in capi.YUV_FORMATS
        fl = torch.empty(h, w, 3, dtype=torch.float32, device=img.device) if (want_float or out is None) else None
        rb = 0 if out is None else render_row_bytes(format, w)
        capi.lib().chainImage(img.data_ptr(), img.stride(0) * 4, None if count is None else count.data_ptr(),
                              0 if count is None else count.stride(0) * 4, None if fl is None else fl.data_ptr(), 12 * w,
                              None if out is None else out.data_ptr(), rb, out.data_ptr() + rb * h if two else None, rb if two else 0,
                              w, h, None if r is None else ctypes.byref(r), 1 if apply_gamma else 0, ctypes.byref(c),
                              None if grid is None else grid.data_ptr(), int(offset[0]), int(offset[1]), fw, fh,
                              torch.cuda.current_stream().cuda_stream)
        del lut, grid
    if out is None:
        return fl
    return (out, fl) if want_float else out


_GEO_FILTERS = {"bilinear": capi.GEO_BILINEAR, "cubic": capi.GEO_CUBIC}


def lens_geometry(src_w: int, src_h: int, out_w: int, out_h: int, zoom: float = 1.0, distortion=(0, 0, 0), lateral=(1, 1),
                  filter: str = "cubic") -> capi.Geometry:
    if filter not in _GEO_FILTERS:
        raise ValueError('filter: "bilinear" or "cubic"')
    k = [float(v) for v in distortion]
    lat = [float(v) for v in lateral]
    if len(k) != 3 or len(lat) != 2:
        raise ValueError("distortion: (k1, k2, k3); lateral: (red, blue)")
    g = capi.Geometry()
    if capi.lib().raw["mfsr_geometry_lens"](int(src_w), int(src_h), int(out_w), int(out_h), float(zoom), (ctypes.c_double * 3)(*k),
                                            (ctypes.c_double * 2)(*lat), _GEO_FILTERS[filter], ctypes.byref(g)) != 0:
        raise ValueError("lens_geometry: extents 1 .. 32768, step in [1/8, 8], |lateral - 1| <= 0.25, |k| <= 4, all finite")
    return g


def geometry_image(img: torch.Tensor, geometry: capi.Geometry, format: Optional[int] = None, matrix=None, tone_lut=None, rect=None,
                   apply_gamma: bool = False, want_float: bool = True):
    if not _dense_f3(img):
        raise ValueError("img: a float32 device tensor [h, w, 3] with dense pixels")
    src_h, src_w = int(img.shape[0]), int(img.shape[1])
    x, y, w, h = (0, 0, geometry.outW, geometry.outH) if rect is None else (int(v) for v in rect)
    with torch.cuda.device(img.device):
        r, lut, out = None, None, None
        if format is not None:
            r, lut = _render_struct(format, matrix, tone_lut, img.device)
            out = _render_buffer(format, h, w, img.device)
        fl = torch.empty(h, w, 3, dtype=torch.float32, device=img.device) if (want_float or out is None) else None
        capi.lib().geometryImage(img.data_ptr(), img.stride(0) * 4, src_w, src_h, None if fl is None else fl.data_ptr(), 12 * w,
                                 None if out is None else out.data_ptr(), 0 if out is None else render_row_bytes(format, w),
                                 None if r is None else ctypes.byref(r), ctypes.byref(geometry), 1 if apply_gamma else 0, x, y, w, h,
                                 torch.cuda.current_stream().cuda_stream)
        del lut
    if out is None:
        return fl
    return (out, fl) if want_float else out


class BurstPipeline:

    def __init__(self, cfg: capi.Config, device: Optional[torch.device] = None, window: Optional[Sequence[int]] = None):
        if not torch.cuda.is_available():
            raise RuntimeError("multi_frame_super_resolution_amd needs a HIP device (MI355X); there is no CPU fallback")
        self.L = capi.lib()
        self.cfg = cfg
        self.window = _Window(cfg, window)
        self._sharpen_on = self._denoise_on = False
        self._chain_reach = 0
        self._chain = self._chain_grid = None
        self._local_tone = None
        self.local_tone_result = None
        self.device = torch.device("cuda", torch.cuda.current_device()) if device is None else torch.device(device)
        nbytes = self.L.burst_workspace_bytes(ctypes.byref(cfg))
        if nbytes == 0:
            raise ValueError("invalid mfsr_config")
        with torch.cuda.device(self.device):
            self.workspace = torch.empty(nbytes + 256, dtype=torch.uint8, device=self.device)
            base = self.workspace.data_ptr()
            self._ws_ptr = (base + 255) // 256 * 256
            self.hr_w, self.hr_h = cfg.width * cfg.scale, cfg.height * cfg.scale
            out_h, out_w = self.window.aligned[3], self.window.aligned[2]
            self._img_out = torch.zeros(out_h, out_w, 3, dtype=torch.float32, device=self.device)
            self._total_weights = torch.zeros_like(self._img_out)
            self.out_img = torch.empty_like(self._img_out)
            self.out16 = torch.empty(out_h, out_w, 3, dtype=torch.int16, device=self.device)
            self._fmt = capi.OUT_RGB16
            handle = ctypes.c_void_p()
            self.L.burst_create(ctypes.byref(handle), ctypes.byref(cfg), self._ws_ptr, nbytes)
            self._h = handle
            self.window.apply(self.L.burst_set_window, self._h)
        self._hold = None
        self._held_frames = []

    def close(self):
        if getattr(self, "_h", None):
            self.L.burst_destroy(self._h)
            self._h = None

    def __del__(self):
        try:
            self.close()
        except Exception:
            pass

    @staticmethod
    def _stream() -> int:
        return torch.cuda.current_stream().cuda_stream

    def set_render(self, format: Optional[int] = capi.OUT_RGB16, matrix=None, tone_lut=None, yuv: int = 0):
        if format is not None:
            self.window.check_yuv(int(format))
        out_h, out_w = self.window.aligned[3], self.window.aligned[2]
        with torch.cuda.device(self.device):
            if format is None:
                self.L.burst_set_render(self._h, None)
                self._render_lut, fmt = None, capi.OUT_RGB16
            else:
                r, lut = _render_struct(format, matrix, tone_lut, self.device, yuv)
                self.L.burst_set_render(self._h, ctypes.byref(r))
                self._render_lut, fmt = lut, int(format)
            self.out16 = _render_buffer(fmt, out_h, out_w, self.device)
            self._out16_host = None
            self._fmt = fmt

    _AUTO_KEYS = {"lo": "lo", "hi": "hi", "chroma_tol": "chromaTol", "iterations": "iterations", "min_count": "minCount",
                  "tone_size": "toneSize"}
    _TONE_KEYS = {"p_lo": "pLo", "p_hi": "pHi", "max_gain": "maxGain", "mid": "mid"}

    def auto_render(self, format: int = capi.OUT_RGB8, matrix=None, awb: bool = True, tone: bool = True, yuv: int = 0,
                    tone_lut=None, **params) -> capi.AutoResult:
        self.window.check_yuv(int(format))
        out_h, out_w = self.window.aligned[3], self.window.aligned[2]
        ap = auto_defaults(out_h * out_w)
        ap.awb, ap.tone = int(bool(awb)), int(bool(tone))
        for k, v in params.items():
            if k in self._AUTO_KEYS:
                setattr(ap, self._AUTO_KEYS[k], int(v))
            elif k in self._TONE_KEYS:
                setattr(ap.toneParams, self._TONE_KEYS[k], float(v))
            else:
                raise TypeError(f"auto_render: unknown parameter {k!r}")
        if not 1 <= ap.toneSize <= 65536:
            raise ValueError("tone_size: 1 .. 65536")
        res = capi.AutoResult()
        with torch.cuda.device(self.device):
            r, lut = _render_struct(format, matrix, None if tone else tone_lut, self.device, yuv)
            table = torch.empty(capi.IMAGE_STATS_WORDS, dtype=torch.int64, device=self.device)
            if tone:
                lut = torch.empty(ap.toneSize + 1, dtype=torch.float32, device=self.device)
            self.L.burst_auto_render(self._h, self._img_out.data_ptr(), self._total_weights.data_ptr(), ctypes.byref(ap),
                                     table.data_ptr(), lut.data_ptr() if tone else None, ctypes.byref(r), ctypes.byref(res),
                                     self._stream())
            self._held_frames.clear()
            self._render_lut, self._auto_table = lut, table
            self.auto_description, self.auto_lut = r, lut
            self.out16 = _render_buffer(int(format), out_h, out_w, self.device)
            self._out16_host = None
            self._fmt = int(format)
# ... 520 lines not shown
```

Baseline: 26730.

## Batch alignment across two held fuse groups for eight-frame wide align launches

Held fuse groups now defer their alignment so that two groups (up to eight frames) are aligned together in one batch. The point is to launch the prepare, LK sweep and robustness kernels fewer times and give each launch more parallel work. The LK band heuristic gets a separate path for batches above four frames, and the Python pipeline allocates the larger workspace the extra align scratch needs. In exchange it uses more memory, adds deferred-alignment bookkeeping that query paths must flush, and robustness and erode kernels are still chunked at four frames.

```diff
diff --git a/include/mfsr.h b/include/mfsr.h
--- a/include/mfsr.h
+++ b/include/mfsr.h
@@ -339,6 +339,7 @@
                                int pitchSD, int width, int height, int halfWindowSize, float minDet, float outScale,
                                mfsr_stream_t stream);
 int mfsr_lucasKanadeSweepBand(int width, int height, int halfWindowSize, int nFrames);
+int mfsr_lucasKanadeSweepBandBatch(int imageWidth, int imageHeight, int halfWindowSize, int nFrames);
 int mfsr_CreateFlowFieldWarped(mfsr_float2* outImg, mfsr_tex2d texObjShiftXY, int imgWidth, int imgHeight, int imgPitch,
                                mfsr_float2 baseShift, float baseRotation, const mfsr_prealign* base, const float* refImg,
                                const float* movedImg, int pitchImg, float* sumOut, float* diffOut, int pitchSD,
@@ -390,6 +391,7 @@
 
 int mfsr_config_default(mfsr_config* cfg, int width, int height, int frames, int scale, int mono);
 size_t mfsr_burst_workspace_bytes(const mfsr_config* cfg);
+size_t mfsr_burst_wide_workspace_bytes(const mfsr_config* cfg);
 size_t mfsr_burst_accumulator_bytes(const mfsr_config* cfg);
 int mfsr_burst_create(mfsr_burst** out, const mfsr_config* cfg, void* workspace, size_t workspaceBytes);
 void mfsr_burst_destroy(mfsr_burst* b);
@@ -408,6 +410,8 @@
 int mfsr_set_burst_fuse(int enable);
 int mfsr_set_margin_sites(int enable);
 int mfsr_set_finish_fuse(int enable);
+int mfsr_set_align_width(int frames);
+int mfsr_get_align_width(void);
 int mfsr_burst_debug_finish_fused(const mfsr_burst* b, int* finishes);
 int mfsr_burst_finish(mfsr_burst* b, const mfsr_float3* imgOut, const mfsr_float3* totalWeights, mfsr_float3* outImg,
                       uint16_t* out16, mfsr_stream_t stream);
diff --git a/multi_frame_super_resolution_amd/capi.py b/multi_frame_super_resolution_amd/capi.py
--- a/multi_frame_super_resolution_amd/capi.py
+++ b/multi_frame_super_resolution_amd/capi.py
@@ -283,7 +283,8 @@
         ret = self.protos[full][0]
         if ret != "int" or full in ("mfsr_version", "mfsr_device_count", "mfsr_gaussin_filter_1D", "mfsr_burst_group_size",
                                      "mfsr_trackTilesFastSupported", "mfsr_packed_row_bytes", "mfsr_render_row_bytes",
-                                     "mfsr_get_accumulate_fast_exp", "mfsr_exactDivisionOk", "mfsr_lucasKanadeSweepBand"):
+                                     "mfsr_get_accumulate_fast_exp", "mfsr_exactDivisionOk", "mfsr_lucasKanadeSweepBand", "mfsr_lucasKanadeSweepBandBatch",
+                                     "mfsr_get_align_width"):
             return raw
 
         def checked(*a):
diff --git a/multi_frame_super_resolution_amd/csrc/common.hpp b/multi_frame_super_resolution_amd/csrc/common.hpp
--- a/multi_frame_super_resolution_amd/csrc/common.hpp
+++ b/multi_frame_super_resolution_amd/csrc/common.hpp
@@ -59,7 +59,7 @@
     return r;
 }
 
-#define MFSR_BATCH_MAX 4
+#define MFSR_BATCH_MAX 8
 
 #define MFSR_INTERNAL __attribute__((visibility("hidden")))
 
diff --git a/multi_frame_super_resolution_amd/csrc/debayer.hip b/multi_frame_super_resolution_amd/csrc/debayer.hip
--- a/multi_frame_super_resolution_amd/csrc/debayer.hip
+++ b/multi_frame_super_resolution_amd/csrc/debayer.hip
@@ -204,6 +204,7 @@
     for (int i = 0; i < n; i++) {
         MFSR_REQUIRE(f[i].dataIn && f[i].halfOut && f[i].pyr0 && ((uintptr_t)f[i].dataIn & 3) == 0);
         MFSR_REQUIRE((f[i].pyr1 != nullptr) == (f[0].pyr1 != nullptr));
+        for (int j = 0; j < i; j++) MFSR_REQUIRE(f[i].halfOut != f[j].halfOut && f[i].pyr0 != f[j].pyr0);
         fr.f[i] = PrepFrame{f[i].dataIn, (pix3*)f[i].halfOut, f[i].pyr0, f[i].pyr1};
     }
     if (f[0].pyr1) MFSR_REQUIRE((long long)pyr1Pitch >= 4LL * (dimX / 2) && (pyr1Pitch & 3) == 0 && dimX >= 2 && dimY >= 2);
diff --git a/multi_frame_super_resolution_amd/csrc/erode.hip b/multi_frame_super_resolution_amd/csrc/erode.hip
--- a/multi_frame_super_resolution_amd/csrc/erode.hip
+++ b/multi_frame_super_resolution_amd/csrc/erode.hip
@@ -5,8 +5,8 @@
 #define ER_ROWS 4
 
 struct ErodeFrames {
-    const float4* in[MFSR_MAX_FUSE_GROUP];
-    float4* out[MFSR_MAX_FUSE_GROUP];
+    const float4* in[MFSR_BATCH_MAX];
+    float4* out[MFSR_BATCH_MAX];
 };
 
 __device__ __forceinline__ float4 min3(const float4& a, const float4& b)
@@ -70,13 +70,13 @@
 extern "C" int mfsr_erodeMaskBatch(int nFrames, const mfsr_float4* const* in, mfsr_float4* const* out, int width, int height,
                                    int inPitch, int outPitch, int radius, mfsr_stream_t stream)
 {
-    MFSR_REQUIRE(nFrames >= 1 && nFrames <= MFSR_MAX_FUSE_GROUP && in != nullptr && out != nullptr);
+    MFSR_REQUIRE(nFrames >= 1 && nFrames <= MFSR_BATCH_MAX && in != nullptr && out != nullptr);
     MFSR_REQUIRE(radius >= 1 && radius <= 2);
     MFSR_REQUIRE(width >= 3 && height >= 3);
     MFSR_REQUIRE((long long)inPitch >= 16LL * width && (inPitch & 15) == 0);
     MFSR_REQUIRE((long long)outPitch >= 16LL * width && (outPitch & 15) == 0);
     ErodeFrames fr;
-    for (int k = 0; k < MFSR_MAX_FUSE_GROUP; k++) {
+    for (int k = 0; k < MFSR_BATCH_MAX; k++) {
         fr.in[k] = nullptr;
         fr.out[k] = nullptr;
     }
diff --git a/multi_frame_super_resolution_amd/csrc/lk_fused.hip b/multi_frame_super_resolution_amd/csrc/lk_fused.hip
--- a/multi_frame_super_resolution_amd/csrc/lk_fused.hip
+++ b/multi_frame_super_resolution_amd/csrc/lk_fused.hip
@@ -427,7 +427,7 @@
                                   pitchImg, pitchSD, stream);
 }
 
-#define MFSR_LK_SWEEP_MAX_BATCH 4
+#define MFSR_LK_SWEEP_MAX_BATCH MFSR_BATCH_MAX
 struct LkSweepFrame {
     const float2* flowIn;
     float2* flowOut;
@@ -587,18 +587,29 @@
     return MFSR_OK;
 }
 
-extern "C" int mfsr_lucasKanadeSweepBand(int width, int height, int halfWindowSize, int nFrames)
+extern "C" int mfsr_lucasKanadeSweepBandBatch(int width, int height, int halfWindowSize, int nFrames)
 {
     if (!lk_sweep_geometry(nFrames, width, height, halfWindowSize)) return 0;
     const int h = halfWindowSize, VW = 64 - 2 * (h + 2);
     const int strips = mfsr_cdiv(width, VW);
     static const int forceBand = mfsr_env_int("MFSR_LK_BAND", 0);
+    static const int occ[8] = {0, 8, 7, 6, 5, 4, 4, 4};
+    const long long places = 1024LL * occ[h];
+    if (nFrames > 4) {
+        int band = 0;
+        for (long long k = 1; band == 0; k++) {
+            const long long maxBands = k * places / ((long long)strips * nFrames);
+            if (maxBands < 1) continue;
+            int b = (int)((height + maxBands - 1) / maxBands);
+            b = b < 8 ? 8 : b;
+            if (b <= 64) band = b;
+        }
+        return forceBand >= 8 ? forceBand : band;
+    }
     int band = (int)((long long)height * strips * nFrames / 8192);
     band = (band + 4) & ~7;
     band = band < 8 ? 8 : (band > 32 ? 32 : band);
     {
-        static const int occ[8] = {0, 8, 7, 6, 5, 4, 4, 4};
-        const long long places = 1024LL * occ[h];
         const long long maxBands = places / ((long long)strips * nFrames);
         if (maxBands >= 1) {
             int b = (int)((height + maxBands - 1) / maxBands);
@@ -608,6 +619,11 @@
     }
     if (forceBand >= 8) band = forceBand;
     return band;
+}
+
+extern "C" int mfsr_lucasKanadeSweepBand(int width, int height, int halfWindowSize, int nFrames)
+{
+    return nFrames <= 4 ? mfsr_lucasKanadeSweepBandBatch(width, height, halfWindowSize, nFrames) : 0;
 }
 
 extern "C" int mfsr_lucasKanadeSweepBatch(int nFrames, const mfsr_lk_frame* frames, const float* refImg, int pitchShift, int pitchImg,
@@ -625,11 +641,12 @@
         MFSR_REQUIRE(((uintptr_t)f.shiftsIn & 7) == 0 && ((uintptr_t)f.shiftsOut & 7) == 0);
         MFSR_REQUIRE((f.sumOut != nullptr) == (f.diffOut != nullptr) && f.sumOut != f.sumIn && f.diffOut != f.diffIn);
         MFSR_REQUIRE(!f.sumOut || outScale == 1.0f);
-        b.f[i] = LkSweepFrame{(const float2*)f.shiftsIn, (float2*)f.shiftsOut, f.movedImg, f.sumIn, f.diffIn, f.sumOut, f.diffOut};
+        for (int j = 0; j < i; j++) MFSR_REQUIRE(f.shiftsOut != frames[j].shiftsOut);
+        b.f[i] =LkSweepFrame{(const float2*)f.shiftsIn, (float2*)f.shiftsOut, f.movedImg, f.sumIn, f.diffIn, f.sumOut, f.diffOut};
     }
     const int h = halfWindowSize, VW = 64 - 2 * (h + 2);
     const int strips = mfsr_cdiv(width, VW);
-    const int band = mfsr_lucasKanadeSweepBand(width, height, h, nFrames);
+    const int band = mfsr_lucasKanadeSweepBandBatch(width, height, h, nFrames);
     static const int xcdRemap = mfsr_env_int("MFSR_LK_XCD", 1);
     const int bands = mfsr_cdiv(height, band);
     const int total = strips * bands * nFrames;
diff --git a/multi_frame_super_resolution_amd/csrc/pipeline.cpp b/multi_frame_super_resolution_amd/csrc/pipeline.cpp
--- a/multi_frame_super_resolution_amd/csrc/pipeline.cpp
+++ b/multi_frame_super_resolution_amd/csrc/pipeline.cpp
@@ -45,8 +45,8 @@
     int lw[kMaxLevels], lh[kMaxLevels];
     int tcx[kMaxLevels], tcy[kMaxLevels];
     int maxFactor;
-    FrameProducts ref, mov[MFSR_MAX_FUSE_GROUP];
-    AlignScratch work[MFSR_MAX_FUSE_GROUP];
+    FrameProducts ref, mov[MFSR_BATCH_MAX];
+    AlignScratch work[MFSR_BATCH_MAX];
     int nAlign;
     Img kparam4;
     Img tensor, tensorTmp, tensorSm;
@@ -64,6 +64,7 @@
     uint16_t* refRaw[2];
     uint8_t* stage[kMaxUploadRing + 2];
     size_t total;
+    size_t totalWide;
 };
 
 struct Bump {
@@ -127,7 +128,15 @@
     return MFSR_OK;
 }
 
-Layout make_layout(const mfsr_config* c, char* base)
+int align_capacity(const mfsr_config* c)
+{
+    if (!c->fused) return 1;
+    const int group = mfsr_burst_group_size(c);
+    const bool holds = !c->mono && c->scale == 2 && group == MFSR_MAX_FUSE_GROUP && c->frames >= 2 * MFSR_MAX_FUSE_GROUP;
+    return holds ? MFSR_BATCH_MAX : group;
+}
+
+Layout make_layout(const mfsr_config* c, char* base, size_t avail = 0)
 {
     Layout layout;
     memset((void*)&layout, 0, sizeof(layout));
@@ -205,8 +214,8 @@
         L->preWork = b.take(mfsr_preAlign_workspace_bytes(c->preAlignMaxAngle));
         L->work[0].preResult = (mfsr_prealign*)b.take(sizeof(mfsr_prealign));
     }
-    L->nAlign = c->fused ? mfsr_burst_group_size(c) : 1;
-    for (int q = 1; q < L->nAlign; q++) {
+    L->nAlign = align_capacity(c);
+    auto align_position = [&](int q) {
         FrameProducts& M = L->mov[q];
         AlignScratch& S = L->work[q];
         M.half = b.image(L->hw, L->hh, 12);
@@ -220,7 +229,9 @@
             M.prePyr = b.take(mfsr_preAlign_pyramid_bytes(L->tw, L->th));
             S.preResult = (mfsr_prealign*)b.take(sizeof(mfsr_prealign));
         }
-    }
+    };
+    const int groupAlign = c->fused ? mfsr_burst_group_size(c) : 1;
+    for (int q = 1; q < groupAlign; q++) align_position(q);
     for (int i = 0; i < c->uploadRing; i++) L->rawRing[i] = (uint16_t*)b.take((size_t)L->W * L->H * 2);
     if (c->uploadRing > 0)
         for (int i = 0; i < 2; i++) L->refRaw[i] = (uint16_t*)b.take((size_t)L->W * L->H * 2);
@@ -235,6 +246,9 @@
         L->maskBuf[i] = b.image(L->hw, L->hh, 16);
     }
     L->total = align_up(b.off, 256);
+    for (int q = groupAlign; q < L->nAlign; q++) align_position(q);
+    L->totalWide = align_up(b.off, 256);
+    if (avail < L->totalWide) L->nAlign = groupAlign;
     return layout;
 }
 
@@ -262,7 +276,7 @@
 };
 
 struct mfsr_burst {
-    mfsr_burst(const mfsr_config& c, char* workspace) : cfg(c), L(make_layout(&c, workspace)) {}
+    mfsr_burst(const mfsr_config& c, char* workspace, size_t bytes) : cfg(c), L(make_layout(&c, workspace, bytes)) {}
     mfsr_config cfg;
     int cfa;
     const Layout L;
@@ -283,6 +297,8 @@
     bool holdFuse;
     int nHold;
     FuseGroup hold[MFSR_MAX_BURST_FUSE / MFSR_MAX_FUSE_GROUP];
+    int nUnaligned;
+    mfsr_stream_t waitStream;
     int burstLaunches, burstGroups;
     int nFramesTimed;
     struct Fresh {
@@ -468,6 +484,12 @@
     return make_layout(cfg, nullptr).total;
 }
 
+extern "C" size_t mfsr_burst_wide_workspace_bytes(const mfsr_config* cfg)
+{
+    if (validate(cfg) != MFSR_OK) return 0;
+    return make_layout(cfg, nullptr).totalWide;
+}
+
 extern "C" size_t mfsr_burst_accumulator_bytes(const mfsr_config* cfg)
 {
     if (!cfg || cfg->width <= 0 || cfg->height <= 0 || cfg->scale <= 0) return 0;
@@ -485,7 +507,7 @@
         return MFSR_E_NODEVICE;
     }
     MFSR_REQUIRE(((uintptr_t)workspace & 255) == 0);
-    mfsr_burst* b = new (std::nothrow) mfsr_burst(*cfg, (char*)workspace);
+    mfsr_burst* b = new (std::nothrow) mfsr_burst(*cfg, (char*)workspace, workspaceBytes);
     MFSR_REQUIRE(b != nullptr);
     if (b->L.total > workspaceBytes) {
         fprintf(stderr, "mfsr: workspace too small: need %zu bytes, got %zu\n", b->L.total, workspaceBytes);
@@ -504,6 +526,8 @@
     b->ring = ring_size(&b->cfg);
     b->holdFuse = false;
     b->nHold = 0;
+    b->nUnaligned = 0;
+    b->waitStream = nullptr;
     b->burstLaunches = b->burstGroups = 0;
     b->fresh.has = false;
     b->nFramesTimed = 0;
@@ -991,6 +1015,7 @@
 }
 
 static int align_deferred(mfsr_burst* b, FuseGroup& g, mfsr_stream_t stream);
+static int align_waiting(mfsr_burst* b, mfsr_stream_t stream);
 
 static int timed_begin(mfsr_burst* b, mfsr_stream_t stream, bool* timed)
 {
@@ -1075,6 +1100,20 @@
     g_finish_fuse.set(enable ? 1 : 0);
     return MFSR_OK;
 }
+static MfsrKnob g_align_width;
+static int align_width()
+{
+    return g_align_width.get([] {
+        return mfsr_env_int("MFSR_ALIGN_WIDTH", MFSR_BATCH_MAX) == MFSR_MAX_FUSE_GROUP ? MFSR_MAX_FUSE_GROUP : MFSR_BATCH_MAX;
+    });
+}
+extern "C" int mfsr_set_align_width(int frames)
+{
+    MFSR_REQUIRE(frames == MFSR_MAX_FUSE_GROUP || frames == MFSR_BATCH_MAX);
+    g_align_width.set(frames);
+    return MFSR_OK;
+}
+extern "C" int mfsr_get_align_width(void) { return align_width(); }
 extern "C" int mfsr_burst_debug_finish_fused(const mfsr_burst* b, int* finishes)
 {
     MFSR_REQUIRE(b && finishes);
@@ -1135,6 +1174,7 @@
 
 static int drain_waiting(mfsr_burst* b, mfsr_stream_t stream, bool heldToo = true)
 {
+    TRY(align_waiting(b, stream));
     const int G = b->nHold;
     b->nHold = 0;
     const mfsr_config& c = b->cfg;
@@ -1318,12 +1358,20 @@
     return f;
 }
 
-static void prepare_table(const Layout& L, const FuseGroup& g, const int* idx, const int* mq, int m, mfsr_prepare_frame* pf)
+struct BatchFrame {
+    FuseGroup* g;
+    int i;
+    const uint16_t* raw() const { return g->raw[i]; }
+    int slot() const { return g->slot[i]; }
+    int isRef() const { return g->isRef[i]; }
+};
+
+static void prepare_table(const Layout& L, const BatchFrame* fr, const int* mq, int m, mfsr_prepare_frame* pf)
 {
     const int nlev = ilog2(L.maxFactor) + 1;
     for (int k = 0; k < m; k++) {
         const Img* pyr = L.mov[mq[k]].pyr;
-        pf[k].dataIn = g.raw[idx[mq[k]]];
+        pf[k].dataIn = fr[mq[k]].raw();
         pf[k].halfOut = (mfsr_float3*)L.mov[mq[k]].half.ptr;
         pf[k].pyr0 = (float*)pyr[0].ptr;
         pf[k].pyr1 = nlev > 1 ? (float*)pyr[1].ptr : nullptr;
@@ -1447,14 +1495,19 @@
                MFSR_OK;
 }
 
-static int align_deferred(mfsr_burst* b, FuseGroup& g, mfsr_stream_t stream)
+static int align_batch(mfsr_burst* b, FuseGroup* const* groups, int nGroups, mfsr_stream_t stream)
 {
     const mfsr_config& c = b->cfg;
     const Layout& L = b->L;
     const FrameProducts& ref = b->ref;
-    int idx[MFSR_MAX_FUSE_GROUP], n = 0;
-    for (int i = 0; i < g.n; i++)
-        if (g.deferred[i]) idx[n++] = i;
+    BatchFrame bf[MFSR_BATCH_MAX];
+    int n = 0;
+    for (int k = 0; k < nGroups; k++)
+        for (int i = 0; i < groups[k]->n; i++)
+            if (groups[k]->deferred[i]) {
+                MFSR_REQUIRE(n < L.nAlign && n < MFSR_BATCH_MAX);
+                bf[n++] = BatchFrame{groups[k], i};
+            }
     if (n == 0) return MFSR_OK;
     TRY(wait_uploads(b, stream));
     b->paths[MFSR_PATH_ALIGN_BATCHES]++;
@@ -1462,23 +1515,23 @@
     bool stageBatch = align_batch_mode() == ALIGN_BATCH_STAGES && c.fused && !c.mono && !c.preAlign && b->ntaps / 2 <= 8 &&
                       L.tw == L.hw && L.th == L.hh;
     for (int l = 0; l < c.levels && stageBatch; l++) stageBatch = mfsr_trackTilesFastSupported(c.tileSize[l], c.maxShift[l]) != 0;
-    int mq[MFSR_MAX_FUSE_GROUP], m = 0;
+    int mq[MFSR_BATCH_MAX], m = 0;
     for (int q = 0; q < n; q++)
-        if (!g.isRef[idx[q]]) mq[m++] = q;
+        if (!bf[q].isRef()) mq[m++] = q;
     const bool maskGroup = stageBatch && m > 0 && b->ntaps >= 3 && mfsr_robustness_group() != 0 &&
                            mfsr_robustness_group_fits(L.hh, L.flowBuf[0].pitch, L.mov[0].half.pitch, L.maskBuf[0].pitch) != 0;
     if (stageBatch) {
         b->paths[MFSR_PATH_STAGE_BATCHES]++;
         for (int q = 0; q < n; q++) {
-            const int i = idx[q], slot = g.slot[i];
-            if (g.isRef[i]) {
-                TRY(align_pre(b, g.raw[i], 1, slot, L.mov[q], false, L.work[q], nullptr, stream));
+            const int slot = bf[q].slot();
+            if (bf[q].isRef()) {
+                TRY(align_pre(b, bf[q].raw(), 1, slot, L.mov[q], false, L.work[q], nullptr, stream));
             } else
                 TRY(wait_slot_fused(b, slot, stream));
         }
         if (m > 0) {
-            mfsr_prepare_frame pf[MFSR_MAX_FUSE_GROUP];
-            prepare_table(L, g, idx, mq, m, pf);
+            mfsr_prepare_frame pf[MFSR_BATCH_MAX];
+            prepare_table(L, bf, mq, m, pf);
             TRY(mfsr_cfa::prepareFrames(b->cfa, m, pf, L.mov[0].half.pitch, c.maxVal, L.hw, L.hh, L.mov[0].pyr[0].pitch,
                                         nlev > 1 ? L.mov[0].pyr[1].pitch : 0, b->taps, b->ntaps, stream, maskGroup));
             b->paths[MFSR_PATH_PREPARE_BATCH]++;
@@ -1490,7 +1543,7 @@
             }
             for (int l = 0; l < c.levels; l++) {
                 const int pi = ilog2(c.levelFactor[l]);
-                mfsr_track_frame tf[MFSR_MAX_FUSE_GROUP];
+                mfsr_track_frame tf[MFSR_BATCH_MAX];
                 for (int k = 0; k < m; k++) {
                     tf[k].movedImg = (const float*)L.mov[mq[k]].pyr[pi].ptr;
                     tf[k].coarseShifts = l > 0 ? (const mfsr_float2*)L.work[mq[k]].shifts[l - 1].ptr : nullptr;
@@ -1508,9 +1561,9 @@
                 b->paths[MFSR_PATH_TRACK_FAST_PAIR]++;
             }
             const int last = c.levels - 1;
-            mfsr_flowfield_frame ff[MFSR_MAX_FUSE_GROUP];
+            mfsr_flowfield_frame ff[MFSR_BATCH_MAX];
             for (int k = 0; k < m; k++) {
-                const int slot = g.slot[idx[mq[k]]];
+                const int slot = bf[mq[k]].slot();
                 ff[k].outImg = (mfsr_float2*)L.flowBuf[2 * slot].ptr;
                 ff[k].tileShifts = (const mfsr_float2*)L.work[mq[k]].shifts[last].ptr;
                 ff[k].base = nullptr;
@@ -1525,63 +1578,66 @@
         }
     } else {
         for (int q = 0; q < n; q++) {
-            const int i = idx[q];
-            TRY(align_pre(b, g.raw[i], g.isRef[i], g.slot[i], L.mov[q], false, L.work[q], nullptr, stream));
+            TRY(align_pre(b, bf[q].raw(), bf[q].isRef(), bf[q].slot(), L.mov[q], false, L.work[q], nullptr, stream));
         }
     }
     for (int it = 0; it < c.lkIterations; it++) {
-        mfsr_lk_frame fr[MFSR_MAX_FUSE_GROUP];
-        int m = 0;
+        if (m == 0) break;
+        mfsr_lk_frame fr[MFSR_BATCH_MAX];
         const bool lastIt = it == c.lkIterations - 1;
-        for (int q = 0; q < n; q++)
-            if (!g.isRef[idx[q]]) fr[m++] = lk_frame_desc(L, g.slot[idx[q]], it, lastIt, L.mov[q], L.work[q]);
-        if (m == 0) break;
+        for (int k = 0; k < m; k++) fr[k] = lk_frame_desc(L, bf[mq[k]].slot(), it, lastIt, L.mov[mq[k]], L.work[mq[k]]);
         TRY(mfsr_lucasKanadeSweepBatch(m, fr, (const float*)ref.pyr[0].ptr, L.flowBuf[0].pitch, ref.pyr[0].pitch, L.work[0].lkSum[0].pitch,
                                        L.tw, L.th, c.lkHalfWindow, c.lkMinDet, lastIt ? (float)L.flowScale : 1.0f, stream));
         b->paths[MFSR_PATH_LK_SWEEP_BATCH]++;
     }
     bool maskBatch = stageBatch && m > 0;
-    if (maskBatch && maskGroup) {
-        mfsr_robustness_group_frame gf[MFSR_MAX_FUSE_GROUP];
-        for (int k = 0; k < m; k++) {
-            const int slot = g.slot[idx[mq[k]]];
-            gf[k].movedMeans = (const mfsr_float3*)L.mov[mq[k]].half.ptr;
-            gf[k].movedRaw = g.raw[idx[mq[k]]];
-            gf[k].mask = (mfsr_float4*)(c.maskErode > 0 ? L.maskRaw[k].ptr : L.maskBuf[slot].ptr);
-            gf[k].flow = (const mfsr_float2*)final_flow(b, slot, 0)->ptr;
-        }
-        TRY(mfsr_cfa::robustnessMaskGroup(b->cfa, m, gf, (const mfsr_float3*)ref.half.ptr, ref.half.pitch, L.flowBuf[0].pitch, L.mov[0].half.pitch,
-                                     L.maskBuf[0].pitch, L.hw, L.hh, c.maxVal, c.alpha, c.beta, c.thresholdM, stream));
-        b->robustGroupLaunches++;
-        b->paths[MFSR_PATH_ROBUST_BATCH]++;
-    } else if (maskBatch) {
-        mfsr_robustness_frame rf[MFSR_MAX_FUSE_GROUP];
-        for (int k = 0; k < m; k++) {
-            const int slot = g.slot[idx[mq[k]]];
-            rf[k].movedHalf = (const mfsr_float3*)L.mov[mq[k]].half.ptr;
-            rf[k].mask = (mfsr_float4*)(c.maskErode > 0 ? L.maskRaw[k].ptr : L.maskBuf[slot].ptr);
-            rf[k].flow = (const mfsr_float2*)final_flow(b, slot, 0)->ptr;
-        }
-        const int rc = mfsr_robustnessMaskFusedBatch(m, rf, (const mfsr_float3*)ref.half.ptr, L.flowBuf[0].pitch, L.tw, L.th, L.hw, L.hh,
-                                                     ref.half.pitch, L.maskBuf[0].pitch, c.alpha, c.beta, c.thresholdM, stream);
-        if (rc == MFSR_E_UNSUPPORTED)
-            maskBatch = false;
-        else if (rc)
-            return rc;
-        else
+    for (int k0 = 0; k0 < m && maskBatch; k0 += MFSR_MAX_FUSE_GROUP) {
+        const int mc = m - k0 < MFSR_MAX_FUSE_GROUP ? m - k0 : MFSR_MAX_FUSE_GROUP;
+        const int* cq = mq + k0;
+        if (maskGroup) {
+            mfsr_robustness_group_frame gf[MFSR_MAX_FUSE_GROUP];
+            for (int k = 0; k < mc; k++) {
+                const int slot = bf[cq[k]].slot();
+                gf[k].movedMeans = (const mfsr_float3*)L.mov[cq[k]].half.ptr;
+                gf[k].movedRaw = bf[cq[k]].raw();
+                gf[k].mask = (mfsr_float4*)(c.maskErode > 0 ? L.maskRaw[k].ptr : L.maskBuf[slot].ptr);
+                gf[k].flow = (const mfsr_float2*)final_flow(b, slot, 0)->ptr;
+            }
+            TRY(mfsr_cfa::robustnessMaskGroup(b->cfa, mc, gf, (const mfsr_float3*)ref.half.ptr, ref.half.pitch, L.flowBuf[0].pitch,
+                                              L.mov[0].half.pitch, L.maskBuf[0].pitch, L.hw, L.hh, c.maxVal, c.alpha, c.beta, c.thresholdM,
+                                              stream));
+            b->robustGroupLaunches++;
             b->paths[MFSR_PATH_ROBUST_BATCH]++;
-    }
-    if (maskBatch && c.maskErode > 0) {
-        const mfsr_float4* ein[MFSR_MAX_FUSE_GROUP];
-        mfsr_float4* eout[MFSR_MAX_FUSE_GROUP];
-        for (int k = 0; k < m; k++) {
-            ein[k] = (const mfsr_float4*)L.maskRaw[k].ptr;
-            eout[k] = (mfsr_float4*)L.maskBuf[g.slot[idx[mq[k]]]].ptr;
-        }
-        TRY(mfsr_erodeMaskBatch(m, ein, eout, L.hw, L.hh, L.maskRaw[0].pitch, L.maskBuf[0].pitch, c.maskErode, stream));
+        } else {
+            mfsr_robustness_frame rf[MFSR_MAX_FUSE_GROUP];
+            for (int k = 0; k < mc; k++) {
+                const int slot = bf[cq[k]].slot();
+                rf[k].movedHalf = (const mfsr_float3*)L.mov[cq[k]].half.ptr;
+                rf[k].mask = (mfsr_float4*)(c.maskErode > 0 ? L.maskRaw[k].ptr : L.maskBuf[slot].ptr);
+                rf[k].flow = (const mfsr_float2*)final_flow(b, slot, 0)->ptr;
+            }
+            const int rc = mfsr_robustnessMaskFusedBatch(mc, rf, (const mfsr_float3*)ref.half.ptr, L.flowBuf[0].pitch, L.tw, L.th, L.hw, L.hh,
+                                                         ref.half.pitch, L.maskBuf[0].pitch, c.alpha, c.beta, c.thresholdM, stream);
+            if (rc == MFSR_E_UNSUPPORTED) {
+                maskBatch = false;
+                break;
+            }
+            if (rc) return rc;
+            b->paths[MFSR_PATH_ROBUST_BATCH]++;
+        }
+        if (c.maskErode > 0) {
+            const mfsr_float4* ein[MFSR_MAX_FUSE_GROUP];
+            mfsr_float4* eout[MFSR_MAX_FUSE_GROUP];
+            for (int k = 0; k < mc; k++) {
+                ein[k] = (const mfsr_float4*)L.maskRaw[k].ptr;
+                eout[k] = (mfsr_float4*)L.maskBuf[bf[cq[k]].slot()].ptr;
+            }
+            TRY(mfsr_erodeMaskBatch(mc, ein, eout, L.hw, L.hh, L.maskRaw[0].pitch, L.maskBuf[0].pitch, c.maskErode, stream));
+        }
     }
     for (int q = 0; q < n; q++) {
-        const int i = idx[q], slot = g.slot[i];
+        FuseGroup& g = *bf[q].g;
+        const int i = bf[q].i, slot = g.slot[i];
         if (!g.isRef[i] && !maskBatch) TRY(align_post(b, slot, L.mov[q], stream));
         aligned_outputs(b, slot, g.isRef[i], &g.flow[i], &g.mask[i]);
         g.deferred[i] = false;
@@ -1590,6 +1646,23 @@
         if (b->fuseStream) MFSR_HIP_TRY(hipEventRecord(b->evAligned[g.slot[i]], mfsr_s(stream)));
     }
     return MFSR_OK;
+}
+
+static int align_deferred(mfsr_burst* b, FuseGroup& g, mfsr_stream_t stream)
+{
+    FuseGroup* one = &g;
+    return align_batch(b, &one, 1, stream);
+}
+
+static int align_waiting(mfsr_burst* b, mfsr_stream_t stream)
+{
+    const int u = b->nUnaligned;
+    if (u == 0) return MFSR_OK;
+    b->nUnaligned = 0;
+    FuseGroup* groups[MFSR_BATCH_MAX / MFSR_MAX_FUSE_GROUP];
+    MFSR_REQUIRE(u <= MFSR_BATCH_MAX / MFSR_MAX_FUSE_GROUP && u <= b->nHold);
+    for (int k = 0; k < u; k++) groups[k] = &b->hold[b->nHold - u + k];
+    return align_batch(b, groups, u, stream);
 }
 
 static int add_frame_impl(mfsr_burst* b, const uint16_t* raw, int isReference, mfsr_float3* imgOut, mfsr_float3* totalWeights,
@@ -1612,6 +1685,7 @@
     const bool defer = can_defer_alignment(b, prepared || suppliedShifts);
     b->paths[defer ? MFSR_PATH_FRAMES_DEFERRED : MFSR_PATH_FRAMES_IMMEDIATE]++;
     if (!defer) {
+        TRY(align_waiting(b, stream));
         TRY(align_deferred(b, b->pend, stream));
         TRY(align_frame(b, raw, isReference, slot, prepared, suppliedShifts, &flow, &mask, stream));
         b->flowCur = flow;
@@ -1644,9 +1718,18 @@
         }
     }
     if (can_hold_group(b, hostBurst)) {
-        TRY(align_deferred(b, b->pend, stream));
+        bool wide = align_width() > MFSR_MAX_FUSE_GROUP && b->L.nAlign >= MFSR_BATCH_MAX;
+        for (int j = 0; j < b->pend.n; j++) wide = wide && b->pend.deferred[j];
+        if (!wide) {
+            TRY(align_waiting(b, stream));
+            TRY(align_deferred(b, b->pend, stream));
+        }
         b->hold[b->nHold++] = b->pend;
         b->pend.n = 0;
+        if (wide) {
+            b->waitStream = stream;
+            if (++b->nUnaligned == MFSR_BATCH_MAX / MFSR_MAX_FUSE_GROUP) TRY(align_waiting(b, stream));
+        }
         return MFSR_OK;
     }
     return accumulate_pending(b, stream);
@@ -2897,6 +2980,7 @@
 {
     MFSR_REQUIRE(b != nullptr);
     if ((flow || mask) && b->pend.n > 0 && b->pend.deferred[b->pend.n - 1]) return MFSR_E_INVALID;
+    if (flow || mask) TRY(align_waiting(b, b->waitStream));
     if (flow) *flow = as_tex(*b->flowCur);
     if (mask) *mask = as_tex(*b->maskCur);
     if (kernelParam) *kernelParam = as_tex(b->L.kparam4);
@@ -2917,6 +3001,7 @@
 {
     MFSR_REQUIRE(b != nullptr && framesBack >= 0 && framesBack < b->ring && framesBack < b->frameCounter);
     const int slot = (int)((b->frameCounter - 1 - framesBack) % b->ring);
+    if (b->slotFlow[slot] == nullptr) TRY(align_waiting(b, b->waitStream));
     MFSR_REQUIRE(b->slotFlow[slot] != nullptr);
     if (flow) *flow = as_tex(*b->slotFlow[slot]);
     if (mask) *mask = as_tex(b->L.maskBuf[slot]);
@@ -2927,6 +3012,7 @@
 {
     MFSR_REQUIRE(b && hostOut);
     MFSR_REQUIRE(b->cfg.preAlign && b->preCur);
+    TRY(align_waiting(b, stream));
     TRY(align_deferred(b, b->pend, stream));
     MFSR_HIP_TRY(hipMemcpyAsync(hostOut, b->preCur, sizeof(*hostOut), hipMemcpyDeviceToHost, mfsr_s(stream)));
     MFSR_HIP_TRY(hipStreamSynchronize(mfsr_s(stream)));
diff --git a/multi_frame_super_resolution_amd/csrc/robustness.hip b/multi_frame_super_resolution_amd/csrc/robustness.hip
--- a/multi_frame_super_resolution_amd/csrc/robustness.hip
+++ b/multi_frame_super_resolution_amd/csrc/robustness.hip
@@ -210,8 +210,9 @@
     float4* mask;
     const float2* flow;
 };
+constexpr int RB_GROUP_MAX = 4;
 struct RobustGroupArgs {
-    RobustGroupFrame f[MFSR_BATCH_MAX];
+    RobustGroupFrame f[RB_GROUP_MAX];
 };
 __device__ __forceinline__ int rb_wrap_add(int a, int b) { return (int)((unsigned)a + (unsigned)b); }
 
@@ -439,7 +440,7 @@
                                   int refRowBytes, int flowRowBytes, int meansRowBytes, int maskRowBytes, int w, int h, float maxVal,
                                   float alpha, float beta, float thresholdM, mfsr_stream_t stream)
 {
-    MFSR_REQUIRE(frames && nFrames >= 1 && nFrames <= MFSR_BATCH_MAX && refHalf && w > 2 && h > 2);
+    MFSR_REQUIRE(frames && nFrames >= 1 && nFrames <= RB_GROUP_MAX && refHalf && w > 2 && h > 2);
     MFSR_REQUIRE((long long)refRowBytes >= 12LL * w && (refRowBytes & 3) == 0);
     MFSR_REQUIRE((long long)meansRowBytes >= 12LL * w && (meansRowBytes & 3) == 0);
     MFSR_REQUIRE((long long)maskRowBytes >= 16LL * w && (maskRowBytes & 15) == 0);
diff --git a/multi_frame_super_resolution_amd/pipeline.py b/multi_frame_super_resolution_amd/pipeline.py
--- a/multi_frame_super_resolution_amd/pipeline.py
+++ b/multi_frame_super_resolution_amd/pipeline.py
@@ -963,6 +963,7 @@
         nbytes = self.L.burst_workspace_bytes(ctypes.byref(cfg))
         if nbytes == 0:
             raise ValueError("invalid mfsr_config")
+        nbytes = max(nbytes, self.L.burst_wide_workspace_bytes(ctypes.byref(cfg)))
         with torch.cuda.device(self.device):
             self.workspace = torch.empty(nbytes + 256, dtype=torch.uint8, device=self.device)
             base = self.workspace.data_ptr()
```

After: 26980, median of 6. About the same (+0.9%).
